# index-tts/index-tts

Hardware: AMD Instinct MI355X
Metric: audio-seconds/sec (RTF) IndexTTS-2.5, 64-utt batch @1/2/4/8 MI355X (higher is better)
Workload: dtype bf16 (GPT GEMM operands / KV cache; f32 accumulate, residual stream, norms: the reference's own GPU mode) + fp32x3 (flow matching: f32 activations / weights / accumulation, GEMM and attention products on the bf16 matrix pipe with every f32 operand carried exactly as three bf16 planes = 24 significan

## Files before the change

indextts_amd/csrc/capi_s2mel.hip:

```cpp
#include <math.h>
#include <stdlib.h>
#include <string.h>
#include <algorithm>
#include <map>
#include <string>
#include <vector>

#include "../../include/indextts_hip.h"
#include "gpt_kernels.h"
#include "s2mel_kernels.h"

static bool s2_fused(int precision, bool opt_fused) {
    if (precision == PREC_F32X3) return true;
    return (precision == PREC_BF16 || precision == PREC_F32) && opt_fused;
}

struct S2Layer {
    void *w_qkv = 0, *w_o = 0, *w_13 = 0, *w_2 = 0, *w_skip_a = 0, *w_skip_b = 0;
    float *g_attn = 0, *g_ffn = 0, *b_skip = 0;
};
struct S2Wn {
    void *w_in = 0, *w_rs = 0;
    float *b_in = 0, *b_rs = 0;
};

struct itts_s2mel {
    itts_s2mel_config cfg;
    int I = 0, Kx = 0;
    std::map<std::string, std::pair<std::vector<float>, std::vector<int64_t>>> host;
    std::vector<S2Layer> layers;
    std::vector<S2Wn> wn;
    float* g_norm = 0;
    void *w_x = 0, *w_sl_a = 0, *w_sl_b = 0, *w_c1 = 0, *w_rp = 0, *w_fl = 0, *w_c2 = 0;
    float *b_sl = 0, *b_c1 = 0, *b_rp = 0, *b_fl = 0, *b_c2 = 0;
    std::vector<void*> owned;
    bool finalized = false;
    bool opt_fused = true;
    bool opt_fused_qkv = true;
    int device = -1;
    bool profiling = false;
    std::vector<hipEvent_t> ev_pool;
    struct Rec { int cls; double flops; };
    std::vector<Rec> recs;
    hipStream_t prof_stream = nullptr;
    SeqTab tail{};
    const int* tail_src = nullptr;
    const int* tail_base = nullptr;
    bool tail_set = false;
    unsigned long long* trace = nullptr;
    int trace_cap = 0, trace_n = 0;
    int trace_wanted = 0;
    std::vector<const char*> trace_labels;
    char* capture = nullptr;
    size_t capture_bytes = 0, capture_used = 0;
    std::string capture_prefix;
    std::vector<long long> capture_off;
    std::vector<size_t> capture_len;
};

static int s2_trace(itts_s2mel* h, hipStream_t st, const char* label, const void* p, size_t bytes) {
    if (!h->trace) return ITTS_OK;
    ++h->trace_wanted;
    if (h->trace_n >= h->trace_cap) return ITTS_OK;
    if ((int)h->trace_labels.size() <= h->trace_n) { h->trace_labels.push_back(label); h->capture_off.push_back(-1); h->capture_len.push_back(0); }
    else { h->trace_labels[h->trace_n] = label; h->capture_off[h->trace_n] = -1; h->capture_len[h->trace_n] = 0; }
    if (h->capture && !h->capture_prefix.empty() && strncmp(label, h->capture_prefix.c_str(), h->capture_prefix.size()) == 0) {
        const size_t at = (h->capture_used + 255) & ~(size_t)255;
        if (at + bytes <= h->capture_bytes) {
            HIP_TRY(hipMemcpyAsync(h->capture + at, p, bytes, hipMemcpyDeviceToDevice, st));
            h->capture_off[h->trace_n] = (long long)at;
            h->capture_len[h->trace_n] = bytes;
            h->capture_used = at + bytes;
        }
    }
    return launch_trace_hash(p, bytes, h->trace + h->trace_n++, st);
}
static int s2_trace_begin(itts_s2mel* h, hipStream_t st) {
    h->trace_n = 0;
    h->trace_wanted = 0;
    h->capture_used = 0;
    if (h->trace && h->trace_cap > 0) HIP_TRY(hipMemsetAsync(h->trace, 0, (size_t)h->trace_cap * 8, st));
    return ITTS_OK;
}

enum { S2_GEMM = 0, S2_ATTN = 1, S2_OTHER = 2, S2_CLASSES = 3 };

struct S2Prof {
    itts_s2mel* h;
    hipStream_t st;
    bool on;
    size_t idx;
    S2Prof(itts_s2mel* h_, hipStream_t st_, int cls, double flops) : h(h_), st(st_), on(h_->profiling), idx(0) {
        if (!on) return;
        idx = h->recs.size();
        h->recs.push_back({cls, flops});
        while (h->ev_pool.size() < 2 * (idx + 1)) {
            hipEvent_t e;
            if (hipEventCreate(&e) != hipSuccess) { on = false; h->recs.pop_back(); return; }
            h->ev_pool.push_back(e);
        }
        (void)hipEventRecord(h->ev_pool[2 * idx], st);
    }
    ~S2Prof() { if (on) (void)hipEventRecord(h->ev_pool[2 * idx + 1], st); }
};

static int s2_upload(itts_s2mel* h, const void* host, size_t bytes, void** dst) {
    void* d = nullptr;
    HIP_TRY(hipMalloc(&d, bytes));
    h->owned.push_back(d);
    HIP_TRY(hipMemcpy(d, host, bytes, hipMemcpyHostToDevice));
    *dst = d;
    return ITTS_OK;
}

static int s2_intermediate(int H) {
    int n = (int)(2 * (4 * (long long)H) / 3);
    return n % 256 == 0 ? n : n + 256 - (n % 256);
}

extern "C" int itts_s2mel_create(const itts_s2mel_config* cfg, itts_s2mel** out) {
    if (!cfg || !out) { itts_set_error("s2mel_create: null"); return ITTS_ERR_ARG; }
    const itts_s2mel_config& c = *cfg;
    if (c.hidden_dim != c.num_heads * 64 || c.hidden_dim % 64 || c.depth < 1 || c.in_channels < 1 || c.in_channels % 4 || c.wavenet_hidden % 64 ||
        c.wavenet_layers < 1 || c.wavenet_kernel < 1 || (c.wavenet_kernel & 1) == 0 || c.wavenet_dilation_rate < 1 ||
        (c.precision != PREC_F32 && c.precision != PREC_BF16 && c.precision != PREC_F32X3)) {
        itts_set_error("s2mel_create: unsupported config (hidden=%d heads=%d: head_dim must be 64; wavenet=%d x %d k=%d; prec=%d)", c.hidden_dim,
                       c.num_heads, c.wavenet_hidden, c.wavenet_layers, c.wavenet_kernel, c.precision);
        return ITTS_ERR_ARG;
    }
    itts_s2mel* h = new itts_s2mel();
    h->cfg = c;
    h->opt_fused = itts_opt(OPT_S2MEL_FUSED) != 0;
    h->opt_fused_qkv = true;
    h->I = s2_intermediate(c.hidden_dim);
    h->Kx = (c.in_channels + 63) / 64 * 64;
    h->layers.resize(c.depth);
    h->wn.resize(c.wavenet_layers);
    h->device = itts_current_device();
    *out = h;
    return ITTS_OK;
}

extern "C" int itts_s2mel_device(const itts_s2mel* h) { return h ? h->device : -1; }

extern "C" void itts_s2mel_destroy(itts_s2mel* h) {
    if (!h) return;
    ItDevGuard dg(h->device);
    for (void* p : h->owned) (void)hipFree(p);
    for (hipEvent_t e : h->ev_pool) (void)hipEventDestroy(e);
    delete h;
}

extern "C" int itts_s2mel_set_profiling(itts_s2mel* h, int enable) {
    if (!h) { itts_set_error("s2mel_set_profiling: null"); return ITTS_ERR_ARG; }
    h->profiling = enable != 0;
    h->recs.clear();
    return ITTS_OK;
}

extern "C" int itts_s2mel_set_trace(itts_s2mel* h, void* dev_u64, int capacity) {
    if (!h || capacity < 0) { itts_set_error("s2mel_set_trace: bad args"); return ITTS_ERR_ARG; }
    h->trace = (unsigned long long*)dev_u64;
    h->trace_cap = dev_u64 ? capacity : 0;
    h->trace_n = 0;
    return ITTS_OK;
}
extern "C" int itts_s2mel_trace_count(const itts_s2mel* h) { return h ? h->trace_n : 0; }
extern "C" int itts_s2mel_trace_wanted(const itts_s2mel* h) { return h ? h->trace_wanted : 0; }
extern "C" int itts_s2mel_set_capture(itts_s2mel* h, void* dev_buf, size_t bytes, const char* label_prefix) {
    if (!h || (dev_buf && !label_prefix)) { itts_set_error("s2mel_set_capture: bad args"); return ITTS_ERR_ARG; }
    h->capture = (char*)dev_buf;
    h->capture_bytes = dev_buf ? bytes : 0;
    h->capture_used = 0;
    h->capture_prefix = dev_buf ? label_prefix : "";
    return ITTS_OK;
}
extern "C" long long itts_s2mel_capture_offset(const itts_s2mel* h, int index, size_t* bytes) {
    if (!h || index < 0 || index >= (int)h->capture_off.size() || index >= h->trace_n) return -1;
    if (bytes) *bytes = h->capture_len[index];
    return h->capture_off[index];
}
extern "C" const char* itts_s2mel_trace_label(const itts_s2mel* h, int i) {
    return (h && i >= 0 && i < (int)h->trace_labels.size()) ? h->trace_labels[i] : nullptr;
}

extern "C" int itts_s2mel_profile_read(itts_s2mel* h, double* ms, double* launches, double* flops) {
    if (!h || !ms || !launches || !flops) { itts_set_error("s2mel_profile_read: null"); return ITTS_ERR_ARG; }
    ItDevGuard dg(h->device);
    for (int i = 0; i < S2_CLASSES; ++i) ms[i] = launches[i] = flops[i] = 0;
    if (h->recs.empty()) return ITTS_OK;
    HIP_TRY(hipStreamSynchronize(h->prof_stream));
    for (size_t i = 0; i < h->recs.size(); ++i) {
        float t = 0.f;
        HIP_TRY(hipEventElapsedTime(&t, h->ev_pool[2 * i], h->ev_pool[2 * i + 1]));
        ms[h->recs[i].cls] += t; launches[h->recs[i].cls] += 1; flops[h->recs[i].cls] += h->recs[i].flops;
    }
    return ITTS_OK;
}

extern "C" int itts_s2mel_load_tensor(itts_s2mel* h, const char* name, const float* data, const int64_t* shape, int ndim) {
    if (!h || !name || !data || !shape || ndim < 1 || ndim > 3) { itts_set_error("s2mel_load_tensor: bad args"); return ITTS_ERR_ARG; }
    size_t n = 1;
    for (int i = 0; i < ndim; ++i) n *= (size_t)shape[i];
    auto& e = h->host[name];
    e.first.assign(data, data + n);
    e.second.assign(shape, shape + ndim);
    h->finalized = false;
    return ITTS_OK;
}

namespace {
struct Fin {
    itts_s2mel* h;
    std::string missing;
    const std::vector<float>* get(const std::string& name, std::initializer_list<int64_t> shape) {
        auto it = h->host.find(name);
        if (it == h->host.end()) { missing += name + " "; return nullptr; }
        const auto& sh = it->second.second;
        size_t want = 1, have = 1;
        for (auto v : shape) want *= (size_t)v;
        for (auto v : sh) have *= (size_t)v;
        if (want != have) { missing += name + "(shape) "; return nullptr; }
        return &it->second.first;
    }
    int pack_kn(const std::vector<float>& kn, int K, int Kp, int N, void** dst) {
        std::vector<float> m((size_t)Kp * N, 0.f);
        memcpy(m.data(), kn.data(), (size_t)K * N * sizeof(float));
        std::vector<char> pk(itts_packed_gemm_bytes(Kp, N, h->cfg.precision));
        int rc = itts_pack_gemm_weight(m.data(), Kp, N, 0, h->cfg.precision, pk.data());
        if (rc) return rc;
        return s2_upload(h, pk.data(), pk.size(), dst);
    }
    static std::vector<float> cols_kn(const std::vector<float>& w, int N, int ldw, int c0, int K) {
        std::vector<float> kn((size_t)K * N);
        for (int n = 0; n < N; ++n)
            for (int k = 0; k < K; ++k) kn[(size_t)k * N + n] = w[(size_t)n * ldw + c0 + k];
        return kn;
    }
    std::vector<float> pair_tiles(const std::vector<float>& kn, int K, int N) const {
        if (!s2_fused(h->cfg.precision, h->opt_fused)) return kn;
        const int half = N / 2;
        std::vector<float> o((size_t)K * N);
        for (int k = 0; k < K; ++k)
            for (int j = 0; j < half / 16; ++j)
                for (int c = 0; c < 16; ++c) {
                    o[(size_t)k * N + (2 * j) * 16 + c] = kn[(size_t)k * N + 16 * j + c];
                    o[(size_t)k * N + (2 * j + 1) * 16 + c] = kn[(size_t)k * N + half + 16 * j + c];
                }
        return o;
    }
    int vec(const std::vector<float>* v, float** dst) { return s2_upload(h, v->data(), v->size() * sizeof(float), (void**)dst); }
};
}

extern "C" int itts_s2mel_finalize(itts_s2mel* h) {
    if (!h) { itts_set_error("s2mel_finalize: null"); return ITTS_ERR_ARG; }
    ItDevGuard dg(h->device);
    const itts_s2mel_config& c = h->cfg;
    const int H = c.hidden_dim, I = h->I, W = c.wavenet_hidden, C = c.in_channels, Kx = h->Kx, k = c.wavenet_kernel, L = c.wavenet_layers;
    Fin f{h, ""};
    int rc = ITTS_OK;
    const std::string P = "estimator.";
#define NEED(var, name, ...) const std::vector<float>* var = f.get(name, {__VA_ARGS__})
    for (int i = 0; i < c.depth && rc == ITTS_OK; ++i) {
        const std::string Lp = P + "transformer.layers." + std::to_string(i) + ".";
        S2Layer& Ly = h->layers[i];
        NEED(wqkv, Lp + "attention.wqkv.weight", 3 * H, H);
        NEED(wo, Lp + "attention.wo.weight", H, H);
        NEED(w1, Lp + "feed_forward.w1.weight", I, H);
        NEED(w3, Lp + "feed_forward.w3.weight", I, H);
        NEED(w2, Lp + "feed_forward.w2.weight", H, I);
        NEED(ga, Lp + "attention_norm.norm.weight", H);
        NEED(gf, Lp + "ffn_norm.norm.weight", H);
        const bool skip = i > c.depth / 2;
        const std::vector<float>* ws = skip ? f.get(Lp + "skip_in_linear.weight", {H, 2 * H}) : nullptr;
        const std::vector<float>* bs = skip ? f.get(Lp + "skip_in_linear.bias", {H}) : nullptr;
        if (!wqkv || !wo || !w1 || !w3 || !w2 || !ga || !gf || (skip && (!ws || !bs))) continue;
        rc = f.pack_kn(Fin::cols_kn(*wqkv, 3 * H, H, 0, H), H, H, 3 * H, &Ly.w_qkv);
        if (!rc) rc = f.pack_kn(Fin::cols_kn(*wo, H, H, 0, H), H, H, H, &Ly.w_o);
        if (!rc) {
            std::vector<float> w13(*w1);
            w13.insert(w13.end(), w3->begin(), w3->end());
            rc = f.pack_kn(f.pair_tiles(Fin::cols_kn(w13, 2 * I, H, 0, H), H, 2 * I), H, H, 2 * I, &Ly.w_13);
        }
        if (!rc) rc = f.pack_kn(Fin::cols_kn(*w2, H, I, 0, I), I, I, H, &Ly.w_2);
        if (!rc) rc = f.vec(ga, &Ly.g_attn);
        if (!rc) rc = f.vec(gf, &Ly.g_ffn);
        if (!rc && skip) {
            rc = f.pack_kn(Fin::cols_kn(*ws, H, 2 * H, 0, H), H, H, H, &Ly.w_skip_a);
            if (!rc) rc = f.pack_kn(Fin::cols_kn(*ws, H, 2 * H, H, H), H, H, H, &Ly.w_skip_b);
            if (!rc) rc = f.vec(bs, &Ly.b_skip);
        }
    }
    NEED(gn, P + "transformer.norm.norm.weight", H);
    const std::vector<float>* wmerge = nullptr;
    {
        auto it = h->host.find(P + "cond_x_merge_linear.weight");
        if (it == h->host.end() || it->second.second.size() != 2 || it->second.second[0] != H) f.missing += P + "cond_x_merge_linear.weight ";
        else wmerge = &it->second.first;
    }
    NEED(wsl, P + "skip_linear.weight", H, H + C);
    NEED(bsl, P + "skip_linear.bias", H);
    NEED(wc1, P + "conv1.weight", W, H);
    NEED(bc1, P + "conv1.bias", W);
    NEED(wrp, P + "res_projection.weight", W, H);
    NEED(brp, P + "res_projection.bias", W);
    NEED(wfl, P + "final_layer.linear.weight", W, W);
    NEED(bfl, P + "final_layer.linear.bias", W);
    NEED(wc2, P + "conv2.weight", C, W);
    NEED(bc2, P + "conv2.bias", C);
    if (rc == ITTS_OK && gn && wmerge && wsl && bsl && wc1 && bc1 && wrp && brp && wfl && bfl && wc2 && bc2) {
        const int ldm = (int)h->host[P + "cond_x_merge_linear.weight"].second.back();
        if (ldm < C) { itts_set_error("s2mel_finalize: cond_x_merge_linear has %d input columns, fewer than the mel channels", ldm); return ITTS_ERR_ARG; }
        rc = f.vec(gn, &h->g_norm);
        if (!rc) rc = f.pack_kn(Fin::cols_kn(*wmerge, H, ldm, 0, C), C, Kx, H, &h->w_x);
        if (!rc) rc = f.pack_kn(Fin::cols_kn(*wsl, H, H + C, 0, H), H, H, H, &h->w_sl_a);
        if (!rc) rc = f.pack_kn(Fin::cols_kn(*wsl, H, H + C, H, C), C, Kx, H, &h->w_sl_b);
        if (!rc) rc = f.vec(bsl, &h->b_sl);
        if (!rc) rc = f.pack_kn(Fin::cols_kn(*wc1, W, H, 0, H), H, H, W, &h->w_c1);
        if (!rc) rc = f.vec(bc1, &h->b_c1);
        if (!rc) rc = f.pack_kn(Fin::cols_kn(*wrp, W, H, 0, H), H, H, W, &h->w_rp);
        if (!rc) rc = f.vec(brp, &h->b_rp);
        if (!rc) rc = f.pack_kn(Fin::cols_kn(*wfl, W, W, 0, W), W, W, W, &h->w_fl);
        if (!rc) rc = f.vec(bfl, &h->b_fl);
        if (!rc) rc = f.pack_kn(Fin::cols_kn(*wc2, C, W, 0, W), W, W, C, &h->w_c2);
        if (!rc) rc = f.vec(bc2, &h->b_c2);
    }
    for (int i = 0; i < L && rc == ITTS_OK; ++i) {
        const std::string a = P + "wavenet.in_layers." + std::to_string(i) + ".conv.conv.", b = P + "wavenet.res_skip_layers." + std::to_string(i) + ".conv.conv.";
        const int ro = i < L - 1 ? 2 * W : W;
        NEED(wi, a + "weight", 2 * W, W, k);
        NEED(bi, a + "bias", 2 * W);
        NEED(wr, b + "weight", ro, W, 1);
        NEED(br, b + "bias", ro);
        if (!wi || !bi || !wr || !br) continue;
        std::vector<float> kn((size_t)k * W * 2 * W);
        for (int n = 0; n < 2 * W; ++n)
            for (int cc = 0; cc < W; ++cc)
                for (int j = 0; j < k; ++j) kn[((size_t)j * W + cc) * 2 * W + n] = (*wi)[((size_t)n * W + cc) * k + j];
        rc = f.pack_kn(f.pair_tiles(kn, k * W, 2 * W), k * W, k * W, 2 * W, &h->wn[i].w_in);
        if (!rc) rc = f.vec(bi, &h->wn[i].b_in);
        if (!rc) rc = f.pack_kn(Fin::cols_kn(*wr, ro, W, 0, W), W, W, ro, &h->wn[i].w_rs);
        if (!rc) rc = f.vec(br, &h->wn[i].b_rs);
    }
#undef NEED
    if (rc) return rc;
    if (!f.missing.empty()) { itts_set_error("s2mel_finalize: missing or mis-shaped tensors: %s", f.missing.c_str()); return ITTS_ERR_STATE; }
    h->host.clear();
    h->finalized = true;
    return ITTS_OK;
}

extern "C" int itts_s2mel_mods_per_step(const itts_s2mel* h) {
    if (!h) return 0;
    const itts_s2mel_config& c = h->cfg;
    return c.depth * 4 * c.hidden_dim + 2 * c.hidden_dim + c.wavenet_layers * 2 * c.wavenet_hidden + 2 * c.wavenet_hidden;
}

static size_t s_a256(size_t x) { return (x + 255) & ~(size_t)255; }

struct S2Ws {
    float *X, *X2, *BIG, *WX, *OUT, *RP, *D;
    char *HB, *QA, *AO, *FC, *COL, *XA, *SK, *KC, *VC, *WXA, *ZR, *HBP;
    size_t hbp_stride;
    size_t sk_stride, total;
};

static S2Ws s2_carve(const itts_s2mel* h, char* base, int n_tok, int n_seq, int t_pad) {
    const itts_s2mel_config& c = h->cfg;
    const size_t N = (size_t)n_tok, H = c.hidden_dim, I = h->I, W = c.wavenet_hidden, C = c.in_channels, Kx = h->Kx;
    const size_t esz = c.precision == PREC_BF16 ? 2 : 4;
    const size_t big = std::max(std::max(3 * H, 2 * I), 2 * W);
    const size_t hw = std::max(H, W), fw = std::max(I, W);
    S2Ws w;
    size_t off = 0;
    auto take = [&](size_t bytes) { char* p = base ? base + off : nullptr; off += s_a256(bytes); return p; };
    w.X = (float*)take(N * H * 4);
    w.X2 = (float*)take(N * H * 4);
    w.BIG = (float*)take(N * big * 4);
    w.WX = (float*)take(N * W * 4);
    w.OUT = (float*)take(N * W * 4);
    w.RP = (float*)take(N * W * 4);
    w.D = (float*)take(N * C * 4);
    w.HB = take(N * hw * esz);
    w.QA = take(N * H * esz);
    w.AO = take(N * H * esz);
    w.FC = take(N * fw * esz);
    w.COL = take(N * (size_t)c.wavenet_kernel * W * esz);
    w.XA = take(N * Kx * esz);
    w.sk_stride = s_a256(N * H * esz);
    w.SK = take(w.sk_stride * (size_t)(c.depth / 2));
    w.WXA = take(N * W * esz);
    w.hbp_stride = (N * H + 127) / 128 * 128;
    w.HBP = take(c.precision == PREC_F32X3 ? w.hbp_stride * 6 : 0);
    const size_t kv = (size_t)n_seq * c.num_heads * t_pad * 64 * (c.precision == PREC_F32X3 ? 6 : esz);
    w.ZR = take(256);
    w.KC = take(kv);
    w.VC = take(kv);
    w.total = off + 256;
    return w;
}

extern "C" size_t itts_s2mel_workspace_bytes(const itts_s2mel* h, int n_tok, int n_seq, int t_max) {
    if (!h || n_tok <= 0 || n_seq <= 0 || t_max <= 0) return 0;
    return s2_carve(h, nullptr, n_tok, n_seq, (t_max + 63) / 64 * 64).total;
}

static int s2_launch_gemm(itts_s2mel* h, const GemmArgs& g, hipStream_t st) {
    S2Prof ps(h, st, S2_GEMM, 2.0 * g.M * (double)g.N * g.K);
    return launch_gemm(g, h->cfg.precision, true, st);
}

static int s2_gemm(itts_s2mel* h, const void* A, int lda, const void* Wp, const float* bias, float* out, int ldo, int M, int N, int K,
                   int epi, hipStream_t st, void* shadow = nullptr) {
    GemmArgs g{};
    g.A = A; g.lda = lda; g.Wp = Wp; g.bias = bias; g.M = M; g.N = N; g.K = K; g.nsplit = 1; g.epi = epi; g.out_f32 = out; g.ldo = ldo; g.D = N;
    g.out_act2 = shadow;
    return s2_launch_gemm(h, g, st);
}

static int s2_estimator(itts_s2mel* h, const S2Ws& w, const SeqTab& tab, int t_pad, const float* x_src, int src_rows, const float* const_in,
                        const float* mods, const float* rope, float* d_out, hipStream_t st, double attn_flops = 0.0,
                        const SeqTab* tail = nullptr, const int* tail_src = nullptr) {
    S2Prof whole(h, st, S2_OTHER, 0.0);
    const itts_s2mel_config& c = h->cfg;
    const int H = c.hidden_dim, I = h->I, W = c.wavenet_hidden, C = c.in_channels, Kx = h->Kx, N = tab.n_tok, prec = c.precision;
    const int nh = c.num_heads;
    const bool fused = s2_fused(prec, h->opt_fused);
    const bool x3_attn = prec == PREC_F32X3 && itts_opt(OPT_X3_ATTN) != 0;
    const size_t kv_plane = (size_t)tab.n_seq * nh * t_pad * 64;
    const bool a_planes = prec == PREC_F32X3 && fused && itts_opt(OPT_X3_APLANES) != 0 && itts_opt(OPT_X3_PRODUCTS) == 6 && itts_opt(OPT_X3_SCHED) != 0 && H % 32 == 0;
    int rc;
    float *X = w.X, *X2 = w.X2;
    const size_t esz = prec == PREC_BF16 ? 2 : 4;
    const size_t kvb = kv_plane * (prec == PREC_F32X3 ? (x3_attn ? 6 : 4) : esz);
#define S2_TRACE(label, ptr, bytes) do { if (h->trace && (rc = s2_trace(h, st, label, ptr, bytes))) return rc; } while (0)
    if ((rc = launch_cast_pad(x_src, w.XA, N, src_rows, C, Kx, prec, st))) return rc;
    HIP_TRY(hipMemcpyAsync(X, const_in, (size_t)N * H * 4, hipMemcpyDeviceToDevice, st));
    S2_TRACE("cast_pad(x) -> XA", w.XA, (size_t)N * Kx * esz);
    if ((rc = s2_gemm(h, w.XA, Kx, h->w_x, nullptr, X, H, N, H, Kx, EPI_RESIDUAL, st))) return rc;
    S2_TRACE("x_in GEMM -> X", X, (size_t)N * H * 4);
    int n_skip = 0;
    for (int i = 0; i < c.depth; ++i) {
        const S2Layer& L = h->layers[i];
        if (i > c.depth / 2) {
            if (!fused && (rc = launch_cast_pad(X, w.HB, N, N, H, H, prec, st))) return rc;
            --n_skip;
            if ((rc = s2_gemm(h, w.HB, H, L.w_skip_a, L.b_skip, X2, H, N, H, H, EPI_STORE_F32, st))) return rc;
            if ((rc = s2_gemm(h, w.SK + w.sk_stride * n_skip, H, L.w_skip_b, nullptr, X2, H, N, H, H, EPI_RESIDUAL, st))) return rc;
            S2_TRACE("skip_in GEMMs -> X", X2, (size_t)N * H * 4);
            float* tmp = X; X = X2; X2 = tmp;
        }
        if (a_planes) {
            if ((rc = launch_ada_rmsnorm_planes(X, L.g_attn, mods + (size_t)i * 4 * H, w.HBP, w.hbp_stride, N, H, c.norm_eps, st))) return rc;
            S2_TRACE("ada_rmsnorm(attn) -> HB planes", w.HBP, w.hbp_stride * 6);
        } else {
            if ((rc = launch_ada_rmsnorm(X, L.g_attn, mods + (size_t)i * 4 * H, w.HB, N, H, c.norm_eps, prec, st))) return rc;
            S2_TRACE("ada_rmsnorm(attn) -> HB", w.HB, (size_t)N * H * esz);
        }
        if (fused && h->opt_fused_qkv) {
            GemmArgs g{};
            g.A = w.HB; g.lda = H; g.Wp = L.w_qkv; g.M = N; g.N = 3 * H; g.K = H; g.nsplit = 1; g.epi = EPI_QKV_ROPE;
            if (a_planes) { g.A = w.HBP; g.a_planes = w.hbp_stride; }
            g.out_act = w.QA; g.kcache = w.KC; g.vcache = w.VC; g.D = H; g.H = nh; g.Tmax = t_pad;
            g.tok_seq = tab.tok_seq; g.tok_t = tab.tok_t; g.rope = rope;
            g.kv_planes = x3_attn ? kv_plane : 0;
            if ((rc = s2_launch_gemm(h, g, st))) return rc;
        } else {
            if ((rc = s2_gemm(h, w.HB, H, L.w_qkv, nullptr, w.BIG, 3 * H, N, 3 * H, H, EPI_STORE_F32, st))) return rc;
            if ((rc = launch_rope_split(w.BIG, rope, w.QA, w.KC, w.VC, tab, nh, t_pad, prec, st))) return rc;
        }
        S2_TRACE("wqkv -> Q", w.QA, (size_t)N * H * esz);
        S2_TRACE("wqkv -> K", w.KC, kvb);
        S2_TRACE("wqkv -> V^T", w.VC, kvb);
        { S2Prof ps(h, st, S2_ATTN, attn_flops);
          if (x3_attn) rc = launch_s2mel_attention_x3(w.QA, w.KC, w.VC, w.AO, tab, nh, t_pad, st);
          else rc = launch_s2mel_attention(w.QA, w.KC, w.VC, w.AO, tab, nh, t_pad, prec, st);
          if (rc) return rc; }
        S2_TRACE("attention -> AO", w.AO, (size_t)N * H * esz);
        if ((rc = s2_gemm(h, w.AO, H, L.w_o, nullptr, X, H, N, H, H, EPI_RESIDUAL, st))) return rc;
        S2_TRACE("wo GEMM -> X", X, (size_t)N * H * 4);
        if (a_planes) {
            if ((rc = launch_ada_rmsnorm_planes(X, L.g_ffn, mods + (size_t)i * 4 * H + 2 * H, w.HBP, w.hbp_stride, N, H, c.norm_eps, st))) return rc;
            S2_TRACE("ada_rmsnorm(ffn) -> HB planes", w.HBP, w.hbp_stride * 6);
        } else {
            if ((rc = launch_ada_rmsnorm(X, L.g_ffn, mods + (size_t)i * 4 * H + 2 * H, w.HB, N, H, c.norm_eps, prec, st))) return rc;
            S2_TRACE("ada_rmsnorm(ffn) -> HB", w.HB, (size_t)N * H * esz);
        }
        if (fused) {
            GemmArgs g{};
            g.A = w.HB; g.lda = H; g.Wp = L.w_13; g.M = N; g.N = 2 * I; g.K = H; g.nsplit = 1; g.epi = EPI_SWIGLU; g.out_act = w.FC; g.D = I;
            if (a_planes) { g.A = w.HBP; g.a_planes = w.hbp_stride; }
            if ((rc = s2_launch_gemm(h, g, st))) return rc;
        } else {
            if ((rc = s2_gemm(h, w.HB, H, L.w_13, nullptr, w.BIG, 2 * I, N, 2 * I, H, EPI_STORE_F32, st))) return rc;
            if ((rc = launch_swiglu(w.BIG, w.FC, N, I, prec, st))) return rc;
        }
        void* shadow = nullptr;
        if (fused && i < c.depth / 2) shadow = w.SK + w.sk_stride * n_skip;
        else if (fused && i + 1 < c.depth && i + 1 > c.depth / 2) shadow = w.HB;
        S2_TRACE("w13 + SwiGLU -> FC", w.FC, (size_t)N * I * esz);
        if ((rc = s2_gemm(h, w.FC, I, L.w_2, nullptr, X, H, N, H, I, EPI_RESIDUAL, st, shadow))) return rc;
        S2_TRACE("w2 GEMM -> X", X, (size_t)N * H * 4);
        if (i < c.depth / 2) {
            if (!fused && (rc = launch_cast_pad(X, w.SK + w.sk_stride * n_skip, N, N, H, H, prec, st))) return rc;
            ++n_skip;
        }
    }
    const float* m_norm = mods + (size_t)c.depth * 4 * H;
    const float* m_gc = m_norm + 2 * H;
    const float* m_fl = m_gc + (size_t)c.wavenet_layers * 2 * W;
    const SeqTab& tt = tail ? *tail : tab;
    const void* XAt = w.XA;
    if (tail) {
        if ((rc = launch_cast_pad(x_src, w.QA, tail->n_tok, src_rows, C, Kx, prec, st, tail_src))) return rc;
        XAt = w.QA;
    }
    const int NT = tt.n_tok;
    if ((rc = launch_ada_rmsnorm(X, h->g_norm, m_norm, w.HB, NT, H, c.norm_eps, prec, st, tail ? tail_src : nullptr))) return rc;
    S2_TRACE("final ada_rmsnorm -> HB", w.HB, (size_t)NT * H * esz);
    if ((rc = s2_gemm(h, w.HB, H, h->w_sl_a, h->b_sl, X2, H, NT, H, H, EPI_STORE_F32, st))) return rc;
    if ((rc = s2_gemm(h, XAt, Kx, h->w_sl_b, nullptr, X2, H, NT, H, Kx, EPI_RESIDUAL, st, fused ? w.HB : nullptr))) return rc;
    if (!fused && (rc = launch_cast_pad(X2, w.HB, NT, NT, H, H, prec, st))) return rc;
    S2_TRACE("skip_linear -> X2", X2, (size_t)NT * H * 4);
    if ((rc = s2_gemm(h, w.HB, H, h->w_c1, h->b_c1, w.WX, W, NT, W, H, EPI_STORE_F32, st, fused ? w.WXA : nullptr))) return rc;
    S2_TRACE("conv1 -> WX", w.WX, (size_t)NT * W * 4);
    if ((rc = s2_gemm(h, w.HB, H, h->w_rp, h->b_rp, w.RP, W, NT, W, H, EPI_STORE_F32, st))) return rc;
    int dil = 1;
    for (int i = 0; i < c.wavenet_layers; ++i) {
        const S2Wn& Wn = h->wn[i];
        const int last = i == c.wavenet_layers - 1;
        if (!fused && (rc = launch_im2col_reflect(w.WX, w.COL, tt, W, c.wavenet_kernel, dil, prec, st))) return rc;
        const int ro = last ? W : 2 * W;
        if (fused) {
            GemmArgs g{};
            g.A = w.WXA; g.lda = W; g.Wp = Wn.w_in; g.bias = Wn.b_in; g.M = NT; g.N = 2 * W; g.K = c.wavenet_kernel * W;
            g.nsplit = 1; g.epi = EPI_GATE; g.out_act = w.FC; g.gvec = m_gc + (size_t)i * 2 * W; g.D = W;
            g.conv_taps = c.wavenet_kernel; g.conv_dil = dil; g.conv_W = W; g.tok_seq = tt.tok_seq; g.tok_t = tt.tok_t;
            g.seq_start = tt.seq_start; g.seq_T = tt.seq_T; g.zero_row = w.ZR;
            if ((rc = s2_launch_gemm(h, g, st))) return rc;
            GemmArgs r{};
            r.A = w.FC; r.lda = W; r.Wp = Wn.w_rs; r.bias = Wn.b_rs; r.M = NT; r.N = ro; r.K = W; r.nsplit = 1; r.epi = EPI_WN_RS;
            r.out_f32 = w.WX; r.out2 = w.OUT; r.D = W; r.wn_first = i == 0; r.wn_last = last; r.out_act2 = last ? nullptr : w.WXA;
            r.tok_seq = tt.tok_seq; r.tok_t = tt.tok_t; r.seq_len = tt.seq_len;
            S2_TRACE("wavenet in_layer + gate -> FC", w.FC, (size_t)NT * W * esz);
            if ((rc = s2_launch_gemm(h, r, st))) return rc;
            S2_TRACE("wavenet res_skip -> WX", w.WX, (size_t)NT * W * 4);
            S2_TRACE("wavenet res_skip -> OUT", w.OUT, (size_t)NT * W * 4);
        } else {
            if ((rc = s2_gemm(h, w.COL, c.wavenet_kernel * W, Wn.w_in, Wn.b_in, w.BIG, 2 * W, NT, 2 * W, c.wavenet_kernel * W, EPI_STORE_F32, st))) return rc;
            if ((rc = launch_wn_gate(w.BIG, m_gc + (size_t)i * 2 * W, w.FC, NT, W, prec, st))) return rc;
            if ((rc = s2_gemm(h, w.FC, W, Wn.w_rs, Wn.b_rs, w.BIG, ro, NT, ro, W, EPI_STORE_F32, st))) return rc;
            if ((rc = launch_wn_update(w.BIG, w.WX, w.OUT, tt, W, i == 0, last, st))) return rc;
        }
        dil *= c.wavenet_dilation_rate;
    }
    if ((rc = launch_final_ln_mod(w.OUT, w.RP, m_fl, w.HB, tt, W, prec, st))) return rc;
    if ((rc = s2_gemm(h, w.HB, W, h->w_fl, h->b_fl, w.BIG, W, NT, W, W, EPI_STORE_F32, st, fused ? w.FC : nullptr))) return rc;
    if (!fused && (rc = launch_cast_pad(w.BIG, w.FC, NT, NT, W, W, prec, st))) return rc;
    S2_TRACE("final_layer -> FC", w.FC, (size_t)NT * W * esz);
    if ((rc = s2_gemm(h, w.FC, W, h->w_c2, h->b_c2, d_out, C, NT, C, W, EPI_STORE_F32, st))) return rc;
    S2_TRACE("conv2 -> output", d_out, (size_t)NT * C * 4);
    return ITTS_OK;
#undef S2_TRACE
}

static int s2_check(const itts_s2mel* h, const void* a, const void* b, const char* who) {
    const int da = itts_ptr_device(a), db = itts_ptr_device(b);
    if ((da >= 0 && da != h->device) || (db >= 0 && db != h->device)) {
        itts_set_error("%s: tensors are on device %d/%d but the model was created on device %d", who, da, db, h->device);
        return ITTS_ERR_ARG;
    }
    return ITTS_OK;
}

static SeqTab s2_tab(const int32_t* tok_seq, const int32_t* tok_t, const int32_t* seq_start, const int32_t* seq_T, const int32_t* seq_len,
                     int n_seq, int n_tok, int t_max) {
    SeqTab t;
    t.tok_seq = tok_seq; t.tok_t = tok_t; t.seq_start = seq_start; t.seq_T = seq_T; t.seq_len = seq_len;
    t.n_seq = n_seq; t.n_tok = n_tok; t.t_max = t_max;
    return t;
}

extern "C" int itts_s2mel_estimator(itts_s2mel* h, const float* x, const float* const_in, const float* mods, const float* rope,
                                    const int32_t* tok_seq, const int32_t* tok_t, const int32_t* seq_start, const int32_t* seq_T,
                                    const int32_t* seq_len, int n_seq, int n_tok, int t_max, float* d_out, void* workspace,
                                    size_t workspace_bytes, void* stream) {
    if (!h || !x || !const_in || !mods || !rope || !tok_seq || !tok_t || !seq_start || !seq_T || !seq_len || !d_out || !workspace) {
        itts_set_error("s2mel_estimator: null pointer");
        return ITTS_ERR_ARG;
    }
    if (!h->finalized) { itts_set_error("s2mel_estimator: call itts_s2mel_finalize first"); return ITTS_ERR_STATE; }
    if (n_seq <= 0 || n_tok <= 0 || t_max <= 0) { itts_set_error("s2mel_estimator: bad sizes"); return ITTS_ERR_ARG; }
    ItDevGuard dg(h->device);
    if (int rc = s2_check(h, x, workspace, "s2mel_estimator")) return rc;
    const int t_pad = (t_max + 63) / 64 * 64;
    const S2Ws w0 = s2_carve(h, nullptr, n_tok, n_seq, t_pad);
    if (workspace_bytes < w0.total) { itts_set_error("s2mel_estimator: workspace too small (%zu < %zu)", workspace_bytes, w0.total); return ITTS_ERR_ARG; }
    char* base = (char*)(((uintptr_t)workspace + 255) & ~(uintptr_t)255);
    const S2Ws w = s2_carve(h, base, n_tok, n_seq, t_pad);
    hipStream_t st = (hipStream_t)stream;
    const size_t kv = (size_t)((char*)w.VC - (char*)w.KC);
    HIP_TRY(hipMemsetAsync(w.ZR, 0, (size_t)((char*)w.KC - (char*)w.ZR) + 2 * kv, st));
    const SeqTab tab = s2_tab(tok_seq, tok_t, seq_start, seq_T, seq_len, n_seq, n_tok, t_max);
    h->recs.clear();
    h->prof_stream = st;
    if (int rc = s2_trace_begin(h, st)) return rc;
    return s2_estimator(h, w, tab, t_pad, x, n_tok, const_in, mods, rope, d_out, st);
}

extern "C" int itts_s2mel_solve(itts_s2mel* h, float* x_state, const float* const_in, const float* mods, const float* rope,
                                const int32_t* tok_seq, const int32_t* tok_t, const int32_t* seq_start, const int32_t* seq_T,
                                const int32_t* seq_len, const int32_t* prompt_len, int n_seq, int n_tok, int t_max, int n_branch,
                                int n_steps, const float* t_span, float cfg_rate, void* workspace, size_t workspace_bytes, void* stream) {
    if (!h || !x_state || !const_in || !mods || !rope || !tok_seq || !tok_t || !seq_start || !seq_T || !seq_len || !prompt_len || !t_span || !workspace) {
        itts_set_error("s2mel_solve: null pointer");
        return ITTS_ERR_ARG;
    }
    if (!h->finalized) { itts_set_error("s2mel_solve: call itts_s2mel_finalize first"); return ITTS_ERR_STATE; }
    if (n_seq <= 0 || n_tok <= 0 || t_max <= 0 || n_steps < 1 || (n_branch != 1 && n_branch != 2) || n_tok % n_branch || n_seq % n_branch) {
        itts_set_error("s2mel_solve: bad sizes (n_seq=%d n_tok=%d n_branch=%d n_steps=%d)", n_seq, n_tok, n_branch, n_steps);
        return ITTS_ERR_ARG;
    }
    ItDevGuard dg(h->device);
    if (int rc = s2_check(h, x_state, workspace, "s2mel_solve")) return rc;
    const int t_pad = (t_max + 63) / 64 * 64;
    const S2Ws w0 = s2_carve(h, nullptr, n_tok, n_seq, t_pad);
    if (workspace_bytes < w0.total) { itts_set_error("s2mel_solve: workspace too small (%zu < %zu)", workspace_bytes, w0.total); return ITTS_ERR_ARG; }
    char* base = (char*)(((uintptr_t)workspace + 255) & ~(uintptr_t)255);
    const S2Ws w = s2_carve(h, base, n_tok, n_seq, t_pad);
    hipStream_t st = (hipStream_t)stream;
    const size_t kv = (size_t)((char*)w.VC - (char*)w.KC);
    HIP_TRY(hipMemsetAsync(w.ZR, 0, (size_t)((char*)w.KC - (char*)w.ZR) + 2 * kv, st));
    const SeqTab tab = s2_tab(tok_seq, tok_t, seq_start, seq_T, seq_len, n_seq, n_tok, t_max);
    const int mps = itts_s2mel_mods_per_step(h);
    h->recs.clear();
    h->prof_stream = st;
    if (int rc = s2_trace_begin(h, st)) return rc;
    for (int step = 0; step < n_steps; ++step) {
        const bool use_tail = h->tail_set && h->tail.n_seq == n_seq && h->tail.n_tok > 0 && h->tail.n_tok <= n_tok && h->tail.n_tok % n_branch == 0;
        int rc = s2_estimator(h, w, tab, t_pad, x_state, n_tok / n_branch, const_in, mods + (size_t)step * mps, rope, w.D, st, 0.0,
                              use_tail ? &h->tail : nullptr, use_tail ? h->tail_src : nullptr);
        if (rc) return rc;
        const float dt = t_span[step + 1] - t_span[step];
        if ((rc = launch_euler_update(x_state, w.D, tab, prompt_len, h->cfg.in_channels, n_branch, dt, cfg_rate, st,
                                      use_tail ? h->tail_base : nullptr, use_tail ? h->tail.n_tok / n_branch : 0))) return rc;
    }
    return ITTS_OK;
}

extern "C" int itts_s2mel_set_tail(itts_s2mel* h, const int32_t* tok_seq, const int32_t* tok_t, const int32_t* seq_start, const int32_t* seq_T,
                                   const int32_t* seq_len, const int32_t* tail_src, const int32_t* tail_base, int n_seq, int n_tail, int t_max) {
    if (!h) { itts_set_error("s2mel_set_tail: null"); return ITTS_ERR_ARG; }
    if (!tok_seq) { h->tail_set = false; return ITTS_OK; }
    if (!tok_t || !seq_start || !seq_T || !seq_len || !tail_src || !tail_base || n_seq <= 0 || n_tail <= 0 || t_max <= 0) {
        itts_set_error("s2mel_set_tail: bad args");
        return ITTS_ERR_ARG;
    }
    h->tail = s2_tab(tok_seq, tok_t, seq_start, seq_T, seq_len, n_seq, n_tail, t_max);
    h->tail_src = tail_src; h->tail_base = tail_base; h->tail_set = true;
    return ITTS_OK;
}

extern "C" size_t itts_s2mel_attention_scratch_bytes(int n_tok, int n_seq, int heads, int t_max, int precision) {
    const size_t esz = precision == PREC_BF16 ? 2 : 4;
    const size_t t_pad = (size_t)(t_max + 63) / 64 * 64;
    const size_t planes = precision == PREC_F32X3 ? 2 * s_a256((size_t)n_seq * heads * t_pad * 64 * 6) : 0;
    return s_a256((size_t)n_tok * heads * 64 * esz) + 2 * s_a256((size_t)n_seq * heads * t_pad * 64 * esz) + planes + 256;
}

extern "C" int itts_s2mel_attention_forward(const float* qkv, const float* rope, const int32_t* tok_seq, const int32_t* tok_t,
                                            const int32_t* seq_start, const int32_t* seq_T, const int32_t* seq_len, int n_seq, int n_tok,
                                            int t_max, int heads, int precision, void* out, void* scratch, size_t scratch_bytes, void* stream) {
    if (!qkv || !rope || !tok_seq || !tok_t || !seq_start || !seq_T || !seq_len || !out || !scratch) { itts_set_error("s2mel_attention: null pointer"); return ITTS_ERR_ARG; }
    if (n_seq <= 0 || n_tok <= 0 || t_max <= 0 || heads <= 0 || (precision != PREC_F32 && precision != PREC_BF16 && precision != PREC_F32X3)) { itts_set_error("s2mel_attention: bad sizes"); return ITTS_ERR_ARG; }
    if (scratch_bytes < itts_s2mel_attention_scratch_bytes(n_tok, n_seq, heads, t_max, precision)) { itts_set_error("s2mel_attention: scratch too small"); return ITTS_ERR_ARG; }
    const size_t esz = precision == PREC_BF16 ? 2 : 4;
    const int t_pad = (t_max + 63) / 64 * 64;
    char* base = (char*)(((uintptr_t)scratch + 255) & ~(uintptr_t)255);
    char* q = base;
    char* k = q + s_a256((size_t)n_tok * heads * 64 * esz);
    const size_t kv = s_a256((size_t)n_seq * heads * t_pad * 64 * esz);
    char* v = k + kv;
    hipStream_t st = (hipStream_t)stream;
    HIP_TRY(hipMemsetAsync(k, 0, 2 * kv, st));
    const SeqTab tab = s2_tab(tok_seq, tok_t, seq_start, seq_T, seq_len, n_seq, n_tok, t_max);
    int rc = launch_rope_split(qkv, rope, q, k, v, tab, heads, t_pad, precision == PREC_F32X3 ? PREC_F32 : precision, st);
    if (rc) return rc;
    if (precision == PREC_F32X3) {
        const size_t n = (size_t)n_seq * heads * t_pad * 64;
        char* kp = v + kv;
        char* vp = kp + s_a256(n * 6);
        if ((rc = launch_split_planes((const float*)k, kp, n, st))) return rc;
        if ((rc = launch_split_planes((const float*)v, vp, n, st))) return rc;
        return launch_s2mel_attention_x3(q, kp, vp, out, tab, heads, t_pad, st);
    }
    return launch_s2mel_attention(q, k, v, out, tab, heads, t_pad, precision, st);
}
```

indextts_amd/csrc/common.h:

```cpp
#pragma once
#include <hip/hip_runtime.h>
#include <stdint.h>
#include <stdio.h>
#include <string.h>

#define ITTS_OK 0
#define ITTS_ERR_ARG 1
#define ITTS_ERR_HIP 2
#define ITTS_ERR_STATE 3
#define ITTS_ERR_NOMEM 4

#define HIP_TRY(expr)                                                                         \
    do {                                                                                      \
        hipError_t _e = (expr);                                                               \
        if (_e != hipSuccess) {                                                               \
            itts_set_error("%s:%d %s -> %s", __FILE__, __LINE__, #expr, hipGetErrorString(_e)); \
            return ITTS_ERR_HIP;                                                              \
        }                                                                                     \
    } while (0)

void itts_set_error(const char* fmt, ...);

enum { OPT_DECODE_FUSE_LN, OPT_DECODE_GEMM, OPT_DECODE_ROT, OPT_DECODE_WNT, OPT_DECODE_NT, OPT_PREFILL_GEMM, OPT_TILE256, OPT_F32_TILE,
       OPT_X3_PRODUCTS, OPT_X3_SCHED, OPT_X3_ATTN, OPT_SAMPLE_RADIX, OPT_GPT_COMPACT, OPT_ATTN_WAVES, OPT_S2MEL_FUSED, OPT_FA_QS,
       OPT_F32_ATTN_SCALAR, OPT_FA32_QS, OPT_AA_ACT, OPT_CONV_BM, OPT_H3_KERNEL, OPT_DECODE_LN_NT, OPT_X3_APLANES, OPT_X3_PIN, OPT_PREFILL_ATTN, OPT_VOC_ACT_PLANES, OPT_X3_WAVES, OPT_COUNT };
int itts_opt(int id);
unsigned itts_opt_epoch();

typedef float f32x4 __attribute__((ext_vector_type(4)));
typedef float f32x16 __attribute__((ext_vector_type(16)));
typedef short bf16x8 __attribute__((ext_vector_type(8)));
typedef unsigned short u16;

static inline int ceil_div(int a, int b) { return (a + b - 1) / b; }

struct ItDevGuard {
    int prev = -1;
    bool switched = false;
    explicit ItDevGuard(int dev) {
        if (dev < 0) return;
        if (hipGetDevice(&prev) != hipSuccess) { prev = -1; (void)hipGetLastError(); }
        if (prev != dev && hipSetDevice(dev) == hipSuccess) switched = true;
    }
    ~ItDevGuard() { if (switched && prev >= 0) (void)hipSetDevice(prev); }
    ItDevGuard(const ItDevGuard&) = delete;
    ItDevGuard& operator=(const ItDevGuard&) = delete;
};
static inline int itts_current_device() {
    int d = -1;
    if (hipGetDevice(&d) != hipSuccess) { d = -1; (void)hipGetLastError(); }
    return d;
}
static inline int itts_ptr_device(const void* p) {
    hipPointerAttribute_t at;
    if (!p || hipPointerGetAttributes(&at, p) != hipSuccess) { (void)hipGetLastError(); return -1; }
    return at.type == hipMemoryTypeDevice ? at.device : -1;
}

template <class T>
struct ItPerDevice {
    T v[32] = {};
    T& cur() {
        const int d = itts_current_device();
        return v[(d >= 0 && d < 32) ? d : 0];
    }
};

#ifdef __HIPCC__
__device__ __forceinline__ float wave_sum(float v) {
#pragma unroll
    for (int o = 32; o > 0; o >>= 1) v += __shfl_xor(v, o, 64);
    return v;
}
__device__ __forceinline__ float wave_max(float v) {
#pragma unroll
    for (int o = 32; o > 0; o >>= 1) v = fmaxf(v, __shfl_xor(v, o, 64));
    return v;
}
__device__ __forceinline__ float bf16_to_f32(u16 h) { return __uint_as_float(((uint32_t)h) << 16); }
__device__ __forceinline__ u16 f32_to_bf16(float f) {
    uint32_t u = __float_as_uint(f);
    if ((u & 0x7fffffffu) > 0x7f800000u) return (u16)((u >> 16) | 0x40);
    u += 0x7fffu + ((u >> 16) & 1u);
    return (u16)(u >> 16);
}
#endif

static inline u16 host_f32_to_bf16(float f) {
    uint32_t u;
    memcpy(&u, &f, 4);
    if ((u & 0x7fffffffu) > 0x7f800000u) return (u16)((u >> 16) | 0x40);
    u += 0x7fffu + ((u >> 16) & 1u);
    return (u16)(u >> 16);
}
```

indextts_amd/csrc/gemm_tile.h:

```cpp
#pragma once
#include "gpt_kernels.h"
#include <type_traits>

typedef __bf16 bf16x8_t __attribute__((ext_vector_type(8)));
typedef unsigned int v4u __attribute__((ext_vector_type(4)));

__device__ __forceinline__ float gelu_new_f(float x) {
    const float c = 0.7978845608028654f;
    return 0.5f * x * (1.0f + tanhf(c * (x + 0.044715f * x * x * x)));
}

#define PF_BM 128
#define PF_BN 128
#define PF_BK 64
#define PF_GM 8
#define PF_LDS 67584
#ifndef PF_SCHED
#define PF_SCHED 1
#endif

__device__ __forceinline__ uint32_t pf_pack2(float a, float b) { return (uint32_t)f32_to_bf16(a) | ((uint32_t)f32_to_bf16(b) << 16); }

template <int EPI>
__device__ __forceinline__ void pf_epilogue(const GemmArgs& a, int mbase, int nbase, int lane, f32x4 v) {
    const int n = nbase + (lane & 15);
    if (n >= a.N) return;
    const float bias = a.bias ? a.bias[n] : 0.f;
    int which = 0, c = n;
    if constexpr (EPI == EPI_QKV || EPI == EPI_QKV_ROPE) { which = n / a.D; c = n - which * a.D; }
    if constexpr (EPI == EPI_QKV_ROPE) {
        const int hd = c >> 6, d = c & 63, i = d >> 1;
        const bool odd = d & 1;
#pragma unroll
        for (int r = 0; r < 4; ++r) {
            const int m = mbase + (lane >> 4) * 4 + r;
            const int mc = m < a.M ? m : a.M - 1;
            const float val = v[r] + bias;
            const float partner = __shfl_xor(val, 1, 64);
            const int s = a.tok_seq[mc], t = a.tok_t[mc];
            float y = val;
            if (which < 2) {
                const float cs = a.rope[((size_t)t * 32 + i) * 2], sn = a.rope[((size_t)t * 32 + i) * 2 + 1];
                y = odd ? val * cs + partner * sn : val * cs - partner * sn;
            }
            if (m < a.M) {
                if (which == 0) ((u16*)a.out_act)[(size_t)m * a.D + c] = f32_to_bf16(y);
                else if (which == 1) ((u16*)a.kcache)[(((size_t)s * a.H + hd) * a.Tmax + t) * 64 + d] = f32_to_bf16(y);
                else ((u16*)a.vcache)[(((size_t)s * a.H + hd) * 64 + d) * a.Tmax + t] = f32_to_bf16(y);
            }
        }
        return;
    }
#pragma unroll
    for (int r = 0; r < 4; ++r) {
        const int m = mbase + (lane >> 4) * 4 + r;
        if (m >= a.M) continue;
        const float val = v[r] + bias;
        if constexpr (EPI == EPI_STORE_F32) {
            a.out_f32[(size_t)m * a.ldo + n] = val;
            if (a.out_act2) ((u16*)a.out_act2)[(size_t)m * a.ldo + n] = f32_to_bf16(val);
        } else if constexpr (EPI == EPI_RESIDUAL) {
            const float nv = a.out_f32[(size_t)m * a.ldo + n] + val;
            a.out_f32[(size_t)m * a.ldo + n] = nv;
            if (a.out_act2) ((u16*)a.out_act2)[(size_t)m * a.ldo + n] = f32_to_bf16(nv);
        } else if constexpr (EPI == EPI_GELU_ACT) ((u16*)a.out_act)[(size_t)m * a.ldo + n] = f32_to_bf16(gelu_new_f(val));
        else if constexpr (EPI == EPI_WN_RS) {
            if (a.wn_last || n >= a.D) {
                float* o = a.out2 + (size_t)m * a.D + (a.wn_last ? n : n - a.D);
                *o = a.wn_first ? val : *o + val;
            } else {
                const float mask = a.tok_t[m] < a.seq_len[a.tok_seq[m]] ? 1.f : 0.f;
                float* o = a.out_f32 + (size_t)m * a.D + n;
                *o = (*o + val) * mask;
            }
        } else {
            if (which == 0) {
                a.qbuf[(size_t)m * a.D + c] = val;
            } else {
                const int b = m / a.S, si = m - b * a.S;
                const size_t pb = (size_t)b * (a.seq_mul > 1 ? a.seq_mul : 1);
                const int pos = *a.pos_ptr + si - (a.pos_shift ? a.pos_shift[pb] : 0);
                const size_t o = ((pb * a.H + (c >> 6)) * a.Tmax + pos) * 64 + (c & 63);
                ((u16*)(which == 1 ? a.kcache : a.vcache))[o] = f32_to_bf16(val);
            }
        }
    }
}

typedef __bf16 pf_bf16x2_t __attribute__((ext_vector_type(2)));
typedef float pf_f32x2_t __attribute__((ext_vector_type(2)));
typedef unsigned int v2u_t __attribute__((ext_vector_type(2)));
__device__ __forceinline__ uint32_t pf_cvt2(float a, float b) { return __builtin_bit_cast(uint32_t, __builtin_convertvector(pf_f32x2_t{a, b}, pf_bf16x2_t)); }
__device__ __forceinline__ v2u_t pf_cvt4(f32x4 v) { return v2u_t{pf_cvt2(v[0], v[1]), pf_cvt2(v[2], v[3])}; }

__device__ __forceinline__ void pf_split4(const f32x4 v, v2u_t& H, v2u_t& M, v2u_t& L) {
#pragma unroll
    for (int i = 0; i < 2; ++i) {
        const float a = v[2 * i], b = v[2 * i + 1];
        const uint32_t h = pf_cvt2(a, b);
        const float ra = a - __uint_as_float(h << 16), rb = b - __uint_as_float(h & 0xffff0000u);
        const uint32_t m = pf_cvt2(ra, rb);
        const float sa = ra - __uint_as_float(m << 16), sb = rb - __uint_as_float(m & 0xffff0000u);
        H[i] = h; M[i] = m; L[i] = pf_cvt2(sa, sb);
    }
}
__device__ __forceinline__ void pf_store_planes4(void* base, size_t stride, size_t idx, const f32x4 v) {
    v2u_t h, m, l;
    pf_split4(v, h, m, l);
    u16* p = (u16*)base + idx;
    *(v2u_t*)p = h; *(v2u_t*)(p + stride) = m; *(v2u_t*)(p + 2 * stride) = l;
}
__device__ __forceinline__ void pf_store_planes1(void* base, size_t stride, size_t idx, float x) {
    const u16 h = f32_to_bf16(x);
    const float r = x - bf16_to_f32(h);
    const u16 m = f32_to_bf16(r);
    u16* p = (u16*)base + idx;
    p[0] = h; p[stride] = m; p[2 * stride] = f32_to_bf16(r - bf16_to_f32(m));
}

__device__ __forceinline__ float pf_sigmoid(float x) { return __builtin_amdgcn_rcpf(1.0f + __builtin_amdgcn_exp2f(-1.4426950408889634f * x)); }
__device__ __forceinline__ float pf_tanh(float x) { return 1.0f - 2.0f * __builtin_amdgcn_rcpf(1.0f + __builtin_amdgcn_exp2f(2.8853900817779268f * x)); }
template <bool F32> __device__ __forceinline__ float pf_sigmoid_t(float x) { if constexpr (F32) return 1.0f / (1.0f + expf(-x)); else return pf_sigmoid(x); }
template <bool F32> __device__ __forceinline__ float pf_tanh_t(float x) { if constexpr (F32) return tanhf(x); else return pf_tanh(x); }
template <bool F32> __device__ __forceinline__ void pf_store_act4(void* base, size_t idx, f32x4 v) {
    if constexpr (F32) *(f32x4*)((float*)base + idx) = v;
    else *(v2u_t*)((u16*)base + idx) = pf_cvt4(v);
}

template <int EPI, int ROWS>
__device__ __forceinline__ void pf_stage_meta(const GemmArgs& a, int* meta, int m0, int ltid) {
    if constexpr (EPI == EPI_QKV_ROPE || EPI == EPI_WN_RS) {
        if (ltid < ROWS) {
            int m = m0 + ltid;
            m = m < a.M ? m : a.M - 1;
            const int sq = a.tok_seq[m], t = a.tok_t[m];
            if constexpr (EPI == EPI_QKV_ROPE) { meta[ltid] = sq; meta[ROWS + ltid] = t; }
            else meta[ltid] = (a.wn_last || t < a.seq_len[sq]) ? 1 : 0;
        }
    }
}

__device__ __forceinline__ f32x4 pf_rope4(const f32x4 v, const f32x4 cs) {
    float t0 = v[1] * cs[1], t1 = v[1] * cs[0], t2 = v[3] * cs[3], t3 = v[3] * cs[2];
    asm volatile("" : "+v"(t0), "+v"(t1), "+v"(t2), "+v"(t3));
    float y0 = __builtin_fmaf(v[0], cs[0], -t0);
    asm volatile("" : "+v"(y0));
    float y1 = __builtin_fmaf(v[0], cs[1], t1);
    asm volatile("" : "+v"(y1));
    float y2 = __builtin_fmaf(v[2], cs[2], -t2);
    asm volatile("" : "+v"(y2));
    float y3 = __builtin_fmaf(v[2], cs[3], t3);
    asm volatile("" : "+v"(y3));
    return f32x4{y0, y1, y2, y3};
}

template <int EPI, int ROWS, int NT, bool F32 = false>
__device__ __forceinline__ void pf_store_tile(const GemmArgs& a, const float* ct, const int* meta, int m0, int n0, int tid) {
    constexpr bool PAIR = (EPI == EPI_SWIGLU || EPI == EPI_GATE);
    constexpr int CH = PAIR ? 16 : 32;
    constexpr int RSTEP = NT / CH;
    const int half = a.N >> 1;
    const int c4 = tid % CH, row0 = tid / CH;
    const int j = c4 >> 2, cc = (c4 & 3) * 4;
    const int n = PAIR ? (n0 >> 1) + j * 16 + cc : n0 + c4 * 4;
    if (PAIR ? n >= half : n >= a.N) return;
    const f32x4 zero4{0.f, 0.f, 0.f, 0.f};
    f32x4 b1 = zero4, b2 = zero4;
    if constexpr (EPI == EPI_GATE) {
        b1 = *(const f32x4*)(a.gvec + n);
        b2 = *(const f32x4*)(a.gvec + half + n);
        if (a.bias) {
            const f32x4 x1 = *(const f32x4*)(a.bias + n), x2 = *(const f32x4*)(a.bias + half + n);
#pragma unroll
            for (int q = 0; q < 4; ++q) { b1[q] += x1[q]; b2[q] += x2[q]; }
        }
    } else if constexpr (!PAIR) {
        if (a.bias) b1 = *(const f32x4*)(a.bias + n);
    }
    int which = 0, c = n;
    if constexpr (EPI == EPI_QKV || EPI == EPI_QKV_ROPE) { which = n / a.D; c = n - which * a.D; }
    const int hd = c >> 6, d = c & 63;
    const int ca = PAIR ? (2 * j) * 16 + cc : c4 * 4, cb = (2 * j + 1) * 16 + cc;
#pragma unroll 4
    for (int i = 0; i < ROWS / RSTEP; ++i) {
        const int row = row0 + i * RSTEP;
        const int m = m0 + row;
        if (m >= a.M) break;
        const int sw = ((row >> 2) & 3) << 4;
        if constexpr (PAIR) {
            const f32x4 va = *(const f32x4*)(ct + row * 128 + (ca ^ sw));
            const f32x4 vb = *(const f32x4*)(ct + row * 128 + (cb ^ sw));
            f32x4 o;
            if constexpr (EPI == EPI_SWIGLU) {
#pragma unroll
                for (int q = 0; q < 4; ++q) o[q] = va[q] * pf_sigmoid_t<F32>(va[q]) * vb[q];
            } else {
#pragma unroll
                for (int q = 0; q < 4; ++q) o[q] = pf_tanh_t<F32>(va[q] + b1[q]) * pf_sigmoid_t<F32>(vb[q] + b2[q]);
            }
            pf_store_act4<F32>(a.out_act, (size_t)m * half + n, o);
        } else {
            f32x4 v = *(const f32x4*)(ct + row * 128 + (ca ^ sw));
#pragma unroll
            for (int q = 0; q < 4; ++q) v[q] += b1[q];
            if constexpr (EPI == EPI_STORE_F32) {
                *(f32x4*)(a.out_f32 + (size_t)m * a.ldo + n) = v;
                if (a.out_act2) pf_store_act4<F32>(a.out_act2, (size_t)m * a.ldo + n, v);
            } else if constexpr (EPI == EPI_RESIDUAL) {
                f32x4* o = (f32x4*)(a.out_f32 + (size_t)m * a.ldo + n);
                const f32x4 old = *o;
#pragma unroll
                for (int q = 0; q < 4; ++q) v[q] += old[q];
                *o = v;
                if (a.out_act2) pf_store_act4<F32>(a.out_act2, (size_t)m * a.ldo + n, v);
            } else if constexpr (EPI == EPI_GELU_ACT) {
#pragma unroll
                for (int q = 0; q < 4; ++q) v[q] = gelu_new_f(v[q]);
                if constexpr (F32) *(f32x4*)((float*)a.out_act + (size_t)m * a.ldo + n) = v;
                else *(v2u_t*)((u16*)a.out_act + (size_t)m * a.ldo + n) = v2u_t{(uint32_t)f32_to_bf16(v[0]) | ((uint32_t)f32_to_bf16(v[1]) << 16),
                                                                               (uint32_t)f32_to_bf16(v[2]) | ((uint32_t)f32_to_bf16(v[3]) << 16)};
            } else if constexpr (EPI == EPI_WN_RS) {
                if (a.wn_last || n >= a.D) {
                    f32x4* o = (f32x4*)(a.out2 + (size_t)m * a.D + (a.wn_last ? n : n - a.D));
                    if (!a.wn_first) {
                        const f32x4 old = *o;
#pragma unroll
                        for (int q = 0; q < 4; ++q) v[q] += old[q];
                    }
                    *o = v;
                } else {
                    const float mask = (float)meta[row];
                    f32x4* o = (f32x4*)(a.out_f32 + (size_t)m * a.D + n);
                    const f32x4 old = *o;
#pragma unroll
                    for (int q = 0; q < 4; ++q) v[q] = (old[q] + v[q]) * mask;
                    *o = v;
                    if (a.out_act2) pf_store_act4<F32>(a.out_act2, (size_t)m * a.D + n, v);
                }
            } else if constexpr (EPI == EPI_QKV) {
                if (which == 0) {
                    *(f32x4*)(a.qbuf + (size_t)m * a.D + c) = v;
                } else {
                    const int b = m / a.S, si = m - b * a.S;
                    const size_t pb = (size_t)b * (a.seq_mul > 1 ? a.seq_mul : 1);
                    const int pos = *a.pos_ptr + si - (a.pos_shift ? a.pos_shift[pb] : 0);
                    const size_t o = ((pb * a.H + hd) * a.Tmax + pos) * 64 + d;
                    if constexpr (F32) *(f32x4*)((float*)(which == 1 ? a.kcache : a.vcache) + o) = v;
                    else *(v2u_t*)((u16*)(which == 1 ? a.kcache : a.vcache) + o) =
                        v2u_t{(uint32_t)f32_to_bf16(v[0]) | ((uint32_t)f32_to_bf16(v[1]) << 16), (uint32_t)f32_to_bf16(v[2]) | ((uint32_t)f32_to_bf16(v[3]) << 16)};
                }
            } else {
                const int sq = meta[row], t = meta[ROWS + row];
                if (which < 2) {
                    const f32x4 cs = *(const f32x4*)(a.rope + ((size_t)t * 32 + (d >> 1)) * 2);
                    const f32x4 y = pf_rope4(v, cs);
                    if (which == 0) pf_store_act4<F32>(a.out_act, (size_t)m * a.D + c, y);
                    else if (F32 && a.kv_planes) pf_store_planes4(a.kcache, a.kv_planes, (((size_t)sq * a.H + hd) * a.Tmax + t) * 64 + d, y);
                    else pf_store_act4<F32>(a.kcache, (((size_t)sq * a.H + hd) * a.Tmax + t) * 64 + d, y);
                } else if constexpr (F32) {
                    const size_t o = (((size_t)sq * a.H + hd) * 64 + d) * a.Tmax + t;
                    if (a.kv_planes) {
#pragma unroll
                        for (int q = 0; q < 4; ++q) pf_store_planes1(a.vcache, a.kv_planes, o + (size_t)q * a.Tmax, v[q]);
                    } else {
                        float* vt = (float*)a.vcache + o;
#pragma unroll
                        for (int q = 0; q < 4; ++q) vt[(size_t)q * a.Tmax] = v[q];
                    }
                } else {
                    u16* vt = (u16*)a.vcache + (((size_t)sq * a.H + hd) * 64 + d) * a.Tmax + t;
                    const v2u_t pk = pf_cvt4(v);
                    vt[0] = (u16)(pk.x & 0xffffu);
                    vt[(size_t)a.Tmax] = (u16)(pk.x >> 16);
                    vt[(size_t)2 * a.Tmax] = (u16)(pk.y & 0xffffu);
                    vt[(size_t)3 * a.Tmax] = (u16)(pk.y >> 16);
                }
            }
        }
    }
}

template <int ROWS, int NT, bool F32 = false>
__device__ __forceinline__ void pf_store_vt(const GemmArgs& a, const float* ctT, int m0, int n0, int tid) {
    constexpr int RQ = ROWS / 4, CSTEP = NT / RQ;
    const int rq = tid % RQ, col0 = tid / RQ;
    const int m = m0 + 4 * rq;
    if (m >= a.M) return;
    const int ml = m + 3 < a.M ? m + 3 : a.M - 1;
    const int s0 = a.tok_seq[m], t0 = a.tok_t[m];
    const bool run = m + 3 < a.M && a.tok_seq[ml] == s0;
    const bool wide = run && (((t0 | a.Tmax) & 3) == 0);
    int sq[4], tq[4];
    if (!run) {
#pragma unroll
        for (int q = 0; q < 4; ++q) { const int mq = m + q < a.M ? m + q : a.M - 1; sq[q] = a.tok_seq[mq]; tq[q] = a.tok_t[mq]; }
    }
#pragma unroll 4
    for (int i = 0; i < 128 / CSTEP; ++i) {
        const int col = col0 + i * CSTEP;
        const int n = n0 + col;
        if (n >= a.N) break;
        f32x4 v = *(const f32x4*)(ctT + col * (ROWS + 4) + 4 * rq);
        if (a.bias) {
            const float b = a.bias[n];
#pragma unroll
            for (int q = 0; q < 4; ++q) v[q] += b;
        }
        const int c = n - 2 * a.D, hd = c >> 6, d = c & 63;
        if constexpr (F32) {
            if (a.kv_planes) {
                if (run && wide) {
                    pf_store_planes4(a.vcache, a.kv_planes, (((size_t)s0 * a.H + hd) * 64 + d) * a.Tmax + t0, v);
                } else {
#pragma unroll
                    for (int q = 0; q < 4; ++q)
                        if (m + q < a.M) {
                            const size_t o = run ? (((size_t)s0 * a.H + hd) * 64 + d) * a.Tmax + t0 + q : (((size_t)sq[q] * a.H + hd) * 64 + d) * a.Tmax + tq[q];
                            pf_store_planes1(a.vcache, a.kv_planes, o, v[q]);
                        }
                }
                continue;
            }
            if (run) {
                float* vt = (float*)a.vcache + (((size_t)s0 * a.H + hd) * 64 + d) * a.Tmax + t0;
                if (wide) *(f32x4*)vt = v;
                else { vt[0] = v[0]; vt[1] = v[1]; vt[2] = v[2]; vt[3] = v[3]; }
            } else {
#pragma unroll
                for (int q = 0; q < 4; ++q)
                    if (m + q < a.M) ((float*)a.vcache)[(((size_t)sq[q] * a.H + hd) * 64 + d) * a.Tmax + tq[q]] = v[q];
            }
            continue;
        }
        const v2u_t pk = pf_cvt4(v);
        if (run) {
            u16* vt = (u16*)a.vcache + (((size_t)s0 * a.H + hd) * 64 + d) * a.Tmax + t0;
            if (wide) {
                *(v2u_t*)vt = pk;
            } else {
                vt[0] = (u16)(pk.x & 0xffffu); vt[1] = (u16)(pk.x >> 16); vt[2] = (u16)(pk.y & 0xffffu); vt[3] = (u16)(pk.y >> 16);
            }
        } else {
            const u16 e[4] = {(u16)(pk.x & 0xffffu), (u16)(pk.x >> 16), (u16)(pk.y & 0xffffu), (u16)(pk.y >> 16)};
#pragma unroll
            for (int q = 0; q < 4; ++q)
                if (m + q < a.M) ((u16*)a.vcache)[(((size_t)sq[q] * a.H + hd) * 64 + d) * a.Tmax + tq[q]] = e[q];
        }
    }
}

static inline bool pf_vec_ok(const GemmArgs& a) {
    return (a.N % 4 == 0) && (a.ldo % 4 == 0 || (a.epi != EPI_STORE_F32 && a.epi != EPI_RESIDUAL && a.epi != EPI_GELU_ACT)) && (a.D % 4 == 0);
}
static inline bool pf_f32_ok(const GemmArgs& a) {
    return a.K % 32 == 0 && a.lda % 4 == 0 && a.nsplit == 1 && a.epi != EPI_PARTIAL && pf_vec_ok(a) && (((uintptr_t)a.A) & 15) == 0;
}
```

indextts_amd/csrc/gemm_x3.hip:

```cpp
#include "gemm_tile.h"

#define X3_LDS PF_LDS
#define X3_LDS_ONE (96 * 1024)

typedef const __attribute__((address_space(1))) char* pf_gptr_t;
__device__ __forceinline__ pf_gptr_t pf_uni(const char* p) {
    const uint64_t u = (uint64_t)p;
    const uint32_t lo = __builtin_amdgcn_readfirstlane((uint32_t)u), hi = __builtin_amdgcn_readfirstlane((uint32_t)(u >> 32));
    return (pf_gptr_t)(((uint64_t)hi << 32) | lo);
}

__device__ __forceinline__ void x3_split8(const f32x4 p0, const f32x4 p1, v4u& H, v4u& M, v4u& L) {
    const float x[8] = {p0[0], p0[1], p0[2], p0[3], p1[0], p1[1], p1[2], p1[3]};
#pragma unroll
    for (int i = 0; i < 4; ++i) {
        const float a = x[2 * i], b = x[2 * i + 1];
        const uint32_t h = pf_cvt2(a, b);
        const float ra = a - __uint_as_float(h << 16), rb = b - __uint_as_float(h & 0xffff0000u);
        const uint32_t m = pf_cvt2(ra, rb);
        const float sa = ra - __uint_as_float(m << 16), sb = rb - __uint_as_float(m & 0xffff0000u);
        H[i] = h; M[i] = m; L[i] = pf_cvt2(sa, sb);
    }
}

template <int EPI, bool CONV = false, int NPROD = 8, bool SCHED = true, bool APL = false>
__global__ __launch_bounds__(256, 2) void gemm_x3_kernel(GemmArgs a) {
    extern __shared__ __attribute__((aligned(16))) char pf_sm[];
    const int lane = threadIdx.x & 63, w = __builtin_amdgcn_readfirstlane(threadIdx.x >> 6);
    const int wr = w >> 1, wc = w & 1;
    const int n_mt = (a.M + PF_BM - 1) / PF_BM, n_nt = (a.N + PF_BN - 1) / PF_BN;
    const int total = n_mt * n_nt, per = (total + 7) >> 3;
    const int t = (int)(blockIdx.x & 7) * per + (int)(blockIdx.x >> 3);
    if (t >= total) return;
    const int g0 = t / (PF_GM * n_nt), first_m = g0 * PF_GM;
    const int gm = (n_mt - first_m) < PF_GM ? (n_mt - first_m) : PF_GM;
    const int r = t - g0 * PF_GM * n_nt;
    const int bn = r / gm, bm = first_m + (r - bn * gm);
    const int m0 = bm * PF_BM, nt0 = bn * (PF_BN / 16);
    const int nk = a.K >> 5;
    const int ntiles = (a.N + 15) >> 4;

    constexpr int STAGE = APL ? 24576 : 16384;
    const char* asrc[APL ? 6 : 4];
    uint32_t aoff[APL ? 6 : 4];
    const char* abase = (const char*)a.A + (size_t)m0 * a.lda * (APL ? 2 : 4);
    int cv_t[4], cv_T[4];
    const char* cv_base[4];
    const char* cv_zero[4];
    const int cv_kpt = CONV ? a.conv_W / 32 : 1;
    const int cv_left = CONV ? (a.conv_taps - 1) * a.conv_dil - ((a.conv_taps - 1) * a.conv_dil) / 2 : 0;
    if constexpr (APL) {
#pragma unroll
        for (int i = 0; i < 6; ++i) {
            const int pl = i >> 1, c = w + 4 * (i & 1);
            int m = m0 + c * 16 + (lane >> 2);
            m = m < a.M ? m : a.M - 1;
            const int piece = (lane & 3) ^ ((lane >> 4) & 3);
            asrc[i] = (const char*)a.A + ((size_t)pl * a.a_planes + (size_t)m * a.lda) * 2 + piece * 16;
            aoff[i] = (uint32_t)(m - m0) * (uint32_t)a.lda * 2u + piece * 16;
        }
    } else {
#pragma unroll
    for (int i = 0; i < 4; ++i) {
        const int c = w * 4 + i;
        const int row_t = c * 8 + (lane >> 3), row16 = row_t & 15;
        const int piece = (lane & 7) ^ ((row16 >> 1) & 7);
        int m = m0 + row_t;
        m = m < a.M ? m : a.M - 1;
        asrc[i] = (const char*)a.A + (size_t)m * a.lda * 4 + piece * 16;
        aoff[i] = (uint32_t)(m - m0) * (uint32_t)a.lda * 4u + piece * 16;
        if constexpr (CONV) {
            const int sq = a.tok_seq[m];
            cv_t[i] = a.tok_t[m];
            cv_T[i] = a.seq_T[sq];
            cv_base[i] = (const char*)a.A + (size_t)a.seq_start[sq] * a.lda * 4 + piece * 16;
            cv_zero[i] = (const char*)a.zero_row + piece * 16;
        }
    }
    }
    const char* wbase[4];
    const uint32_t lane16 = lane * 16;
#pragma unroll
    for (int nt = 0; nt < 4; ++nt) {
        int ntile = nt0 + wc * 4 + nt;
        ntile = ntile < ntiles ? ntile : ntiles - 1;
        wbase[nt] = (const char*)a.Wp + (size_t)ntile * nk * 3072;
    }
    auto issue_a = [&](int kt, int buf) {
        char* base = pf_sm + buf * STAGE;
        if constexpr (APL) {
#pragma unroll
            for (int i = 0; i < 6; ++i)
                __builtin_amdgcn_global_load_lds((const __attribute__((address_space(1))) void*)(pf_uni(abase + (size_t)(i >> 1) * a.a_planes * 2 + (size_t)kt * 64) + aoff[i]),
                                                 (__attribute__((address_space(3))) void*)(base + (i >> 1) * 8192 + (w + 4 * (i & 1)) * 1024), 16, 0, 0);
            return;
        }
        int tap = 0, rem = kt;
        if constexpr (CONV) { tap = kt / cv_kpt; rem = kt - tap * cv_kpt; }
#pragma unroll
        for (int i = 0; i < 4; ++i) {
            const char* ap = asrc[i] + (size_t)kt * 128;
            if constexpr (CONV) {
                const int maxpad = cv_left;
                const int Tv = cv_T[i] <= maxpad ? maxpad + 1 : cv_T[i];
                int p = cv_t[i] + tap * a.conv_dil - cv_left;
                p = p < 0 ? -p : p;
                p = p >= Tv ? 2 * (Tv - 1) - p : p;
                const bool ok = p >= 0 && p < cv_T[i];
                ap = ok ? cv_base[i] + ((size_t)p * a.lda + (size_t)rem * 32) * 4 : cv_zero[i];
            }
            if constexpr (CONV)
                __builtin_amdgcn_global_load_lds((const __attribute__((address_space(1))) void*)ap,
                                                 (__attribute__((address_space(3))) void*)(base + (w * 4 + i) * 1024), 16, 0, 0);
            else
                __builtin_amdgcn_global_load_lds((const __attribute__((address_space(1))) void*)(pf_uni(abase + (size_t)kt * 128) + aoff[i]),
                                                 (__attribute__((address_space(3))) void*)(base + (w * 4 + i) * 1024), 16, 0, 0);
        }
    };
    auto load_w = [&](int kt, v4u (&bw)[4][3]) {
#pragma unroll
        for (int nt = 0; nt < 4; ++nt)
#pragma unroll
            for (int p = 0; p < 3; ++p) bw[nt][p] = *(const __attribute__((address_space(1))) v4u*)(pf_uni(wbase[nt] + (size_t)kt * 3072) + lane16 + p * 1024);
    };

    f32x4 acc[4][4];
#pragma unroll
    for (int i = 0; i < 4; ++i)
#pragma unroll
        for (int j = 0; j < 4; ++j) acc[i][j] = f32x4{0.f, 0.f, 0.f, 0.f};

    const int row16 = lane & 15, kg = lane >> 4;
    int a_off[2];
#pragma unroll
    for (int s2 = 0; s2 < 2; ++s2) {
        const int pos = (s2 * 4 + kg) ^ ((row16 >> 1) & 7);
        a_off[s2] = (row16 >> 3) * 1024 + ((row16 & 7) * 8 + pos) * 16;
    }
    const int a_wave = wr * 4 * 2048;
    const int a_off_pl = (row16 * 4 + (kg ^ ((row16 >> 2) & 3))) * 16;

    auto ktile = [&](int kt, v4u (&bw)[4][3], v4u (&bn_)[4][3]) {
        asm volatile("s_waitcnt vmcnt(0)" ::: "memory");
        __syncthreads();
        if (kt + 1 < nk) {
            issue_a(kt + 1, (kt + 1) & 1);
            load_w(kt + 1, bn_);
        }
        const char* base = pf_sm + (kt & 1) * STAGE;
        v4u ap[3], an[3];
        if constexpr (APL) {
#pragma unroll
            for (int pl = 0; pl < 3; ++pl) ap[pl] = *(const v4u*)(base + pl * 8192 + wr * 4096 + a_off_pl);
        } else {
            const f32x4 p0 = *(const f32x4*)(base + a_wave + a_off[0]);
            const f32x4 p1 = *(const f32x4*)(base + a_wave + a_off[1]);
            x3_split8(p0, p1, ap[0], ap[1], ap[2]);
        }
#pragma unroll
        for (int mt = 0; mt < 4; ++mt) {
            if (mt < 3) {
                if constexpr (APL) {
#pragma unroll
                    for (int pl = 0; pl < 3; ++pl) an[pl] = *(const v4u*)(base + pl * 8192 + wr * 4096 + (mt + 1) * 1024 + a_off_pl);
                } else {
                const f32x4 p0 = *(const f32x4*)(base + a_wave + (mt + 1) * 2048 + a_off[0]);
                const f32x4 p1 = *(const f32x4*)(base + a_wave + (mt + 1) * 2048 + a_off[1]);
                x3_split8(p0, p1, an[0], an[1], an[2]);
                }
            }
            constexpr int PA[8] = {2, 1, 2, 0, 1, 1, 0, 0};
            constexpr int PB[8] = {1, 2, 0, 2, 1, 0, 1, 0};
#pragma unroll
            for (int q = 8 - NPROD; q < 8; ++q)
#pragma unroll
                for (int nt = 0; nt < 4; ++nt)
                    acc[mt][nt] = __builtin_amdgcn_mfma_f32_16x16x32_bf16(__builtin_bit_cast(bf16x8_t, ap[PA[q]]),
                                                                          __builtin_bit_cast(bf16x8_t, bw[nt][PB[q]]), acc[mt][nt], 0, 0, 0);
            if (APL && mt < 3) {
                __builtin_amdgcn_sched_group_barrier(0x100, 3, 0);
                __builtin_amdgcn_sched_group_barrier(0x008, 4 * NPROD, 0);
            }
            if (!APL && SCHED && mt < 3) {
                __builtin_amdgcn_sched_group_barrier(0x100, 2, 0);
#pragma unroll
                for (int i = 0; i < 2 * NPROD; ++i) {
                    __builtin_amdgcn_sched_group_barrier(0x008, 2, 0);
                    __builtin_amdgcn_sched_group_barrier(0x002, 3, 0);
                }
            }
            if (mt < 3) { ap[0] = an[0]; ap[1] = an[1]; ap[2] = an[2]; }
        }
    };
    v4u bw0[4][3], bw1[4][3];
    issue_a(0, 0);
    load_w(0, bw0);
    for (int kt = 0; kt < nk; kt += 2) {
        ktile(kt, bw0, bw1);
        if (kt + 1 < nk) ktile(kt + 1, bw1, bw0);
    }
    __syncthreads();
    float* ct = (float*)pf_sm;
    const int g = lane >> 4, c16 = lane & 15;
    if (EPI == EPI_QKV_ROPE && a.D % 128 == 0 && nt0 * 16 >= 2 * a.D) {
#pragma unroll
        for (int mt = 0; mt < 4; ++mt)
#pragma unroll
            for (int nt = 0; nt < 4; ++nt) *(f32x4*)(ct + (wc * 64 + nt * 16 + c16) * 132 + wr * 64 + mt * 16 + g * 4) = acc[mt][nt];
        __syncthreads();
        pf_store_vt<128, 256, true>(a, ct, m0, nt0 * 16, threadIdx.x);
        return;
    }
#pragma unroll
    for (int mt = 0; mt < 4; ++mt)
#pragma unroll
        for (int nt = 0; nt < 4; ++nt)
#pragma unroll
            for (int rr = 0; rr < 4; ++rr)
                ct[(wr * 64 + mt * 16 + g * 4 + rr) * 128 + ((wc * 64 + nt * 16 + c16) ^ (g << 4))] = acc[mt][nt][rr];
    int* meta = (int*)(pf_sm + 65536);
    pf_stage_meta<EPI, 128>(a, meta, m0, threadIdx.x);
    __syncthreads();
    pf_store_tile<EPI, 128, 256, true>(a, ct, meta, m0, nt0 * 16, threadIdx.x);
}


#define X3W8_STAGE (16384 + 24576)
#define X3W8_LDS (2 * X3W8_STAGE)
template <int EPI, bool CONV = false>
__global__ __launch_bounds__(512, 2) void gemm_x3w8_kernel(GemmArgs a) {
    extern __shared__ __attribute__((aligned(16))) char pf_sm[];
    constexpr int NPROD = 6;
    const int lane = threadIdx.x & 63, w = __builtin_amdgcn_readfirstlane(threadIdx.x >> 6);
    const int wr = w >> 1, wc = w & 1;
    const int n_mt = (a.M + PF_BM - 1) / PF_BM, n_nt = (a.N + PF_BN - 1) / PF_BN;
    const int total = n_mt * n_nt, per = (total + 7) >> 3;
    const int t = (int)(blockIdx.x & 7) * per + (int)(blockIdx.x >> 3);
    if (t >= total) return;
    const int g0 = t / (PF_GM * n_nt), first_m = g0 * PF_GM;
    const int gm = (n_mt - first_m) < PF_GM ? (n_mt - first_m) : PF_GM;
    const int r = t - g0 * PF_GM * n_nt;
    const int bn = r / gm, bm = first_m + (r - bn * gm);
    const int m0 = bm * PF_BM, nt0 = bn * (PF_BN / 16);
    const int nk = a.K >> 5;
    const int ntiles = (a.N + 15) >> 4;

    const char* asrc[2];
    uint32_t aoff[2];
    const char* abase = (const char*)a.A + (size_t)m0 * a.lda * 4;
    int cv_t[2], cv_T[2];
    const char* cv_base[2];
    const char* cv_zero[2];
    const int cv_kpt = CONV ? a.conv_W / 32 : 1;
    const int cv_left = CONV ? (a.conv_taps - 1) * a.conv_dil - ((a.conv_taps - 1) * a.conv_dil) / 2 : 0;
#pragma unroll
    for (int i = 0; i < 2; ++i) {
        const int c = w * 2 + i;
        const int row_t = c * 8 + (lane >> 3), row16 = row_t & 15;
        const int piece = (lane & 7) ^ ((row16 >> 1) & 7);
        int m = m0 + row_t;
        m = m < a.M ? m : a.M - 1;
        asrc[i] = (const char*)a.A + (size_t)m * a.lda * 4 + piece * 16;
        aoff[i] = (uint32_t)(m - m0) * (uint32_t)a.lda * 4u + piece * 16;
        if constexpr (CONV) {
            const int sq = a.tok_seq[m];
            cv_t[i] = a.tok_t[m];
            cv_T[i] = a.seq_T[sq];
            cv_base[i] = (const char*)a.A + (size_t)a.seq_start[sq] * a.lda * 4 + piece * 16;
            cv_zero[i] = (const char*)a.zero_row + piece * 16;
        }
    }
    const char* wdma[3];
    const uint32_t lane16 = lane * 16;
#pragma unroll
    for (int i = 0; i < 3; ++i) {
        const int q = w + 8 * i;
        int ntile = nt0 + q / 3;
        ntile = ntile < ntiles ? ntile : ntiles - 1;
        wdma[i] = (const char*)a.Wp + (size_t)ntile * nk * 3072 + (q % 3) * 1024;
    }
    auto issue = [&](int kt, int buf) {
        char* base = pf_sm + buf * X3W8_STAGE;
        int tap = 0, rem = kt;
        if constexpr (CONV) { tap = kt / cv_kpt; rem = kt - tap * cv_kpt; }
#pragma unroll
        for (int i = 0; i < 2; ++i) {
            if constexpr (CONV) {
                const int maxpad = cv_left;
                const int Tv = cv_T[i] <= maxpad ? maxpad + 1 : cv_T[i];
                int p = cv_t[i] + tap * a.conv_dil - cv_left;
                p = p < 0 ? -p : p;
                p = p >= Tv ? 2 * (Tv - 1) - p : p;
                const bool ok = p >= 0 && p < cv_T[i];
                const char* ap = ok ? cv_base[i] + ((size_t)p * a.lda + (size_t)rem * 32) * 4 : cv_zero[i];
                __builtin_amdgcn_global_load_lds((const __attribute__((address_space(1))) void*)ap,
                                                 (__attribute__((address_space(3))) void*)(base + (w * 2 + i) * 1024), 16, 0, 0);
            } else {
                (void)asrc;
                __builtin_amdgcn_global_load_lds((const __attribute__((address_space(1))) void*)(pf_uni(abase + (size_t)kt * 128) + aoff[i]),
                                                 (__attribute__((address_space(3))) void*)(base + (w * 2 + i) * 1024), 16, 0, 0);
            }
        }
#pragma unroll
        for (int i = 0; i < 3; ++i)
            __builtin_amdgcn_global_load_lds((const __attribute__((address_space(1))) void*)(pf_uni(wdma[i] + (size_t)kt * 3072) + lane16),
                                             (__attribute__((address_space(3))) void*)(base + 16384 + (w + 8 * i) * 1024), 16, 0, 0);
    };

    f32x4 acc[2][4];
#pragma unroll
    for (int i = 0; i < 2; ++i)
#pragma unroll
        for (int j = 0; j < 4; ++j) acc[i][j] = f32x4{0.f, 0.f, 0.f, 0.f};

    const int row16 = lane & 15, kg = lane >> 4;
    int a_off[2];
#pragma unroll
    for (int s2 = 0; s2 < 2; ++s2) {
        const int pos = (s2 * 4 + kg) ^ ((row16 >> 1) & 7);
        a_off[s2] = (row16 >> 3) * 1024 + ((row16 & 7) * 8 + pos) * 16;
    }
    const int a_wave = wr * 2 * 2048;

    issue(0, 0);
    for (int kt = 0; kt < nk; ++kt) {
        asm volatile("s_waitcnt vmcnt(0)" ::: "memory");
        __syncthreads();
        if (kt + 1 < nk) issue(kt + 1, (kt + 1) & 1);
        const char* base = pf_sm + (kt & 1) * X3W8_STAGE;
        v4u bw[4][3];
#pragma unroll
        for (int nt = 0; nt < 4; ++nt)
#pragma unroll
            for (int p = 0; p < 3; ++p) bw[nt][p] = *(const v4u*)(base + 16384 + ((wc * 4 + nt) * 3 + p) * 1024 + lane16);
        v4u ap[3], an[3];
        {
            const f32x4 p0 = *(const f32x4*)(base + a_wave + a_off[0]);
            const f32x4 p1 = *(const f32x4*)(base + a_wave + a_off[1]);
            x3_split8(p0, p1, ap[0], ap[1], ap[2]);
        }
#pragma unroll
        for (int mt = 0; mt < 2; ++mt) {
            if (mt < 1) {
                const f32x4 p0 = *(const f32x4*)(base + a_wave + (mt + 1) * 2048 + a_off[0]);
                const f32x4 p1 = *(const f32x4*)(base + a_wave + (mt + 1) * 2048 + a_off[1]);
                x3_split8(p0, p1, an[0], an[1], an[2]);
            }
            constexpr int PA[8] = {2, 1, 2, 0, 1, 1, 0, 0};
            constexpr int PB[8] = {1, 2, 0, 2, 1, 0, 1, 0};
#pragma unroll
            for (int q = 8 - NPROD; q < 8; ++q)
#pragma unroll
                for (int nt = 0; nt < 4; ++nt)
                    acc[mt][nt] = __builtin_amdgcn_mfma_f32_16x16x32_bf16(__builtin_bit_cast(bf16x8_t, ap[PA[q]]),
                                                                          __builtin_bit_cast(bf16x8_t, bw[nt][PB[q]]), acc[mt][nt], 0, 0, 0);
            if (mt < 1) {
                __builtin_amdgcn_sched_group_barrier(0x100, 2, 0);
#pragma unroll
                for (int i = 0; i < 2 * NPROD; ++i) {
                    __builtin_amdgcn_sched_group_barrier(0x008, 2, 0);
                    __builtin_amdgcn_sched_group_barrier(0x002, 3, 0);
                }
                ap[0] = an[0]; ap[1] = an[1]; ap[2] = an[2];
            }
        }
    }
    __syncthreads();
    float* ct = (float*)pf_sm;
    const int g = lane >> 4, c16 = lane & 15;
    if (EPI == EPI_QKV_ROPE && a.D % 128 == 0 && nt0 * 16 >= 2 * a.D) {
#pragma unroll
        for (int mt = 0; mt < 2; ++mt)
#pragma unroll
            for (int nt = 0; nt < 4; ++nt) *(f32x4*)(ct + (wc * 64 + nt * 16 + c16) * 132 + wr * 32 + mt * 16 + g * 4) = acc[mt][nt];
        __syncthreads();
        pf_store_vt<128, 512, true>(a, ct, m0, nt0 * 16, threadIdx.x);
        return;
    }
#pragma unroll
    for (int mt = 0; mt < 2; ++mt)
#pragma unroll
        for (int nt = 0; nt < 4; ++nt)
#pragma unroll
            for (int rr = 0; rr < 4; ++rr)
                ct[(wr * 32 + mt * 16 + g * 4 + rr) * 128 + ((wc * 64 + nt * 16 + c16) ^ (g << 4))] = acc[mt][nt][rr];
    int* meta = (int*)(pf_sm + 65536);
    pf_stage_meta<EPI, 128>(a, meta, m0, threadIdx.x);
    __syncthreads();
    pf_store_tile<EPI, 128, 512, true>(a, ct, meta, m0, nt0 * 16, threadIdx.x);
}

template <int EPI, bool CONV = false>
static int launch_gemm_x3_e(const GemmArgs& a, hipStream_t st) {
    const int n_mt = ceil_div(a.M, PF_BM), n_nt = ceil_div(a.N, PF_BN);
    const int per = ceil_div(n_mt * n_nt, 8);
    const int nprod = itts_opt(OPT_X3_PRODUCTS) == 6 ? 6 : 8;
    const bool sched = itts_opt(OPT_X3_SCHED) != 0;
    static ItPerDevice<bool> attr_set_pd;
    bool& attr_set = attr_set_pd.cur();
    if (!attr_set) {
        HIP_TRY(hipFuncSetAttribute((const void*)gemm_x3_kernel<EPI, CONV, 8, true>, hipFuncAttributeMaxDynamicSharedMemorySize, X3_LDS_ONE));
        HIP_TRY(hipFuncSetAttribute((const void*)gemm_x3_kernel<EPI, CONV, 6, true>, hipFuncAttributeMaxDynamicSharedMemorySize, X3_LDS_ONE));
        HIP_TRY(hipFuncSetAttribute((const void*)gemm_x3_kernel<EPI, CONV, 8, false>, hipFuncAttributeMaxDynamicSharedMemorySize, X3_LDS_ONE));
        HIP_TRY(hipFuncSetAttribute((const void*)gemm_x3_kernel<EPI, CONV, 6, false>, hipFuncAttributeMaxDynamicSharedMemorySize, X3_LDS_ONE));
        attr_set = true;
    }
    const dim3 grid(per * 8), blk(256);
    const size_t lds = ((nprod == 6 && sched) || itts_opt(OPT_X3_PIN) == 0) ? X3_LDS : X3_LDS_ONE;
    if constexpr (!CONV && (EPI == EPI_QKV_ROPE || EPI == EPI_SWIGLU)) {
        if (a.a_planes) {
            if (nprod != 6 || !sched) { itts_set_error("gemm (f32x3): the plane-operand form exists for the shipped variant only (6 products, interleaved)"); return ITTS_ERR_ARG; }
            static ItPerDevice<bool> apl_set_pd;
            bool& apl_set = apl_set_pd.cur();
            if (!apl_set) {
                HIP_TRY(hipFuncSetAttribute((const void*)gemm_x3_kernel<EPI, CONV, 6, true, true>, hipFuncAttributeMaxDynamicSharedMemorySize, X3_LDS_ONE));
                apl_set = true;
            }
            hipLaunchKernelGGL((gemm_x3_kernel<EPI, CONV, 6, true, true>), grid, blk, lds, st, a);
            HIP_TRY(hipGetLastError());
            return ITTS_OK;
        }
    } else if (a.a_planes) { itts_set_error("gemm (f32x3): plane operands are supported for the wqkv / SwiGLU GEMMs only"); return ITTS_ERR_ARG; }
    if (nprod == 6 && sched && itts_opt(OPT_X3_WAVES) == 8 && itts_opt(OPT_X3_PIN) == 0) {
        static ItPerDevice<bool> w8_set_pd;
        bool& w8_set = w8_set_pd.cur();
        if (!w8_set) {
            HIP_TRY(hipFuncSetAttribute((const void*)gemm_x3w8_kernel<EPI, CONV>, hipFuncAttributeMaxDynamicSharedMemorySize, X3W8_LDS));
            w8_set = true;
        }
        hipLaunchKernelGGL((gemm_x3w8_kernel<EPI, CONV>), grid, dim3(512), X3W8_LDS, st, a);
        HIP_TRY(hipGetLastError());
        return ITTS_OK;
    }
    if (nprod == 6 && sched) hipLaunchKernelGGL((gemm_x3_kernel<EPI, CONV, 6, true>), grid, blk, lds, st, a);
    else if (nprod == 6) hipLaunchKernelGGL((gemm_x3_kernel<EPI, CONV, 6, false>), grid, blk, lds, st, a);
    else if (sched) hipLaunchKernelGGL((gemm_x3_kernel<EPI, CONV, 8, true>), grid, blk, lds, st, a);
    else hipLaunchKernelGGL((gemm_x3_kernel<EPI, CONV, 8, false>), grid, blk, lds, st, a);
    HIP_TRY(hipGetLastError());
    return ITTS_OK;
}

int launch_gemm_x3(const GemmArgs& a, hipStream_t st) {
    if (!pf_f32_ok(a)) {
        itts_set_error("gemm (f32x3): needs K %% 32 == 0, lda %% 4 == 0, N / ldo / D %% 4 == 0, 16-byte aligned rows, no split-K (M=%d N=%d K=%d lda=%d epi=%d)",
                       a.M, a.N, a.K, a.lda, a.epi);
        return ITTS_ERR_ARG;
    }
    if (a.epi == EPI_GATE && a.conv_taps > 0 &&
        (a.conv_W % 32 || a.K != a.conv_taps * a.conv_W || a.lda != a.conv_W || !a.tok_seq || !a.tok_t || !a.seq_start || !a.seq_T || !a.zero_row)) {
        itts_set_error("gemm tap mode (f32x3): need conv_W %% 32 == 0, K == taps * conv_W, lda == conv_W and the sequence tables");
        return ITTS_ERR_ARG;
    }
    switch (a.epi) {
        case EPI_STORE_F32: return launch_gemm_x3_e<EPI_STORE_F32>(a, st);
        case EPI_RESIDUAL: return launch_gemm_x3_e<EPI_RESIDUAL>(a, st);
        case EPI_SWIGLU: return launch_gemm_x3_e<EPI_SWIGLU>(a, st);
        case EPI_GATE: return a.conv_taps > 0 ? launch_gemm_x3_e<EPI_GATE, true>(a, st) : launch_gemm_x3_e<EPI_GATE>(a, st);
        case EPI_QKV_ROPE: return launch_gemm_x3_e<EPI_QKV_ROPE>(a, st);
        case EPI_WN_RS: return launch_gemm_x3_e<EPI_WN_RS>(a, st);
        default: itts_set_error("gemm (f32x3): unsupported epilogue %d", a.epi); return ITTS_ERR_ARG;
    }
}


int gemm_x3_occupancy(int* blocks) {
    int n = 0;
    (void)hipFuncSetAttribute((const void*)gemm_x3_kernel<EPI_RESIDUAL, false, 6, true>, hipFuncAttributeMaxDynamicSharedMemorySize, X3_LDS);
    const hipError_t e = hipOccupancyMaxActiveBlocksPerMultiprocessor(&n, (const void*)gemm_x3_kernel<EPI_RESIDUAL, false, 6, true>, 256, X3_LDS);
    if (e != hipSuccess) { itts_set_error("occupancy query: %s", hipGetErrorString(e)); return ITTS_ERR_HIP; }
    *blocks = n;
    return ITTS_OK;
}
```

indextts_amd/csrc/gpt_kernels.h:

```cpp
#pragma once
#include "common.h"

enum { PREC_F32 = 0, PREC_BF16 = 1,
       PREC_F32X3 = 2 };

struct LnArgs {
    float* x;
    const float* partial;
    int nsplit;
    const float* bias_prev;
    const float* g1; const float* b1;
    const float* g2; const float* b2;
    void* out;
    int out_f32;
    int rows, D;
    int in_row_mul, in_row_add;
    float eps;
};
int launch_ln(const LnArgs& a, int prec, hipStream_t st);

enum { EPI_STORE_F32 = 0, EPI_GELU_ACT = 1, EPI_PARTIAL = 2, EPI_RESIDUAL = 3, EPI_QKV = 4,
       EPI_SWIGLU = 5,
       EPI_GATE = 6,
       EPI_QKV_ROPE = 7,
       EPI_WN_RS = 8 };
struct GemmArgs {
    const void* A; int lda;
    const void* Wp;
    const float* bias;
    int M, N, K;
    int nsplit;
    int epi;
    float* out_f32; int ldo;
    void* out_act;
    float* partial;
    float* qbuf; void* kcache; void* vcache;
    const int* pos_ptr; int S, H, Tmax, D;
    const int* pos_shift;
    size_t a_planes;
    int kb_slice;
    int dma_rot;
    const float* ln_x; float* ln_x_out; const float* ln_partial; const float* ln_bias_prev; const float* ln_g; const float* ln_b; float ln_eps;
    const int* tok_seq; const int* tok_t; const int* seq_len; const float* rope; const float* gvec;
    float* out2; int wn_first, wn_last;
    int conv_taps, conv_dil, conv_W;
    const int* seq_start; const int* seq_T; const void* zero_row;
    void* out_act2;
    int seq_mul;
    const int* seq_map;
    size_t kv_planes;
};
int launch_gemm(const GemmArgs& a, int prec, bool prefill, hipStream_t st);
int launch_gemm_x3(const GemmArgs& a, hipStream_t st);
int gemm_x3_occupancy(int* blocks);
bool gemm_decode_ln_ok(int M, int K, int epi);
int launch_gemm_decode_ln(const GemmArgs& a, hipStream_t st);
int gemm_tile_occupancy(int prec, int* blocks);

struct AttnArgs {
    const float* qbuf;
    const void* kcache; const void* vcache;
    const int* pad;
    const int* row_map;
    const int* row_map_alt;
    const int* step_ptr;
    const int* pos_ptr;
    const int* pos_shift;
    void* out;
    int nseq, H, nq, Tmax, D;
    int seq_mul;
    const int* seq_map;
};
int launch_attention(const AttnArgs& a, int prec, hipStream_t st);

struct SampleArgs {
    const float* logits;
    unsigned char* seen;
    unsigned char* finished;
    long long* tokens;
    const int* step_ptr;
    const double* uniforms;
    unsigned long long seed;
    int B, V, max_new;
    int do_sample, top_k, min_keep;
    float top_p, temperature, rep_penalty;
    float typical_mass;
    int stop_token;
    const float* mel_emb; const float* mel_pos; float* x_next; int D; int pos_offset; int n_mel_pos;
    int* adv_state;
    const unsigned long long* seed_ptr;
    const int* row_slot; int uniforms_stride;
    int radix_select;
    unsigned long long* stamps;
    const int* row_limit;
    const int* row_step0;
};
int launch_sample(const SampleArgs& a, hipStream_t st);
int launch_advance(int* step_ptr, int* pos_ptr, hipStream_t st);

#define BEAM_MAX 4
struct BeamHyp { float score; int step; int row; int pad; };
struct BeamArgs {
    const float* logits;
    unsigned char* seen[2];
    int* row_map[2];
    float* beam_scores;
    float* next_scores; int* next_tokens; int* next_indices;
    int* surv_idx; float* surv_val; int* surv_n;
    BeamHyp* hyps;
    int* n_hyps;
    float* worst;
    unsigned char* done;
    int* hist_tok; int* hist_par;
    const int* step_ptr;
    int logits_shared;
    const double* uniforms;
    unsigned long long seed;
    int B, nb, V, max_new, Tmax, S;
    int do_sample, top_k, min_keep;
    float top_p, temperature, rep_penalty, length_penalty;
    float typical_mass;
    int stop_token;
    const float* mel_emb; const float* mel_pos; float* x_next; int D; int pos_offset; int n_mel_pos;
    int* adv_state;
    const unsigned long long* seed_ptr;
    int radix_select;
    const int* row_step0;
    const int* row_shift;
    const int* grp_cap;
    const int* grp_map;
    int n_grp;
};
int launch_beam_step(const BeamArgs& a, hipStream_t st);
int launch_beam_apply(const BeamArgs& a, hipStream_t st);
```

indextts_amd/csrc/options.hip:

```cpp
#include <atomic>
#include <stdlib.h>
#include <string.h>

#include "../../include/indextts_hip.h"
#include "common.h"

namespace {
struct OptDef {
    const char* name;
    int def, lo, hi;
    const char* doc;
    const char* allowed = nullptr;
};
const OptDef kDefs[OPT_COUNT] = {
    {"decode_fuse_ln", 1, 0, 2, "GPT decode: LayerNorm (+ split-K reduce, bias, residual) inside the consuming GEMM -- 1: steps of 1-8 rows (measured faster), 2: up to 16 rows (measured slower above 8, kept for the A/B record), 0: separate ln_kernel launches; bitwise equal"},
    {"decode_gemm", 1, 0, 1, "bf16 decode GEMMs on the LDS-DMA slab kernel (0: register-path gemm_kernel; bitwise equal)"},
    {"decode_rot", 1, 0, 1, "per-block rotation of the slab DMA issue order in the decode GEMM (same bytes, same LDS image)"},
    {"decode_wnt", 0, 0, 1, "non-temporal policy on the decode GEMM's weight stream"},
    {"decode_nt", 0, 0, 4, "force the n-tiles per block of the 64-row decode GEMM (0: smallest that fits one round of blocks)", "0,1,2,4"},
    {"prefill_gemm", 1, 0, 1, "bf16 prefill GEMMs on the LDS-DMA tile kernels (0: register-path gemm_kernel; bitwise equal)"},
    {"tile256", -1, -1, 2, "bf16 tile GEMM: -1 pick by shape, 0 always 128x128, 1 always 256x256, 2 always 256x128 (bitwise equal)"},
    {"f32_tile", 1, 0, 1, "f32 GEMMs with plain epilogues on the f32-MFMA tile kernel (0: register-path kernel; bitwise equal)"},
    {"x3_products", 6, 6, 8, "plane products per f32 product of the fp32x3 GEMMs and attention: 6 (hh, hm, mh, hl, lh, mm; drops m*l and l*m, 2^-24 |ab| each: measured error vs f64 <= the native f32-MFMA kernels' on every benchmarked shape) or 8 (every term down to 2^-24 |ab|; two blocks per CU like the default since the packed-RoPE fix -- option x3_pin = 1 restores round 4's one-block pin as a diagnostic)", "6,8"},
    {"x3_sched", 1, 0, 1, "fp32x3 GEMM: interleave the operand split with the MFMAs (0: split as a burst; bitwise equal)"},
    {"x3_attn", 1, 0, 1, "fp32x3 s2mel: attention products on bf16 planes too (K / V^T written as three planes by the wqkv epilogue, flash_attn_x3_kernel); 0: the f32-MFMA flash kernel"},
    {"sample_radix", -1, -1, 1, "top-k threshold: -1 per-kernel default (radix select in sample_kernel, ballot bisection in the beam kernels), 0 bisection, 1 radix select (identical ids)"},
    {"gpt_compact", 1, 0, 1, "row compaction of ragged decode batches (0 disables it for every handle; identical ids)"},
    {"attn_waves", 0, 0, 16, "waves per block of the KV-cache attention kernel: 0 pick by shape, else 4 / 8 / 16 (the 16 canonical key streams are mapped onto them; bitwise equal)", "0,4,8,16"},
    {"s2mel_fused", 1, 0, 2, "s2mel: fused GEMM epilogues, sampled when a handle is created -- 1: fused, 0: separate element-wise kernels (2: round 4's spelling of 'the bf16 wqkv epilogue fused too'; the same as 1 since the RoPE fix of round 5)"},
    {"fa_qs", 0, 0, 4, "bf16 flash attention: query sub-tiles per wave (0: pick by shape)", "0,1,2,4"},
    {"f32_attn_scalar", 0, 0, 1, "f32 s2mel attention on the one-wave-per-query reference kernel (the A/B path of the f32 flash kernel)"},
    {"fa32_qs", 2, 1, 2, "f32 flash attention: query sub-tiles per wave"},
    {"aa_act", 2, 0, 2, "anti-aliased activation kernel variant (2: swizzled LDS tiles)"},
    {"conv_bm", 0, 0, 128, "force the co-tile height of conv_mfma_kernel (0: pick by channel count)", "0,32,64,96,128"},
    {"h3_kernel", 1, 0, 1, "f16x3 vocoder conv: 1 window kernel, 0 two-stage kernel"},
    {"decode_ln_nt", 2, 2, 4, "LayerNorm-fused decode GEMM at 5-16 rows (weights on waves 0-3, LayerNorm on waves 4-7): n-tiles per block, 2 or 4 (bitwise equal)", "2,4"},
    {"x3_aplanes", 0, 0, 1, "fp32x3 s2mel: the adaptive-RMSNorm outputs as three bf16 planes in fragment order, wqkv / w1|w3 GEMMs without an operand split (bitwise equal)"},
    {"x3_pin", 0, 0, 1, "fp32x3 GEMM: 1 pins the variants that are not the default one (8 products, burst split) to one block per CU -- round 4's workaround for their run-to-run differences, kept as a diagnostic; not needed since the RoPE fix of round 5 (DESIGN.md section 9)"},
    {"prefill_attn", -1, -1, 1, "attention of S > 1 passes (prefill, latent pass): -1 causal MFMA kernel in the bf16 mode, canonical-stream kernel in the f32 parity mode; 0 canonical-stream kernel (one block per query) always; 1 MFMA kernel in both precisions"},
    {"voc_act_planes", 1, 0, 1, "vocoder, bf16x3 conv mode: the anti-aliased activation in front of an x3 conv writes the conv's three operand planes itself (aa_act_planes_kernel); 0: f32 activation + split pass (bit-identical planes)"},
    {"x3_waves", 8, 4, 8, "fp32x3 GEMM: waves per 128 x 128 block -- 8 (4 x 2, wave tile 32 x 64, weights through LDS: four waves per SIMD at two blocks per CU; 64-utterance solve 314.7 vs 323.0 ms per Euler step, profiles/r06k) or 4 (2 x 2, wave tile 64 x 64, weights in registers: round 5's kernel); bitwise equal", "4,8"},
};
std::atomic<int> g_val[OPT_COUNT];
std::atomic<unsigned> g_epoch{1};
std::atomic<bool> g_init{false};

void ensure_init() {
    if (g_init.load(std::memory_order_acquire)) return;
    static std::atomic_flag once = ATOMIC_FLAG_INIT;
    if (!once.test_and_set()) {
        for (int i = 0; i < OPT_COUNT; ++i) g_val[i].store(kDefs[i].def, std::memory_order_relaxed);
        g_init.store(true, std::memory_order_release);
    } else {
        while (!g_init.load(std::memory_order_acquire)) {}
    }
}
int find(const char* name) {
    if (!name) return -1;
    for (int i = 0; i < OPT_COUNT; ++i)
        if (strcmp(kDefs[i].name, name) == 0) return i;
    return -1;
}
}

int itts_opt(int id) {
    ensure_init();
    return g_val[id].load(std::memory_order_relaxed);
}
unsigned itts_opt_epoch() { return g_epoch.load(std::memory_order_relaxed); }

extern "C" int itts_set_option(const char* name, int value) {
    ensure_init();
    const int i = find(name);
    if (i < 0) { itts_set_error("set_option: unknown option '%s'", name ? name : "(null)"); return ITTS_ERR_ARG; }
    if (value < kDefs[i].lo || value > kDefs[i].hi) {
        itts_set_error("set_option: %s = %d outside [%d, %d]", name, value, kDefs[i].lo, kDefs[i].hi);
        return ITTS_ERR_ARG;
    }
    if (kDefs[i].allowed) {
        bool ok = false;
        for (const char* p = kDefs[i].allowed; *p;) {
            char* end;
            const long v = strtol(p, &end, 10);
            ok |= v == value;
            p = *end == ',' ? end + 1 : end;
        }
        if (!ok) { itts_set_error("set_option: %s = %d is not one of {%s}", name, value, kDefs[i].allowed); return ITTS_ERR_ARG; }
    }
    if (g_val[i].exchange(value) != value) g_epoch.fetch_add(1);
    return ITTS_OK;
}
extern "C" int itts_get_option(const char* name, int* value) {
    ensure_init();
    const int i = find(name);
    if (i < 0 || !value) { itts_set_error("get_option: unknown option '%s'", name ? name : "(null)"); return ITTS_ERR_ARG; }
    *value = g_val[i].load();
    return ITTS_OK;
}
extern "C" int itts_reset_options(void) {
    ensure_init();
    bool changed = false;
    for (int i = 0; i < OPT_COUNT; ++i) changed |= g_val[i].exchange(kDefs[i].def) != kDefs[i].def;
    if (changed) g_epoch.fetch_add(1);
    return ITTS_OK;
}
extern "C" int itts_option_count(void) { return OPT_COUNT; }
extern "C" const char* itts_option_name(int index) { return (index >= 0 && index < OPT_COUNT) ? kDefs[index].name : nullptr; }
extern "C" const char* itts_option_doc(int index) { return (index >= 0 && index < OPT_COUNT) ? kDefs[index].doc : nullptr; }
extern "C" int itts_option_default(int index) { return (index >= 0 && index < OPT_COUNT) ? kDefs[index].def : 0; }
```

indextts_amd/csrc/s2mel_kernels.h:

```cpp
#pragma once
#include "common.h"

struct SeqTab {
    const int* tok_seq;
    const int* tok_t;
    const int* seq_start;
    const int* seq_T;
    const int* seq_len;
    int n_seq, n_tok, t_max;
};

int launch_ada_rmsnorm(const float* x, const float* g, const float* wb, void* out, int n_tok, int H, float eps, int prec, hipStream_t st,
                       const int* row_map = nullptr);
int launch_final_ln_mod(const float* wn_out, const float* rp, const float* mod, void* out, const SeqTab& tab, int W, int prec, hipStream_t st);
int launch_cast_pad(const float* in, void* out, int rows, int src_rows, int C_in, int C_out, int prec, hipStream_t st, const int* row_map = nullptr);
int launch_rope_split(const float* qkv, const float* rope, void* q, void* k, void* v, const SeqTab& tab, int heads, int t_pad, int prec, hipStream_t st);
int launch_s2mel_attention(const void* q, const void* k, const void* v, void* out, const SeqTab& tab, int heads, int t_pad, int prec, hipStream_t st);
int launch_s2mel_attention_x3(const void* q, const void* kp, const void* vp, void* out, const SeqTab& tab, int heads, int t_pad, hipStream_t st);
int launch_split_planes(const float* in, void* out, size_t n, hipStream_t st);
int launch_ada_rmsnorm_planes(const float* x, const float* g, const float* wb, void* out, size_t plane_stride, int n_tok, int H, float eps, hipStream_t st);
int launch_trace_hash(const void* p, size_t bytes, unsigned long long* out, hipStream_t st);
int launch_swiglu(const float* in, void* out, int n_tok, int I, int prec, hipStream_t st);
int launch_im2col_reflect(const float* x, void* col, const SeqTab& tab, int W, int k, int dilation, int prec, hipStream_t st);
int launch_wn_gate(const float* in, const float* g, void* out, int n_tok, int W, int prec, hipStream_t st);
int launch_wn_update(const float* rs, float* x, float* out, const SeqTab& tab, int W, int first, int last, hipStream_t st);
int launch_euler_update(float* xs, const float* d, const SeqTab& tab, const int* prompt_len, int C, int n_branch, float dt, float cfg_rate, hipStream_t st,
                        const int* tail_base = nullptr, int tail_half = 0);
```

indextts_amd/csrc/s2mel_kernels.hip:

```cpp
#include <stdlib.h>
#include <type_traits>
#include "s2mel_kernels.h"
#include "gpt_kernels.h"

typedef __bf16 bf16x8_t __attribute__((ext_vector_type(8)));
typedef unsigned int v4u __attribute__((ext_vector_type(4)));
typedef unsigned int v2u __attribute__((ext_vector_type(2)));

typedef __bf16 bf16x2_t __attribute__((ext_vector_type(2)));
typedef float f32x2_t __attribute__((ext_vector_type(2)));
__device__ __forceinline__ uint32_t pack_bf16x2(float a, float b) {
    return __builtin_bit_cast(uint32_t, __builtin_convertvector(f32x2_t{a, b}, bf16x2_t));
}

template <bool BF16>
__device__ __forceinline__ void store_act4(void* base, size_t idx, f32x4 v) {
    if constexpr (BF16) {
        v2u pk{pack_bf16x2(v[0], v[1]), pack_bf16x2(v[2], v[3])};
        *(v2u*)((u16*)base + idx) = pk;
    } else {
        *(f32x4*)((float*)base + idx) = v;
    }
}

template <bool BF16>
__global__ __launch_bounds__(256) void ada_rmsnorm_kernel(const float* __restrict__ x, const float* __restrict__ g,
                                                          const float* __restrict__ wb, void* __restrict__ out, int n, int H, float eps,
                                                          const int* __restrict__ row_map) {
    const int lane = threadIdx.x & 63, w = threadIdx.x >> 6;
    const int m = blockIdx.x * 4 + w;
    if (m >= n) return;
    const float* xr = x + (size_t)(row_map ? row_map[m] : m) * H;
    float ss = 0.f;
    for (int c = lane * 4; c < H; c += 256) {
        const f32x4 v = *(const f32x4*)(xr + c);
        ss += (v[0] * v[0] + v[1] * v[1]) + (v[2] * v[2] + v[3] * v[3]);
    }
    ss = wave_sum(ss);
    const float rstd = 1.0f / sqrtf(ss / (float)H + eps);
    for (int c = lane * 4; c < H; c += 256) {
        const f32x4 v = *(const f32x4*)(xr + c), gg = *(const f32x4*)(g + c), ww = *(const f32x4*)(wb + c), bb = *(const f32x4*)(wb + H + c);
        f32x4 o;
#pragma unroll
        for (int j = 0; j < 4; ++j) o[j] = ww[j] * ((v[j] * rstd) * gg[j]) + bb[j];
        store_act4<BF16>(out, (size_t)m * H + c, o);
    }
}

__global__ __launch_bounds__(256) void ada_rmsnorm_planes_kernel(const float* __restrict__ x, const float* __restrict__ g, const float* __restrict__ wb,
                                                                 u16* __restrict__ out, size_t stride, int n, int H, float eps) {
    const int lane = threadIdx.x & 63, w = threadIdx.x >> 6;
    const int m = blockIdx.x * 4 + w;
    if (m >= n) return;
    const float* xr = x + (size_t)m * H;
    float ss = 0.f;
    for (int c = lane * 4; c < H; c += 256) {
        const f32x4 v = *(const f32x4*)(xr + c);
        ss += (v[0] * v[0] + v[1] * v[1]) + (v[2] * v[2] + v[3] * v[3]);
    }
    ss = wave_sum(ss);
    const float rstd = 1.0f / sqrtf(ss / (float)H + eps);
    for (int c = lane * 4; c < H; c += 256) {
        const f32x4 v = *(const f32x4*)(xr + c), gg = *(const f32x4*)(g + c), ww = *(const f32x4*)(wb + c), bb = *(const f32x4*)(wb + H + c);
        f32x4 o;
#pragma unroll
        for (int j = 0; j < 4; ++j) o[j] = ww[j] * ((v[j] * rstd) * gg[j]) + bb[j];
        v2u hh, mm, ll;
#pragma unroll
        for (int i = 0; i < 2; ++i) {
            const float a0 = o[2 * i], a1 = o[2 * i + 1];
            const uint32_t h = pack_bf16x2(a0, a1);
            const float r0 = a0 - __uint_as_float(h << 16), r1 = a1 - __uint_as_float(h & 0xffff0000u);
            const uint32_t mi = pack_bf16x2(r0, r1);
            const float s0 = r0 - __uint_as_float(mi << 16), s1 = r1 - __uint_as_float(mi & 0xffff0000u);
            hh[i] = h; mm[i] = mi; ll[i] = pack_bf16x2(s0, s1);
        }
        const int q = c & 31;
        u16* dst = out + (size_t)m * H + (c & ~31) + (((q & 15) >> 2) << 3) + ((q >> 4) << 2);
        *(v2u*)dst = hh;
        *(v2u*)(dst + stride) = mm;
        *(v2u*)(dst + 2 * stride) = ll;
    }
}

int launch_ada_rmsnorm_planes(const float* x, const float* g, const float* wb, void* out, size_t plane_stride, int n_tok, int H, float eps, hipStream_t st) {
    if (n_tok <= 0) return ITTS_OK;
    if (H % 32 || plane_stride % 8) { itts_set_error("ada_rmsnorm_planes: hidden size %d must be a multiple of 32 and the plane stride of 8", H); return ITTS_ERR_ARG; }
    hipLaunchKernelGGL(ada_rmsnorm_planes_kernel, dim3(ceil_div(n_tok, 4)), dim3(256), 0, st, x, g, wb, (u16*)out, plane_stride, n_tok, H, eps);
    HIP_TRY(hipGetLastError());
    return ITTS_OK;
}

int launch_ada_rmsnorm(const float* x, const float* g, const float* wb, void* out, int n_tok, int H, float eps, int prec, hipStream_t st,
                       const int* row_map) {
    if (n_tok <= 0) return ITTS_OK;
    if (H % 4) { itts_set_error("ada_rmsnorm: hidden size %d must be a multiple of 4", H); return ITTS_ERR_ARG; }
    const dim3 grid(ceil_div(n_tok, 4));
    if (prec == PREC_BF16) hipLaunchKernelGGL(ada_rmsnorm_kernel<true>, grid, dim3(256), 0, st, x, g, wb, out, n_tok, H, eps, row_map);
    else hipLaunchKernelGGL(ada_rmsnorm_kernel<false>, grid, dim3(256), 0, st, x, g, wb, out, n_tok, H, eps, row_map);
    HIP_TRY(hipGetLastError());
    return ITTS_OK;
}

template <bool BF16>
__global__ __launch_bounds__(256) void final_ln_mod_kernel(const float* __restrict__ wn, const float* __restrict__ rp,
                                                           const float* __restrict__ mod, void* __restrict__ out, SeqTab tab, int W) {
    const int lane = threadIdx.x & 63, w = threadIdx.x >> 6;
    const int m = blockIdx.x * 4 + w;
    if (m >= tab.n_tok) return;
    const float mask = tab.tok_t[m] < tab.seq_len[tab.tok_seq[m]] ? 1.f : 0.f;
    const float* a = wn + (size_t)m * W;
    const float* b = rp + (size_t)m * W;
    float s = 0.f;
    for (int c = lane * 4; c < W; c += 256) {
        const f32x4 va = *(const f32x4*)(a + c), vb = *(const f32x4*)(b + c);
#pragma unroll
        for (int j = 0; j < 4; ++j) s += va[j] * mask + vb[j];
    }
    const float mean = wave_sum(s) / (float)W;
    float q = 0.f;
    for (int c = lane * 4; c < W; c += 256) {
        const f32x4 va = *(const f32x4*)(a + c), vb = *(const f32x4*)(b + c);
#pragma unroll
        for (int j = 0; j < 4; ++j) { const float d = (va[j] * mask + vb[j]) - mean; q += d * d; }
    }
    const float rstd = 1.0f / sqrtf(wave_sum(q) / (float)W + 1e-6f);
    for (int c = lane * 4; c < W; c += 256) {
        const f32x4 va = *(const f32x4*)(a + c), vb = *(const f32x4*)(b + c), sh = *(const f32x4*)(mod + c), sc = *(const f32x4*)(mod + W + c);
        f32x4 o;
#pragma unroll
        for (int j = 0; j < 4; ++j) o[j] = (((va[j] * mask + vb[j]) - mean) * rstd) * (1.0f + sc[j]) + sh[j];
        store_act4<BF16>(out, (size_t)m * W + c, o);
    }
}

int launch_final_ln_mod(const float* wn_out, const float* rp, const float* mod, void* out, const SeqTab& tab, int W, int prec, hipStream_t st) {
    if (tab.n_tok <= 0) return ITTS_OK;
    if (W % 4) { itts_set_error("final_ln: width %d must be a multiple of 4", W); return ITTS_ERR_ARG; }
    const dim3 grid(ceil_div(tab.n_tok, 4));
    if (prec == PREC_BF16) hipLaunchKernelGGL(final_ln_mod_kernel<true>, grid, dim3(256), 0, st, wn_out, rp, mod, out, tab, W);
    else hipLaunchKernelGGL(final_ln_mod_kernel<false>, grid, dim3(256), 0, st, wn_out, rp, mod, out, tab, W);
    HIP_TRY(hipGetLastError());
    return ITTS_OK;
}

template <bool BF16>
__global__ __launch_bounds__(256) void cast_pad_kernel(const float* __restrict__ in, void* __restrict__ out, int rows, int src_rows,
                                                       int C_in, int C_out, const int* __restrict__ row_map) {
    const int c4n = C_out >> 2;
    const size_t total = (size_t)rows * c4n;
    for (size_t i = (size_t)blockIdx.x * 256 + threadIdx.x; i < total; i += (size_t)gridDim.x * 256) {
        const int m = (int)(i / c4n), c = (int)(i - (size_t)m * c4n) * 4;
        const float* r = in + (size_t)((row_map ? row_map[m] : m) % src_rows) * C_in;
        f32x4 v;
#pragma unroll
        for (int j = 0; j < 4; ++j) v[j] = (c + j) < C_in ? r[c + j] : 0.f;
        store_act4<BF16>(out, (size_t)m * C_out + c, v);
    }
}

int launch_cast_pad(const float* in, void* out, int rows, int src_rows, int C_in, int C_out, int prec, hipStream_t st, const int* row_map) {
    if (rows <= 0) return ITTS_OK;
    if (C_out % 4 || C_out < C_in) { itts_set_error("cast_pad: C_out=%d must be a multiple of 4 and >= C_in=%d", C_out, C_in); return ITTS_ERR_ARG; }
    const size_t total = (size_t)rows * (C_out >> 2);
    const unsigned grid = (unsigned)((total + 255) / 256 < 65536 * 8 ? (total + 255) / 256 : 65536 * 8);
    if (prec == PREC_BF16) hipLaunchKernelGGL(cast_pad_kernel<true>, dim3(grid), dim3(256), 0, st, in, out, rows, src_rows, C_in, C_out, row_map);
    else hipLaunchKernelGGL(cast_pad_kernel<false>, dim3(grid), dim3(256), 0, st, in, out, rows, src_rows, C_in, C_out, row_map);
    HIP_TRY(hipGetLastError());
    return ITTS_OK;
}

template <bool BF16>
__global__ __launch_bounds__(256) void rope_split_kernel(const float* __restrict__ qkv, const float* __restrict__ rope,
                                                         void* __restrict__ q, void* __restrict__ k, void* __restrict__ v, SeqTab tab,
                                                         int heads, int t_pad) {
    const int s = blockIdx.y, t0 = blockIdx.x * 4;
    const int T = tab.seq_T[s];
    if (t0 >= T) return;
    const int H = heads * 64, tid = threadIdx.x;
    const int m0 = tab.seq_start[s] + t0;
    const int nt = (T - t0) < 4 ? (T - t0) : 4;
    for (int tt = 0; tt < nt; ++tt) {
        const float* row = qkv + (size_t)(m0 + tt) * 3 * H;
        const int t = t0 + tt;
        for (int p = tid; p < H; p += 256) {
            const int which = p >= (H >> 1);
            const int pp = which ? p - (H >> 1) : p;
            const int h = pp >> 5, i = pp & 31, c = h * 64 + 2 * i;
            const float x0 = row[which * H + c], x1 = row[which * H + c + 1];
            const float cs = rope[((size_t)t * 32 + i) * 2], sn = rope[((size_t)t * 32 + i) * 2 + 1];
            const float y0 = x0 * cs - x1 * sn, y1 = x1 * cs + x0 * sn;
            const size_t o = which ? (((size_t)(s * heads + h) * t_pad + t) * 64 + 2 * i) : ((size_t)(m0 + tt) * H + c);
            void* dst = which ? k : q;
            if constexpr (BF16) *(uint32_t*)((u16*)dst + o) = pack_bf16x2(y0, y1);
            else { ((float*)dst)[o] = y0; ((float*)dst)[o + 1] = y1; }
        }
    }
    for (int c = tid; c < H; c += 256) {
        const int h = c >> 6, d = c & 63;
        float val[4];
#pragma unroll
        for (int tt = 0; tt < 4; ++tt) val[tt] = tt < nt ? qkv[(size_t)(m0 + tt) * 3 * H + 2 * H + c] : 0.f;
        if constexpr (BF16) {
            const v2u pk{pack_bf16x2(val[0], val[1]), pack_bf16x2(val[2], val[3])};
            *(v2u*)((u16*)v + ((size_t)(s * heads + h) * 64 + d) * t_pad + t0) = pk;
        } else {
            *(f32x4*)((float*)v + ((size_t)(s * heads + h) * 64 + d) * t_pad + t0) = f32x4{val[0], val[1], val[2], val[3]};
        }
    }
}

int launch_rope_split(const float* qkv, const float* rope, void* q, void* k, void* v, const SeqTab& tab, int heads, int t_pad, int prec,
                      hipStream_t st) {
    if (tab.n_tok <= 0) return ITTS_OK;
    if (t_pad % 64 || t_pad < tab.t_max) { itts_set_error("rope_split: t_pad=%d must be a multiple of 64 and >= %d", t_pad, tab.t_max); return ITTS_ERR_ARG; }
    const dim3 grid(ceil_div(tab.t_max, 4), tab.n_seq);
    if (prec == PREC_BF16) hipLaunchKernelGGL(rope_split_kernel<true>, grid, dim3(256), 0, st, qkv, rope, q, k, v, tab, heads, t_pad);
    else hipLaunchKernelGGL(rope_split_kernel<false>, grid, dim3(256), 0, st, qkv, rope, q, k, v, tab, heads, t_pad);
    HIP_TRY(hipGetLastError());
    return ITTS_OK;
}

__global__ __launch_bounds__(64) void attn_f32_kernel(const float* __restrict__ Q, const float* __restrict__ K, const float* __restrict__ V,
                                                      float* __restrict__ O, SeqTab tab, int heads, int t_pad) {
    const int m = blockIdx.x, h = blockIdx.y, lane = threadIdx.x;
    const int s = tab.tok_seq[m], len = tab.seq_len[s];
    const int H = heads * 64, sub = lane & 15, grp = lane >> 4;
    const f32x4 q = *(const f32x4*)(Q + (size_t)m * H + h * 64 + sub * 4);
    const float* Kb = K + ((size_t)(s * heads + h) * t_pad) * 64;
    const float* Vb = V + ((size_t)(s * heads + h) * 64) * t_pad;
    float m_run = -INFINITY, l_run = 0.f;
    f32x4 acc{0.f, 0.f, 0.f, 0.f};
    for (int t0 = 0; t0 < len; t0 += 4) {
        const int t = t0 + grp;
        const bool ok = t < len;
        const int tc = ok ? t : len - 1;
        const f32x4 kf = *(const f32x4*)(Kb + (size_t)tc * 64 + sub * 4);
        const f32x4 vf{Vb[(size_t)(sub * 4 + 0) * t_pad + tc], Vb[(size_t)(sub * 4 + 1) * t_pad + tc], Vb[(size_t)(sub * 4 + 2) * t_pad + tc],
                       Vb[(size_t)(sub * 4 + 3) * t_pad + tc]};
        float sc = (q[0] * kf[0] + q[1] * kf[1]) + (q[2] * kf[2] + q[3] * kf[3]);
#pragma unroll
        for (int o = 1; o < 16; o <<= 1) sc += __shfl_xor(sc, o, 64);
        sc *= 0.125f;
        if (ok) {
            const float nm = fmaxf(m_run, sc);
            const float al = expf(m_run - nm), p = expf(sc - nm);
            l_run = l_run * al + p;
#pragma unroll
            for (int j = 0; j < 4; ++j) acc[j] = acc[j] * al + p * vf[j];
            m_run = nm;
        }
    }
#pragma unroll
    for (int o = 16; o < 64; o <<= 1) {
        const float om = __shfl_xor(m_run, o, 64), ol = __shfl_xor(l_run, o, 64);
        const float nm = fmaxf(m_run, om);
        const float sa = (m_run == -INFINITY) ? 0.f : expf(m_run - nm), sb = (om == -INFINITY) ? 0.f : expf(om - nm);
        l_run = l_run * sa + ol * sb;
#pragma unroll
        for (int j = 0; j < 4; ++j) acc[j] = acc[j] * sa + __shfl_xor(acc[j], o, 64) * sb;
        m_run = nm;
    }
    if (lane < 16) {
        f32x4 r;
#pragma unroll
        for (int j = 0; j < 4; ++j) r[j] = l_run > 0.f ? acc[j] / l_run : 0.f;
        *(f32x4*)(O + (size_t)m * H + h * 64 + sub * 4) = r;
    }
}

#define FA_LD 64

__device__ __forceinline__ float fa_colmax(float x) {
    float a = x, b = x;
    asm volatile("s_nop 1\n\tv_permlane16_swap_b32 %0, %1\n\ts_nop 1\n\tv_max_f32 %0, %0, %1\n\tv_mov_b32 %1, %0\n\ts_nop 1\n\t"
                 "v_permlane32_swap_b32 %0, %1\n\ts_nop 1\n\tv_max_f32 %0, %0, %1"
                 : "+v"(a), "+v"(b));
    return a;
}
__device__ __forceinline__ float fa_max3(float a, float b, float c) { return __builtin_fmaxf(__builtin_fmaxf(a, b), c); }

template <int QS>
__global__ __launch_bounds__(256, (QS == 1 ? 4 : QS == 2 ? 2 : 1)) void flash_attn_bf16_kernel(const u16* __restrict__ Q, const u16* __restrict__ K, const u16* __restrict__ Vt,
                                                              u16* __restrict__ O, SeqTab tab, int heads, int t_pad, float scale_log2e) {
    __shared__ __attribute__((aligned(16))) u16 ks[2][64 * FA_LD];
    __shared__ __attribute__((aligned(16))) u16 vs[2][64 * FA_LD];
    const int s = blockIdx.z, h = blockIdx.y, q0 = blockIdx.x * (64 * QS);
    const int T = tab.seq_T[s], len = tab.seq_len[s];
    if (q0 >= T) return;
    const int H = heads * 64;
    const int tid = threadIdx.x, lane = tid & 63, w = tid >> 6;
    const int g = lane >> 4, c16 = lane & 15;
    const size_t row0 = (size_t)tab.seq_start[s];
    v4u qf[QS][2];
#pragma unroll
    for (int qs = 0; qs < QS; ++qs) {
        int qi = q0 + (w * QS + qs) * 16 + c16;
        qi = qi < T ? qi : T - 1;
        const u16* qrow = Q + (row0 + qi) * H + h * 64;
        qf[qs][0] = *(const v4u*)(qrow + g * 8);
        qf[qs][1] = *(const v4u*)(qrow + 32 + g * 8);
    }
    const u16* Kb = K + ((size_t)(s * heads + h) * t_pad) * 64;
    const u16* Vb = Vt + ((size_t)(s * heads + h) * 64) * t_pad;
    const int r0 = tid >> 3, p0 = tid & 7;
    v4u kreg[2], vreg[2];
    auto fetch = [&](int k0) {
#pragma unroll
        for (int i = 0; i < 2; ++i) {
            const int r = r0 + 32 * i;
            kreg[i] = *(const v4u*)(Kb + (size_t)(k0 + r) * 64 + p0 * 8);
            vreg[i] = *(const v4u*)(Vb + (size_t)r * t_pad + k0 + p0 * 8);
        }
    };
    auto stage = [&](int buf) {
#pragma unroll
        for (int i = 0; i < 2; ++i) {
            const int r = r0 + 32 * i;
            const int pk = (p0 ^ (((r >> 1) & 1) | (((r >> 3) & 3) << 1))) * 8;
            const int pv = (p0 ^ ((r >> 1) & 7)) * 8;
            *(v4u*)(ks[buf] + r * FA_LD + pk) = kreg[i];
            *(v4u*)(vs[buf] + r * FA_LD + pv) = vreg[i];
        }
    };
    const int krow = 8 * (c16 >> 2) + (c16 & 3);
    const int ksw = ((c16 >> 1) & 1) | ((c16 >> 2) << 1), vsw = (c16 >> 1) & 7;
    int k_off[2], v_off[2];
#pragma unroll
    for (int kx = 0; kx < 2; ++kx) {
        k_off[kx] = krow * FA_LD + (((kx * 4 + g) ^ ksw) << 3);
        v_off[kx] = c16 * FA_LD + (((kx * 4 + g) ^ vsw) << 3);
    }
    f32x4 o[QS][4], osum[QS];
    float m_run[QS];
#pragma unroll
    for (int qs = 0; qs < QS; ++qs) {
        m_run[qs] = -INFINITY;
        osum[qs] = f32x4{0.f, 0.f, 0.f, 0.f};
#pragma unroll
        for (int mt = 0; mt < 4; ++mt) o[qs][mt] = f32x4{0.f, 0.f, 0.f, 0.f};
    }
    const unsigned one2 = c16 == 0 ? 0x3f803f80u : 0u;
    const v4u ones_frag{one2, one2, one2, one2};
    fetch(0);
    stage(0);
    __syncthreads();
#pragma unroll
    for (int qs = 0; qs < QS; ++qs) {
        asm volatile("" : "+v"(qf[qs][0]));
        asm volatile("" : "+v"(qf[qs][1]));
    }
    auto tile = [&](auto bufc, int k0) {
        const int BUF = bufc;
        const bool more = k0 + 64 < len;
        if (more) fetch(k0 + 64);
        const u16* kt_s = ks[BUF];
        const u16* vt_s = vs[BUF];
        f32x4 st[QS][4];
#pragma unroll
        for (int kx = 0; kx < 2; ++kx)
#pragma unroll
            for (int kt = 0; kt < 4; ++kt) {
                const v4u a = *(const v4u*)(kt_s + (32 * (kt >> 1) + 4 * (kt & 1)) * FA_LD + k_off[kx]);
#pragma unroll
                for (int qs = 0; qs < QS; ++qs)
                    st[qs][kt] = __builtin_amdgcn_mfma_f32_16x16x32_bf16(__builtin_bit_cast(bf16x8_t, a), __builtin_bit_cast(bf16x8_t, qf[qs][kx]),
                                                                         kx == 0 ? f32x4{0.f, 0.f, 0.f, 0.f} : st[qs][kt], 0, 0, 0);
            }
        const bool tail = k0 + 64 > len;
        v4u pb[QS][2];
#pragma unroll
        for (int qs = 0; qs < QS; ++qs) {
            if (tail) {
#pragma unroll
                for (int kt = 0; kt < 4; ++kt)
#pragma unroll
                    for (int r = 0; r < 4; ++r)
                        if ((k0 + 32 * (kt >> 1) + 8 * g + 4 * (kt & 1) + r) >= len) st[qs][kt][r] = -INFINITY;
            }
            const float t0 = fa_max3(st[qs][0][0], st[qs][0][1], st[qs][0][2]), t1 = fa_max3(st[qs][1][0], st[qs][1][1], st[qs][1][2]);
            const float t2 = fa_max3(st[qs][2][0], st[qs][2][1], st[qs][2][2]), t3 = fa_max3(st[qs][3][0], st[qs][3][1], st[qs][3][2]);
            const float u0 = fa_max3(t0, t1, st[qs][0][3]), u1 = fa_max3(t2, t3, st[qs][1][3]);
            const float m_new = fa_colmax(fa_max3(u0, u1, fa_max3(st[qs][2][3], st[qs][3][3], m_run[qs])));
            if (__builtin_amdgcn_ballot_w64(m_new > m_run[qs]) != 0) {
                const float alpha = __builtin_amdgcn_exp2f((m_run[qs] - m_new) * scale_log2e);
#pragma unroll
                for (int mt = 0; mt < 4; ++mt)
#pragma unroll
                    for (int r = 0; r < 4; ++r) o[qs][mt][r] *= alpha;
                osum[qs][0] *= alpha;
                m_run[qs] = m_new;
            }
            const float off = -m_new * scale_log2e;
#pragma unroll
            for (int kt = 0; kt < 4; ++kt)
#pragma unroll
                for (int r = 0; r < 4; ++r) st[qs][kt][r] = __builtin_amdgcn_exp2f(__builtin_fmaf(st[qs][kt][r], scale_log2e, off));
#pragma unroll
            for (int kx = 0; kx < 2; ++kx)
                pb[qs][kx] = v4u{pack_bf16x2(st[qs][2 * kx][0], st[qs][2 * kx][1]), pack_bf16x2(st[qs][2 * kx][2], st[qs][2 * kx][3]),
                                 pack_bf16x2(st[qs][2 * kx + 1][0], st[qs][2 * kx + 1][1]), pack_bf16x2(st[qs][2 * kx + 1][2], st[qs][2 * kx + 1][3])};
        }
#pragma unroll
        for (int kx = 0; kx < 2; ++kx) {
#pragma unroll
            for (int mt = 0; mt < 4; ++mt) {
                const v4u a = *(const v4u*)(vt_s + mt * 16 * FA_LD + v_off[kx]);
#pragma unroll
                for (int qs = 0; qs < QS; ++qs)
                    o[qs][mt] = __builtin_amdgcn_mfma_f32_16x16x32_bf16(__builtin_bit_cast(bf16x8_t, a), __builtin_bit_cast(bf16x8_t, pb[qs][kx]),
                                                                        o[qs][mt], 0, 0, 0);
            }
#pragma unroll
            for (int qs = 0; qs < QS; ++qs)
                osum[qs] = __builtin_amdgcn_mfma_f32_16x16x32_bf16(__builtin_bit_cast(bf16x8_t, ones_frag), __builtin_bit_cast(bf16x8_t, pb[qs][kx]),
                                                                   osum[qs], 0, 0, 0);
        }
        if (more) stage(BUF ^ 1);
        __syncthreads();
    };
    for (int k0 = 0; k0 < len; k0 += 128) {
        tile(std::integral_constant<int, 0>{}, k0);
        if (k0 + 64 >= len) break;
        tile(std::integral_constant<int, 1>{}, k0 + 64);
    }
#pragma unroll
    for (int qs = 0; qs < QS; ++qs) {
        const float ls = __shfl(osum[qs][0], c16, 64);
        const int qi = q0 + (w * QS + qs) * 16 + c16;
        if (qi < T) {
            const float inv = ls > 0.f ? 1.0f / ls : 0.f;
            u16* orow = O + (row0 + qi) * H + h * 64;
#pragma unroll
            for (int mt = 0; mt < 4; ++mt) {
                const v2u pk{pack_bf16x2(o[qs][mt][0] * inv, o[qs][mt][1] * inv), pack_bf16x2(o[qs][mt][2] * inv, o[qs][mt][3] * inv)};
                *(v2u*)(orow + mt * 16 + g * 4) = pk;
            }
        }
    }
}

#define FA32_STAGE 32768
#define FA32_LDS (2 * FA32_STAGE)
template <int QS>
__global__ __launch_bounds__(256, 2) void flash_attn_f32_kernel(const float* __restrict__ Q, const float* __restrict__ K, const float* __restrict__ Vt,
                                                                float* __restrict__ O, SeqTab tab, int heads, int t_pad, float scale_log2e) {
    extern __shared__ __attribute__((aligned(16))) char fa32_sm[];
    const int s = blockIdx.z, h = blockIdx.y, q0 = blockIdx.x * (64 * QS);
    const int T = tab.seq_T[s], len = tab.seq_len[s];
    if (q0 >= T) return;
    const int H = heads * 64;
    const int tid = threadIdx.x, lane = tid & 63, w = tid >> 6;
    const int g = lane >> 4, c16 = lane & 15;
    const size_t row0 = (size_t)tab.seq_start[s];
    int qi[QS];
    bool q_ok[QS];
    f32x4 qf[QS][4];
#pragma unroll
    for (int qs = 0; qs < QS; ++qs) {
        qi[qs] = q0 + (w * QS + qs) * 16 + c16;
        q_ok[qs] = qi[qs] < T;
        qi[qs] = q_ok[qs] ? qi[qs] : T - 1;
        const float* qrow = Q + (row0 + qi[qs]) * H + h * 64 + g * 4;
#pragma unroll
        for (int ks = 0; ks < 4; ++ks) qf[qs][ks] = *(const f32x4*)(qrow + ks * 16);
    }
    const float* Kb = K + ((size_t)(s * heads + h) * t_pad) * 64;
    const float* Vb = Vt + ((size_t)(s * heads + h) * 64) * t_pad;
    const float* ksrc[4];
    const float* vsrc[4];
#pragma unroll
    for (int i = 0; i < 4; ++i) {
        const int r = 16 * w + 4 * i + g;
        const int piece = c16 ^ (r & 15);
        ksrc[i] = Kb + (size_t)r * 64 + piece * 4;
        vsrc[i] = Vb + (size_t)r * t_pad + piece * 4;
    }
    auto issue = [&](int k0, int buf) {
        char* base = fa32_sm + buf * FA32_STAGE;
#pragma unroll
        for (int i = 0; i < 4; ++i) {
            __builtin_amdgcn_global_load_lds((const __attribute__((address_space(1))) void*)(ksrc[i] + (size_t)k0 * 64),
                                             (__attribute__((address_space(3))) void*)(base + (w * 4 + i) * 1024), 16, 0, 0);
            __builtin_amdgcn_global_load_lds((const __attribute__((address_space(1))) void*)(vsrc[i] + k0),
                                             (__attribute__((address_space(3))) void*)(base + 16384 + (w * 4 + i) * 1024), 16, 0, 0);
        }
    };
    int f_off[4];
#pragma unroll
    for (int y = 0; y < 4; ++y) f_off[y] = c16 * 256 + (((4 * y + g) ^ c16) << 4);
    f32x4 o[QS][4];
    float m_run[QS], l_run[QS];
#pragma unroll
    for (int qs = 0; qs < QS; ++qs) {
        m_run[qs] = -INFINITY;
        l_run[qs] = 0.f;
#pragma unroll
        for (int dt = 0; dt < 4; ++dt) o[qs][dt] = f32x4{0.f, 0.f, 0.f, 0.f};
    }
    issue(0, 0);
    int it = 0;
    for (int k0 = 0; k0 < len; k0 += 64, ++it) {
        asm volatile("s_waitcnt vmcnt(0)" ::: "memory");
        __syncthreads();
        if (k0 + 64 < len) issue(k0 + 64, (it + 1) & 1);
        const char* kt_s = fa32_sm + (it & 1) * FA32_STAGE;
        const char* vt_s = kt_s + 16384;
        f32x4 st[QS][4];
#pragma unroll
        for (int qs = 0; qs < QS; ++qs)
#pragma unroll
            for (int kt = 0; kt < 4; ++kt) st[qs][kt] = f32x4{0.f, 0.f, 0.f, 0.f};
#pragma unroll
        for (int ks = 0; ks < 4; ++ks) {
            f32x4 a[4];
#pragma unroll
            for (int kt = 0; kt < 4; ++kt) a[kt] = *(const f32x4*)(kt_s + kt * 4096 + f_off[ks]);
#pragma unroll
            for (int j = 0; j < 4; ++j)
#pragma unroll
                for (int qs = 0; qs < QS; ++qs)
#pragma unroll
                    for (int kt = 0; kt < 4; ++kt)
                        st[qs][kt] = __builtin_amdgcn_mfma_f32_16x16x4f32(a[kt][j], qf[qs][ks][j], st[qs][kt], 0, 0, 0);
        }
        const bool tail = k0 + 64 > len;
#pragma unroll
        for (int qs = 0; qs < QS; ++qs) {
            if (tail) {
#pragma unroll
                for (int kt = 0; kt < 4; ++kt)
#pragma unroll
                    for (int r = 0; r < 4; ++r)
                        if (k0 + 16 * kt + 4 * g + r >= len) st[qs][kt][r] = -INFINITY;
            }
            const float t0 = fa_max3(st[qs][0][0], st[qs][0][1], st[qs][0][2]), t1 = fa_max3(st[qs][1][0], st[qs][1][1], st[qs][1][2]);
            const float t2 = fa_max3(st[qs][2][0], st[qs][2][1], st[qs][2][2]), t3 = fa_max3(st[qs][3][0], st[qs][3][1], st[qs][3][2]);
            const float u0 = fa_max3(t0, t1, st[qs][0][3]), u1 = fa_max3(t2, t3, st[qs][1][3]);
            const float m_new = fa_colmax(fa_max3(u0, u1, fa_max3(st[qs][2][3], st[qs][3][3], m_run[qs])));
            if (__builtin_amdgcn_ballot_w64(m_new > m_run[qs]) != 0) {
                const float alpha = __builtin_amdgcn_exp2f((m_run[qs] - m_new) * scale_log2e);
#pragma unroll
                for (int dt = 0; dt < 4; ++dt)
#pragma unroll
                    for (int r = 0; r < 4; ++r) o[qs][dt][r] *= alpha;
                l_run[qs] *= alpha;
                m_run[qs] = m_new;
            }
            const float off = -m_new * scale_log2e;
            float psum = 0.f;
#pragma unroll
            for (int kt = 0; kt < 4; ++kt)
#pragma unroll
                for (int r = 0; r < 4; ++r) {
                    const float p = __builtin_amdgcn_exp2f(__builtin_fmaf(st[qs][kt][r], scale_log2e, off));
                    st[qs][kt][r] = p;
                    psum += p;
                }
            l_run[qs] += psum;
        }
#pragma unroll
        for (int kt = 0; kt < 4; ++kt) {
            f32x4 a[4];
#pragma unroll
            for (int dt = 0; dt < 4; ++dt) a[dt] = *(const f32x4*)(vt_s + dt * 4096 + f_off[kt]);
#pragma unroll
            for (int j = 0; j < 4; ++j)
#pragma unroll
                for (int qs = 0; qs < QS; ++qs)
#pragma unroll
                    for (int dt = 0; dt < 4; ++dt)
                        o[qs][dt] = __builtin_amdgcn_mfma_f32_16x16x4f32(a[dt][j], st[qs][kt][j], o[qs][dt], 0, 0, 0);
        }
    }
#pragma unroll
    for (int qs = 0; qs < QS; ++qs) {
        float ls = l_run[qs];
        ls += __shfl_xor(ls, 16, 64);
        ls += __shfl_xor(ls, 32, 64);
        if (q_ok[qs]) {
            const float inv = ls > 0.f ? 1.0f / ls : 0.f;
            float* orow = O + (row0 + qi[qs]) * H + h * 64 + g * 4;
#pragma unroll
            for (int dt = 0; dt < 4; ++dt)
                *(f32x4*)(orow + dt * 16) = f32x4{o[qs][dt][0] * inv, o[qs][dt][1] * inv, o[qs][dt][2] * inv, o[qs][dt][3] * inv};
        }
    }
}

#define FX3_PLANE 8192
#define FX3_STAGE (6 * FX3_PLANE)
#define FX3_LDS (2 * FX3_STAGE)

__device__ __forceinline__ void fx3_split8(const f32x4 p0, const f32x4 p1, v4u& H, v4u& M, v4u& L) {
    const float x[8] = {p0[0], p0[1], p0[2], p0[3], p1[0], p1[1], p1[2], p1[3]};
#pragma unroll
    for (int i = 0; i < 4; ++i) {
        const float a = x[2 * i], b = x[2 * i + 1];
        const uint32_t h = pack_bf16x2(a, b);
        const float ra = a - __uint_as_float(h << 16), rb = b - __uint_as_float(h & 0xffff0000u);
        const uint32_t m = pack_bf16x2(ra, rb);
        const float sa = ra - __uint_as_float(m << 16), sb = rb - __uint_as_float(m & 0xffff0000u);
        H[i] = h; M[i] = m; L[i] = pack_bf16x2(sa, sb);
    }
}

template <int NPROD>
__global__ __launch_bounds__(512) void flash_attn_x3_kernel(const float* __restrict__ Q, const u16* __restrict__ Kp, const u16* __restrict__ Vp,
                                                            size_t pstride, float* __restrict__ O, SeqTab tab, int heads, int t_pad, float scale_log2e) {
    extern __shared__ __attribute__((aligned(16))) char fx3_sm[];
    const int s = blockIdx.z, h = blockIdx.y, q0 = blockIdx.x * 256;
    const int T = tab.seq_T[s], len = tab.seq_len[s];
    if (q0 >= T) return;
    const int H = heads * 64;
    const int tid = threadIdx.x, lane = tid & 63, w = __builtin_amdgcn_readfirstlane(tid >> 6);
    const int g = lane >> 4, c16 = lane & 15;
    const size_t row0 = (size_t)tab.seq_start[s];
    constexpr int PA[8] = {2, 1, 2, 0, 1, 1, 0, 0};
    constexpr int PB[8] = {1, 2, 0, 2, 1, 0, 1, 0};
    int qi[2];
    bool q_ok[2];
    v4u qp[2][3][2];
#pragma unroll
    for (int qs = 0; qs < 2; ++qs) {
        qi[qs] = q0 + (w * 2 + qs) * 16 + c16;
        q_ok[qs] = qi[qs] < T;
        qi[qs] = q_ok[qs] ? qi[qs] : T - 1;
        const float* qrow = Q + (row0 + qi[qs]) * H + h * 64 + g * 8;
#pragma unroll
        for (int kx = 0; kx < 2; ++kx) {
            const f32x4 p0 = *(const f32x4*)(qrow + 32 * kx), p1 = *(const f32x4*)(qrow + 32 * kx + 4);
            fx3_split8(p0, p1, qp[qs][0][kx], qp[qs][1][kx], qp[qs][2][kx]);
        }
    }
    const u16* Kb = Kp + ((size_t)(s * heads + h) * t_pad) * 64;
    const u16* Vb = Vp + ((size_t)(s * heads + h) * 64) * t_pad;
    const int rr = 8 * w + (lane >> 3), slot = lane & 7;
    const u16* ksrc = Kb + (size_t)rr * 64 + ((slot ^ (((rr >> 1) & 1) | (((rr >> 3) & 3) << 1))) << 3);
    const u16* vsrc = Vb + (size_t)rr * t_pad + ((slot ^ ((rr >> 1) & 7)) << 3);
    auto issue = [&](int k0, int buf) {
        char* base = fx3_sm + buf * FX3_STAGE + w * 1024;
#pragma unroll
        for (int p = 0; p < 3; ++p) {
            __builtin_amdgcn_global_load_lds((const __attribute__((address_space(1))) void*)(ksrc + p * pstride + (size_t)k0 * 64),
                                             (__attribute__((address_space(3))) void*)(base + p * FX3_PLANE), 16, 0, 0);
            __builtin_amdgcn_global_load_lds((const __attribute__((address_space(1))) void*)(vsrc + p * pstride + k0),
                                             (__attribute__((address_space(3))) void*)(base + (3 + p) * FX3_PLANE), 16, 0, 0);
        }
    };
    const int krow = 8 * (c16 >> 2) + (c16 & 3);
    const int ksw = ((c16 >> 1) & 1) | ((c16 >> 2) << 1), vsw = (c16 >> 1) & 7;
    int k_off[2], v_off[2];
#pragma unroll
    for (int kx = 0; kx < 2; ++kx) {
        k_off[kx] = (krow * 64 + (((kx * 4 + g) ^ ksw) << 3)) * 2;
        v_off[kx] = (c16 * 64 + (((kx * 4 + g) ^ vsw) << 3)) * 2;
    }
    f32x4 o[2][4];
    float m_run[2], l_run[2];
#pragma unroll
    for (int qs = 0; qs < 2; ++qs) {
        m_run[qs] = -INFINITY;
        l_run[qs] = 0.f;
#pragma unroll
        for (int mt = 0; mt < 4; ++mt) o[qs][mt] = f32x4{0.f, 0.f, 0.f, 0.f};
    }
    issue(0, 0);
    int it = 0;
    for (int k0 = 0; k0 < len; k0 += 64, ++it) {
        asm volatile("s_waitcnt vmcnt(0)" ::: "memory");
        __syncthreads();
        if (k0 + 64 < len) issue(k0 + 64, (it + 1) & 1);
        const char* kt_s = fx3_sm + (it & 1) * FX3_STAGE;
        const char* vt_s = kt_s + 3 * FX3_PLANE;
        f32x4 st[2][4];
#pragma unroll
        for (int qs = 0; qs < 2; ++qs)
#pragma unroll
            for (int kt = 0; kt < 4; ++kt) st[qs][kt] = f32x4{0.f, 0.f, 0.f, 0.f};
#pragma unroll
        for (int kx = 0; kx < 2; ++kx)
#pragma unroll
            for (int kp = 0; kp < 2; ++kp) {
                v4u ka[2][3];
#pragma unroll
                for (int j = 0; j < 2; ++j) {
                    const int kt = 2 * kp + j;
#pragma unroll
                    for (int p = 0; p < 3; ++p) ka[j][p] = *(const v4u*)(kt_s + p * FX3_PLANE + (32 * (kt >> 1) + 4 * (kt & 1)) * 128 + k_off[kx]);
                }
#pragma unroll
                for (int q = 8 - NPROD; q < 8; ++q)
#pragma unroll
                    for (int j = 0; j < 2; ++j)
#pragma unroll
                        for (int qs = 0; qs < 2; ++qs)
                            st[qs][2 * kp + j] = __builtin_amdgcn_mfma_f32_16x16x32_bf16(__builtin_bit_cast(bf16x8_t, ka[j][PA[q]]),
                                                                                         __builtin_bit_cast(bf16x8_t, qp[qs][PB[q]][kx]), st[qs][2 * kp + j], 0, 0, 0);
            }
        const bool tail = k0 + 64 > len;
        v4u pb[2][3][2];
#pragma unroll
        for (int qs = 0; qs < 2; ++qs) {
            if (tail) {
#pragma unroll
                for (int kt = 0; kt < 4; ++kt)
#pragma unroll
                    for (int r = 0; r < 4; ++r)
                        if ((k0 + 32 * (kt >> 1) + 8 * g + 4 * (kt & 1) + r) >= len) st[qs][kt][r] = -INFINITY;
            }
            const float t0 = fa_max3(st[qs][0][0], st[qs][0][1], st[qs][0][2]), t1 = fa_max3(st[qs][1][0], st[qs][1][1], st[qs][1][2]);
            const float t2 = fa_max3(st[qs][2][0], st[qs][2][1], st[qs][2][2]), t3 = fa_max3(st[qs][3][0], st[qs][3][1], st[qs][3][2]);
            const float u0 = fa_max3(t0, t1, st[qs][0][3]), u1 = fa_max3(t2, t3, st[qs][1][3]);
            const float m_new = fa_colmax(fa_max3(u0, u1, fa_max3(st[qs][2][3], st[qs][3][3], m_run[qs])));
            if (__builtin_amdgcn_ballot_w64(m_new > m_run[qs]) != 0) {
                const float alpha = __builtin_amdgcn_exp2f((m_run[qs] - m_new) * scale_log2e);
#pragma unroll
                for (int mt = 0; mt < 4; ++mt)
#pragma unroll
                    for (int r = 0; r < 4; ++r) o[qs][mt][r] *= alpha;
                l_run[qs] *= alpha;
                m_run[qs] = m_new;
            }
            const float off = -m_new * scale_log2e;
            float psum = 0.f;
#pragma unroll
            for (int kt = 0; kt < 4; ++kt)
#pragma unroll
                for (int r = 0; r < 4; ++r) {
                    const float p = __builtin_amdgcn_exp2f(__builtin_fmaf(st[qs][kt][r], scale_log2e, off));
                    st[qs][kt][r] = p;
                    psum += p;
                }
            l_run[qs] += psum;
#pragma unroll
            for (int kx = 0; kx < 2; ++kx) fx3_split8(st[qs][2 * kx], st[qs][2 * kx + 1], pb[qs][0][kx], pb[qs][1][kx], pb[qs][2][kx]);
        }
#pragma unroll
        for (int kx = 0; kx < 2; ++kx)
#pragma unroll
            for (int mp = 0; mp < 2; ++mp) {
                v4u va[2][3];
#pragma unroll
                for (int j = 0; j < 2; ++j)
#pragma unroll
                    for (int p = 0; p < 3; ++p) va[j][p] = *(const v4u*)(vt_s + p * FX3_PLANE + (2 * mp + j) * 2048 + v_off[kx]);
#pragma unroll
                for (int q = 8 - NPROD; q < 8; ++q)
#pragma unroll
                    for (int j = 0; j < 2; ++j)
#pragma unroll
                        for (int qs = 0; qs < 2; ++qs)
                            o[qs][2 * mp + j] = __builtin_amdgcn_mfma_f32_16x16x32_bf16(__builtin_bit_cast(bf16x8_t, va[j][PA[q]]),
                                                                                        __builtin_bit_cast(bf16x8_t, pb[qs][PB[q]][kx]), o[qs][2 * mp + j], 0, 0, 0);
            }
    }
#pragma unroll
    for (int qs = 0; qs < 2; ++qs) {
        float ls = l_run[qs];
        ls += __shfl_xor(ls, 16, 64);
        ls += __shfl_xor(ls, 32, 64);
        if (q_ok[qs]) {
            const float inv = ls > 0.f ? 1.0f / ls : 0.f;
            float* orow = O + (row0 + qi[qs]) * H + h * 64 + g * 4;
#pragma unroll
            for (int mt = 0; mt < 4; ++mt)
                *(f32x4*)(orow + mt * 16) = f32x4{o[qs][mt][0] * inv, o[qs][mt][1] * inv, o[qs][mt][2] * inv, o[qs][mt][3] * inv};
        }
    }
}

__global__ __launch_bounds__(256) void trace_hash_kernel(const uint32_t* __restrict__ p, size_t n_words, unsigned long long* __restrict__ out) {
    unsigned long long acc = 0;
    for (size_t i = (size_t)blockIdx.x * 256 + threadIdx.x; i < n_words; i += (size_t)gridDim.x * 256)
        acc += (unsigned long long)p[i] * (2 * (unsigned long long)i + 0x9E3779B97F4A7C15ull | 1ull);
#pragma unroll
    for (int o = 32; o > 0; o >>= 1) acc += __shfl_xor(acc, o, 64);
    if ((threadIdx.x & 63) == 0 && acc) atomicAdd(out, acc);
}
int launch_trace_hash(const void* p, size_t bytes, unsigned long long* out, hipStream_t st) {
    const size_t n = bytes / 4;
    if (!n) return ITTS_OK;
    const unsigned blocks = (unsigned)((n + 256 * 16 - 1) / (256 * 16) < 2048 ? (n + 256 * 16 - 1) / (256 * 16) : 2048);
    hipLaunchKernelGGL(trace_hash_kernel, dim3(blocks ? blocks : 1), dim3(256), 0, st, (const uint32_t*)p, n, out);
    HIP_TRY(hipGetLastError());
    return ITTS_OK;
}

__global__ __launch_bounds__(256) void split_planes_kernel(const float* __restrict__ in, u16* __restrict__ out, size_t n) {
    const size_t i = ((size_t)blockIdx.x * 256 + threadIdx.x) * 2;
    if (i >= n) return;
    const float a = in[i], b = in[i + 1];
    const uint32_t h = pack_bf16x2(a, b);
    const float ra = a - __uint_as_float(h << 16), rb = b - __uint_as_float(h & 0xffff0000u);
    const uint32_t m = pack_bf16x2(ra, rb);
    const float sa = ra - __uint_as_float(m << 16), sb = rb - __uint_as_float(m & 0xffff0000u);
    *(uint32_t*)(out + i) = h;
    *(uint32_t*)(out + n + i) = m;
    *(uint32_t*)(out + 2 * n + i) = pack_bf16x2(sa, sb);
}
int launch_split_planes(const float* in, void* out, size_t n, hipStream_t st) {
    if (n == 0) return ITTS_OK;
    if (n & 1) { itts_set_error("split_planes: n must be even"); return ITTS_ERR_ARG; }
    hipLaunchKernelGGL(split_planes_kernel, dim3((unsigned)((n / 2 + 255) / 256)), dim3(256), 0, st, in, (u16*)out, n);
    HIP_TRY(hipGetLastError());
    return ITTS_OK;
}

int launch_s2mel_attention_x3(const void* q, const void* kp, const void* vp, void* out, const SeqTab& tab, int heads, int t_pad, hipStream_t st) {
    if (tab.n_tok <= 0) return ITTS_OK;
    static ItPerDevice<bool> attr_set_pd;
    bool& attr_set = attr_set_pd.cur();
    if (!attr_set) {
        HIP_TRY(hipFuncSetAttribute((const void*)flash_attn_x3_kernel<8>, hipFuncAttributeMaxDynamicSharedMemorySize, FX3_LDS));
        HIP_TRY(hipFuncSetAttribute((const void*)flash_attn_x3_kernel<6>, hipFuncAttributeMaxDynamicSharedMemorySize, FX3_LDS));
        attr_set = true;
    }
    const float scale_log2e = 0.125f * 1.4426950408889634f;
    const size_t pstride = (size_t)tab.n_seq * heads * t_pad * 64;
    const dim3 grid(ceil_div(tab.t_max, 256), heads, tab.n_seq);
    if (itts_opt(OPT_X3_PRODUCTS) == 8)
        hipLaunchKernelGGL(flash_attn_x3_kernel<8>, grid, dim3(512), FX3_LDS, st, (const float*)q, (const u16*)kp, (const u16*)vp, pstride, (float*)out, tab, heads, t_pad, scale_log2e);
    else
        hipLaunchKernelGGL(flash_attn_x3_kernel<6>, grid, dim3(512), FX3_LDS, st, (const float*)q, (const u16*)kp, (const u16*)vp, pstride, (float*)out, tab, heads, t_pad, scale_log2e);
    HIP_TRY(hipGetLastError());
    return ITTS_OK;
}

int launch_s2mel_attention(const void* q, const void* k, const void* v, void* out, const SeqTab& tab, int heads, int t_pad, int prec,
                           hipStream_t st) {
    if (tab.n_tok <= 0) return ITTS_OK;
    if (prec == PREC_BF16) {
        const float scale_log2e = 0.125f * 1.4426950408889634f;
        const int force_qs = itts_opt(OPT_FA_QS);
        const int qs = force_qs ? force_qs : 2;
#define FA_LAUNCH(QS_) hipLaunchKernelGGL(flash_attn_bf16_kernel<QS_>, dim3(ceil_div(tab.t_max, 64 * QS_), heads, tab.n_seq), dim3(256), 0, st, \
                                          (const u16*)q, (const u16*)k, (const u16*)v, (u16*)out, tab, heads, t_pad, scale_log2e)
        if (qs >= 4) FA_LAUNCH(4); else if (qs == 2) FA_LAUNCH(2); else FA_LAUNCH(1);
#undef FA_LAUNCH
    } else {
        const bool scalar = itts_opt(OPT_F32_ATTN_SCALAR) != 0;
        if (scalar) {
            hipLaunchKernelGGL(attn_f32_kernel, dim3(tab.n_tok, heads), dim3(64), 0, st, (const float*)q, (const float*)k, (const float*)v, (float*)out, tab, heads, t_pad);
        } else {
            const int qs = itts_opt(OPT_FA32_QS) == 1 ? 1 : 2;
            static ItPerDevice<bool> attr_set_pd;
    bool& attr_set = attr_set_pd.cur();
            if (!attr_set) {
                HIP_TRY(hipFuncSetAttribute((const void*)flash_attn_f32_kernel<1>, hipFuncAttributeMaxDynamicSharedMemorySize, FA32_LDS));
                HIP_TRY(hipFuncSetAttribute((const void*)flash_attn_f32_kernel<2>, hipFuncAttributeMaxDynamicSharedMemorySize, FA32_LDS));
                attr_set = true;
            }
            const float scale_log2e = 0.125f * 1.4426950408889634f;
            if (qs == 2)
                hipLaunchKernelGGL(flash_attn_f32_kernel<2>, dim3(ceil_div(tab.t_max, 128), heads, tab.n_seq), dim3(256), FA32_LDS, st, (const float*)q,
                                   (const float*)k, (const float*)v, (float*)out, tab, heads, t_pad, scale_log2e);
            else
                hipLaunchKernelGGL(flash_attn_f32_kernel<1>, dim3(ceil_div(tab.t_max, 64), heads, tab.n_seq), dim3(256), FA32_LDS, st, (const float*)q,
                                   (const float*)k, (const float*)v, (float*)out, tab, heads, t_pad, scale_log2e);
        }
    }
    HIP_TRY(hipGetLastError());
    return ITTS_OK;
}

template <bool BF16>
__global__ __launch_bounds__(256) void swiglu_kernel(const float* __restrict__ in, void* __restrict__ out, int n, int I) {
    const int i4n = I >> 2;
    const size_t total = (size_t)n * i4n;
    for (size_t i = (size_t)blockIdx.x * 256 + threadIdx.x; i < total; i += (size_t)gridDim.x * 256) {
        const int m = (int)(i / i4n), c = (int)(i - (size_t)m * i4n) * 4;
        const f32x4 a = *(const f32x4*)(in + (size_t)m * 2 * I + c), b = *(const f32x4*)(in + (size_t)m * 2 * I + I + c);
        f32x4 o;
#pragma unroll
        for (int j = 0; j < 4; ++j) o[j] = (a[j] / (1.0f + expf(-a[j]))) * b[j];
        store_act4<BF16>(out, (size_t)m * I + c, o);
    }
}

int launch_swiglu(const float* in, void* out, int n_tok, int I, int prec, hipStream_t st) {
    if (n_tok <= 0) return ITTS_OK;
    if (I % 4) { itts_set_error("swiglu: width %d must be a multiple of 4", I); return ITTS_ERR_ARG; }
    const size_t total = (size_t)n_tok * (I >> 2);
    const unsigned grid = (unsigned)((total + 255) / 256 < 65536 * 8 ? (total + 255) / 256 : 65536 * 8);
    if (prec == PREC_BF16) hipLaunchKernelGGL(swiglu_kernel<true>, dim3(grid), dim3(256), 0, st, in, out, n_tok, I);
    else hipLaunchKernelGGL(swiglu_kernel<false>, dim3(grid), dim3(256), 0, st, in, out, n_tok, I);
    HIP_TRY(hipGetLastError());
    return ITTS_OK;
}

__device__ __forceinline__ int reflect_src(int p, int Tv) {
    if (p < 0) p = -p;
    if (p >= Tv) p = 2 * (Tv - 1) - p;
    return p;
}

template <bool BF16>
__global__ __launch_bounds__(256) void im2col_reflect_kernel(const float* __restrict__ x, void* __restrict__ col, SeqTab tab, int W, int k,
                                                             int dil) {
    const int w4n = W >> 2;
    const size_t total = (size_t)tab.n_tok * k * w4n;
    const int pad_total = (k - 1) * dil, right = pad_total / 2, left = pad_total - right;
    const int maxpad = left > right ? left : right;
    for (size_t i = (size_t)blockIdx.x * 256 + threadIdx.x; i < total; i += (size_t)gridDim.x * 256) {
        const int c = (int)(i % w4n) * 4;
        const size_t mj = i / w4n;
        const int j = (int)(mj % k), m = (int)(mj / k);
        const int s = tab.tok_seq[m], t = tab.tok_t[m], T = tab.seq_T[s];
        const int Tv = T <= maxpad ? maxpad + 1 : T;
        const int src = reflect_src(t + j * dil - left, Tv);
        f32x4 v{0.f, 0.f, 0.f, 0.f};
        if (src >= 0 && src < T) v = *(const f32x4*)(x + (size_t)(tab.seq_start[s] + src) * W + c);
        store_act4<BF16>(col, ((size_t)m * k + j) * W + c, v);
    }
}

int launch_im2col_reflect(const float* x, void* col, const SeqTab& tab, int W, int k, int dilation, int prec, hipStream_t st) {
    if (tab.n_tok <= 0) return ITTS_OK;
    if (W % 4 || k < 1 || dilation < 1) { itts_set_error("im2col: bad W=%d k=%d dilation=%d", W, k, dilation); return ITTS_ERR_ARG; }
    const size_t total = (size_t)tab.n_tok * k * (W >> 2);
    const unsigned grid = (unsigned)((total + 255) / 256 < 65536 * 8 ? (total + 255) / 256 : 65536 * 8);
    if (prec == PREC_BF16) hipLaunchKernelGGL(im2col_reflect_kernel<true>, dim3(grid), dim3(256), 0, st, x, col, tab, W, k, dilation);
    else hipLaunchKernelGGL(im2col_reflect_kernel<false>, dim3(grid), dim3(256), 0, st, x, col, tab, W, k, dilation);
    HIP_TRY(hipGetLastError());
    return ITTS_OK;
}

template <bool BF16>
__global__ __launch_bounds__(256) void wn_gate_kernel(const float* __restrict__ in, const float* __restrict__ gvec, void* __restrict__ out, int n, int W) {
    const int w4n = W >> 2;
    const size_t total = (size_t)n * w4n;
    for (size_t i = (size_t)blockIdx.x * 256 + threadIdx.x; i < total; i += (size_t)gridDim.x * 256) {
        const int m = (int)(i / w4n), c = (int)(i - (size_t)m * w4n) * 4;
        const f32x4 a = *(const f32x4*)(in + (size_t)m * 2 * W + c), b = *(const f32x4*)(in + (size_t)m * 2 * W + W + c);
        const f32x4 ga = *(const f32x4*)(gvec + c), gb = *(const f32x4*)(gvec + W + c);
        f32x4 o;
#pragma unroll
        for (int j = 0; j < 4; ++j) o[j] = tanhf(a[j] + ga[j]) * (1.0f / (1.0f + expf(-(b[j] + gb[j]))));
        store_act4<BF16>(out, (size_t)m * W + c, o);
    }
}

int launch_wn_gate(const float* in, const float* g, void* out, int n_tok, int W, int prec, hipStream_t st) {
    if (n_tok <= 0) return ITTS_OK;
    const size_t total = (size_t)n_tok * (W >> 2);
    const unsigned grid = (unsigned)((total + 255) / 256 < 65536 * 8 ? (total + 255) / 256 : 65536 * 8);
    if (prec == PREC_BF16) hipLaunchKernelGGL(wn_gate_kernel<true>, dim3(grid), dim3(256), 0, st, in, g, out, n_tok, W);
    else hipLaunchKernelGGL(wn_gate_kernel<false>, dim3(grid), dim3(256), 0, st, in, g, out, n_tok, W);
    HIP_TRY(hipGetLastError());
    return ITTS_OK;
}

__global__ __launch_bounds__(256) void wn_update_kernel(const float* __restrict__ rs, float* __restrict__ x, float* __restrict__ out, SeqTab tab,
                                                        int W, int first, int last) {
    const int w4n = W >> 2;
    const size_t total = (size_t)tab.n_tok * w4n;
    const int ld = last ? W : 2 * W;
    for (size_t i = (size_t)blockIdx.x * 256 + threadIdx.x; i < total; i += (size_t)gridDim.x * 256) {
        const int m = (int)(i / w4n), c = (int)(i - (size_t)m * w4n) * 4;
        const float* r = rs + (size_t)m * ld;
        f32x4 sk;
        if (!last) {
            const float mask = tab.tok_t[m] < tab.seq_len[tab.tok_seq[m]] ? 1.f : 0.f;
            const f32x4 res = *(const f32x4*)(r + c);
            f32x4 xv = *(const f32x4*)(x + (size_t)m * W + c);
#pragma unroll
            for (int j = 0; j < 4; ++j) xv[j] = (xv[j] + res[j]) * mask;
            *(f32x4*)(x + (size_t)m * W + c) = xv;
            sk = *(const f32x4*)(r + W + c);
        } else {
            sk = *(const f32x4*)(r + c);
        }
        if (!first) {
            const f32x4 ov = *(const f32x4*)(out + (size_t)m * W + c);
#pragma unroll
            for (int j = 0; j < 4; ++j) sk[j] += ov[j];
        }
        *(f32x4*)(out + (size_t)m * W + c) = sk;
    }
}

int launch_wn_update(const float* rs, float* x, float* out, const SeqTab& tab, int W, int first, int last, hipStream_t st) {
    if (tab.n_tok <= 0) return ITTS_OK;
    const size_t total = (size_t)tab.n_tok * (W >> 2);
    const unsigned grid = (unsigned)((total + 255) / 256 < 65536 * 8 ? (total + 255) / 256 : 65536 * 8);
    hipLaunchKernelGGL(wn_update_kernel, dim3(grid), dim3(256), 0, st, rs, x, out, tab, W, first, last);
    HIP_TRY(hipGetLastError());
    return ITTS_OK;
}

__global__ __launch_bounds__(256) void euler_update_kernel(float* __restrict__ xs, const float* __restrict__ d, SeqTab tab,
                                                           const int* __restrict__ prompt_len, int C, int n_branch, float dt, float cfg_rate,
                                                           const int* __restrict__ tail_base, int tail_half) {
    const int n_half = tab.n_tok / n_branch;
    const size_t total = (size_t)n_half * C;
    for (size_t i = (size_t)blockIdx.x * 256 + threadIdx.x; i < total; i += (size_t)gridDim.x * 256) {
        const int m = (int)(i / C);
        const int sq = tab.tok_seq[m], t = tab.tok_t[m];
        float v = 0.f;
        if (t >= prompt_len[sq]) {
            const size_t j = tail_base ? (size_t)(tail_base[sq] + t) * C + (i - (size_t)m * C) : i;
            float dphi = d[j];
            if (n_branch == 2) dphi = (1.0f + cfg_rate) * dphi - cfg_rate * d[j + (tail_base ? (size_t)tail_half * C : total)];
            v = xs[i] + dt * dphi;
        }
        xs[i] = v;
    }
}

int launch_euler_update(float* xs, const float* d, const SeqTab& tab, const int* prompt_len, int C, int n_branch, float dt, float cfg_rate,
                        hipStream_t st, const int* tail_base, int tail_half) {
    if (tab.n_tok <= 0) return ITTS_OK;
    const size_t total = (size_t)(tab.n_tok / n_branch) * C;
    const unsigned grid = (unsigned)((total + 255) / 256 < 65536 * 8 ? (total + 255) / 256 : 65536 * 8);
    hipLaunchKernelGGL(euler_update_kernel, dim3(grid), dim3(256), 0, st, xs, d, tab, prompt_len, C, n_branch, dt, cfg_rate, tail_base, tail_half);
    HIP_TRY(hipGetLastError());
    return ITTS_OK;
}
```

Measured before the change: 140.2.

## Prune last DiT layer to tail rows and skip masked attention tiles

In the fp32x3 s2mel estimator, the last DiT layer now computes attention queries, wo, the FFN norm and the FFN GEMMs only for the tail rows that the final projection consumes. The residual is gathered through a row map in a new EPI_RESIDUAL_SRC GEMM epilogue. The x_in GEMM reads its residual directly from const_in, which removes a device-to-device copy. Separately, the x3 flash attention kernel skips the MFMAs for the fully masked half of a short last key tile, and waves with no valid queries only stage K/V. This adds code complexity and depends on the tail-layout bookkeeping being correct.

```diff
diff --git a/indextts_amd/csrc/capi_s2mel.hip b/indextts_amd/csrc/capi_s2mel.hip
--- a/indextts_amd/csrc/capi_s2mel.hip
+++ b/indextts_amd/csrc/capi_s2mel.hip
@@ -430,15 +430,22 @@
     const bool x3_attn = prec == PREC_F32X3 && itts_opt(OPT_X3_ATTN) != 0;
     const size_t kv_plane = (size_t)tab.n_seq * nh * t_pad * 64;
     const bool a_planes = prec == PREC_F32X3 && fused && itts_opt(OPT_X3_APLANES) != 0 && itts_opt(OPT_X3_PRODUCTS) == 6 && itts_opt(OPT_X3_SCHED) != 0 && H % 32 == 0;
+    const bool prune_opt = prec == PREC_F32X3 && fused && itts_opt(OPT_S2MEL_PRUNE_LAST) != 0;
+    const bool prune_last = prune_opt && x3_attn && tail != nullptr && c.depth > 0;
     int rc;
     float *X = w.X, *X2 = w.X2;
     const size_t esz = prec == PREC_BF16 ? 2 : 4;
     const size_t kvb = kv_plane * (prec == PREC_F32X3 ? (x3_attn ? 6 : 4) : esz);
 #define S2_TRACE(label, ptr, bytes) do { if (h->trace && (rc = s2_trace(h, st, label, ptr, bytes))) return rc; } while (0)
     if ((rc = launch_cast_pad(x_src, w.XA, N, src_rows, C, Kx, prec, st))) return rc;
-    HIP_TRY(hipMemcpyAsync(X, const_in, (size_t)N * H * 4, hipMemcpyDeviceToDevice, st));
+    if (!prune_opt) HIP_TRY(hipMemcpyAsync(X, const_in, (size_t)N * H * 4, hipMemcpyDeviceToDevice, st));
     S2_TRACE("cast_pad(x) -> XA", w.XA, (size_t)N * Kx * esz);
-    if ((rc = s2_gemm(h, w.XA, Kx, h->w_x, nullptr, X, H, N, H, Kx, EPI_RESIDUAL, st))) return rc;
+    if (prune_opt) {
+        GemmArgs g{};
+        g.A = w.XA; g.lda = Kx; g.Wp = h->w_x; g.M = N; g.N = H; g.K = Kx; g.nsplit = 1; g.epi = EPI_RESIDUAL_SRC; g.out_f32 = X; g.ldo = H; g.D = H;
+        g.res_src = const_in;
+        if ((rc = s2_launch_gemm(h, g, st))) return rc;
+    } else if ((rc = s2_gemm(h, w.XA, Kx, h->w_x, nullptr, X, H, N, H, Kx, EPI_RESIDUAL, st))) return rc;
     S2_TRACE("x_in GEMM -> X", X, (size_t)N * H * 4);
     int n_skip = 0;
     for (int i = 0; i < c.depth; ++i) {
@@ -473,35 +480,43 @@
         S2_TRACE("wqkv -> Q", w.QA, (size_t)N * H * esz);
         S2_TRACE("wqkv -> K", w.KC, kvb);
         S2_TRACE("wqkv -> V^T", w.VC, kvb);
-        { S2Prof ps(h, st, S2_ATTN, attn_flops);
-          if (x3_attn) rc = launch_s2mel_attention_x3(w.QA, w.KC, w.VC, w.AO, tab, nh, t_pad, st);
+        const bool pruned = prune_last && i == c.depth - 1;
+        const int NL = pruned ? tail->n_tok : N;
+        { S2Prof ps(h, st, S2_ATTN, attn_flops * ((double)NL / (double)N));
+          if (x3_attn) rc = launch_s2mel_attention_x3(w.QA, w.KC, w.VC, w.AO, tab, nh, t_pad, st, pruned ? tail : nullptr);
           else rc = launch_s2mel_attention(w.QA, w.KC, w.VC, w.AO, tab, nh, t_pad, prec, st);
           if (rc) return rc; }
-        S2_TRACE("attention -> AO", w.AO, (size_t)N * H * esz);
-        if ((rc = s2_gemm(h, w.AO, H, L.w_o, nullptr, X, H, N, H, H, EPI_RESIDUAL, st))) return rc;
-        S2_TRACE("wo GEMM -> X", X, (size_t)N * H * 4);
+        S2_TRACE("attention -> AO", w.AO, (size_t)NL * H * esz);
+        if (pruned) {
+            GemmArgs g{};
+            g.A = w.AO; g.lda = H; g.Wp = L.w_o; g.M = NL; g.N = H; g.K = H; g.nsplit = 1; g.epi = EPI_RESIDUAL_SRC; g.out_f32 = X2; g.ldo = H; g.D = H;
+            g.res_src = X; g.res_map = tail_src;
+            if ((rc = s2_launch_gemm(h, g, st))) return rc;
+            float* tmp = X; X = X2; X2 = tmp;
+        } else if ((rc = s2_gemm(h, w.AO, H, L.w_o, nullptr, X, H, N, H, H, EPI_RESIDUAL, st))) return rc;
+        S2_TRACE("wo GEMM -> X", X, (size_t)NL * H * 4);
         if (a_planes) {
-            if ((rc = launch_ada_rmsnorm_planes(X, L.g_ffn, mods + (size_t)i * 4 * H + 2 * H, w.HBP, w.hbp_stride, N, H, c.norm_eps, st))) return rc;
+            if ((rc = launch_ada_rmsnorm_planes(X, L.g_ffn, mods + (size_t)i * 4 * H + 2 * H, w.HBP, w.hbp_stride, NL, H, c.norm_eps, st))) return rc;
             S2_TRACE("ada_rmsnorm(ffn) -> HB planes", w.HBP, w.hbp_stride * 6);
         } else {
-            if ((rc = launch_ada_rmsnorm(X, L.g_ffn, mods + (size_t)i * 4 * H + 2 * H, w.HB, N, H, c.norm_eps, prec, st))) return rc;
-            S2_TRACE("ada_rmsnorm(ffn) -> HB", w.HB, (size_t)N * H * esz);
+            if ((rc = launch_ada_rmsnorm(X, L.g_ffn, mods + (size_t)i * 4 * H + 2 * H, w.HB, NL, H, c.norm_eps, prec, st))) return rc;
+            S2_TRACE("ada_rmsnorm(ffn) -> HB", w.HB, (size_t)NL * H * esz);
         }
         if (fused) {
             GemmArgs g{};
-            g.A = w.HB; g.lda = H; g.Wp = L.w_13; g.M = N; g.N = 2 * I; g.K = H; g.nsplit = 1; g.epi = EPI_SWIGLU; g.out_act = w.FC; g.D = I;
+            g.A = w.HB; g.lda = H; g.Wp = L.w_13; g.M = NL; g.N = 2 * I; g.K = H; g.nsplit = 1; g.epi = EPI_SWIGLU; g.out_act = w.FC; g.D = I;
             if (a_planes) { g.A = w.HBP; g.a_planes = w.hbp_stride; }
             if ((rc = s2_launch_gemm(h, g, st))) return rc;
         } else {
-            if ((rc = s2_gemm(h, w.HB, H, L.w_13, nullptr, w.BIG, 2 * I, N, 2 * I, H, EPI_STORE_F32, st))) return rc;
-            if ((rc = launch_swiglu(w.BIG, w.FC, N, I, prec, st))) return rc;
+            if ((rc = s2_gemm(h, w.HB, H, L.w_13, nullptr, w.BIG, 2 * I, NL, 2 * I, H, EPI_STORE_F32, st))) return rc;
+            if ((rc = launch_swiglu(w.BIG, w.FC, NL, I, prec, st))) return rc;
         }
         void* shadow = nullptr;
         if (fused && i < c.depth / 2) shadow = w.SK + w.sk_stride * n_skip;
         else if (fused && i + 1 < c.depth && i + 1 > c.depth / 2) shadow = w.HB;
-        S2_TRACE("w13 + SwiGLU -> FC", w.FC, (size_t)N * I * esz);
-        if ((rc = s2_gemm(h, w.FC, I, L.w_2, nullptr, X, H, N, H, I, EPI_RESIDUAL, st, shadow))) return rc;
-        S2_TRACE("w2 GEMM -> X", X, (size_t)N * H * 4);
+        S2_TRACE("w13 + SwiGLU -> FC", w.FC, (size_t)NL * I * esz);
+        if ((rc = s2_gemm(h, w.FC, I, L.w_2, nullptr, X, H, NL, H, I, EPI_RESIDUAL, st, shadow))) return rc;
+        S2_TRACE("w2 GEMM -> X", X, (size_t)NL * H * 4);
         if (i < c.depth / 2) {
             if (!fused && (rc = launch_cast_pad(X, w.SK + w.sk_stride * n_skip, N, N, H, H, prec, st))) return rc;
             ++n_skip;
@@ -517,7 +532,7 @@
         XAt = w.QA;
     }
     const int NT = tt.n_tok;
-    if ((rc = launch_ada_rmsnorm(X, h->g_norm, m_norm, w.HB, NT, H, c.norm_eps, prec, st, tail ? tail_src : nullptr))) return rc;
+    if ((rc = launch_ada_rmsnorm(X, h->g_norm, m_norm, w.HB, NT, H, c.norm_eps, prec, st, tail && !prune_last ? tail_src : nullptr))) return rc;
     S2_TRACE("final ada_rmsnorm -> HB", w.HB, (size_t)NT * H * esz);
     if ((rc = s2_gemm(h, w.HB, H, h->w_sl_a, h->b_sl, X2, H, NT, H, H, EPI_STORE_F32, st))) return rc;
     if ((rc = s2_gemm(h, XAt, Kx, h->w_sl_b, nullptr, X2, H, NT, H, Kx, EPI_RESIDUAL, st, fused ? w.HB : nullptr))) return rc;
diff --git a/indextts_amd/csrc/common.h b/indextts_amd/csrc/common.h
--- a/indextts_amd/csrc/common.h
+++ b/indextts_amd/csrc/common.h
@@ -23,7 +23,7 @@
 
 enum { OPT_DECODE_FUSE_LN, OPT_DECODE_GEMM, OPT_DECODE_ROT, OPT_DECODE_WNT, OPT_DECODE_NT, OPT_PREFILL_GEMM, OPT_TILE256, OPT_F32_TILE,
        OPT_X3_PRODUCTS, OPT_X3_SCHED, OPT_X3_ATTN, OPT_SAMPLE_RADIX, OPT_GPT_COMPACT, OPT_ATTN_WAVES, OPT_S2MEL_FUSED, OPT_FA_QS,
-       OPT_F32_ATTN_SCALAR, OPT_FA32_QS, OPT_AA_ACT, OPT_CONV_BM, OPT_H3_KERNEL, OPT_DECODE_LN_NT, OPT_X3_APLANES, OPT_X3_PIN, OPT_PREFILL_ATTN, OPT_VOC_ACT_PLANES, OPT_X3_WAVES, OPT_COUNT };
+       OPT_F32_ATTN_SCALAR, OPT_FA32_QS, OPT_AA_ACT, OPT_CONV_BM, OPT_H3_KERNEL, OPT_DECODE_LN_NT, OPT_X3_APLANES, OPT_X3_PIN, OPT_PREFILL_ATTN, OPT_VOC_ACT_PLANES, OPT_X3_WAVES, OPT_S2MEL_PRUNE_LAST, OPT_X3_ATTN_SKIP, OPT_COUNT };
 int itts_opt(int id);
 unsigned itts_opt_epoch();
 
diff --git a/indextts_amd/csrc/gemm_tile.h b/indextts_amd/csrc/gemm_tile.h
--- a/indextts_amd/csrc/gemm_tile.h
+++ b/indextts_amd/csrc/gemm_tile.h
@@ -136,6 +136,12 @@
             const int sq = a.tok_seq[m], t = a.tok_t[m];
             if constexpr (EPI == EPI_QKV_ROPE) { meta[ltid] = sq; meta[ROWS + ltid] = t; }
             else meta[ltid] = (a.wn_last || t < a.seq_len[sq]) ? 1 : 0;
+        }
+    } else if constexpr (EPI == EPI_RESIDUAL_SRC) {
+        if (ltid < ROWS) {
+            int m = m0 + ltid;
+            m = m < a.M ? m : a.M - 1;
+            meta[ltid] = a.res_map ? a.res_map[m] : m;
         }
     }
 }
@@ -213,6 +219,12 @@
                 for (int q = 0; q < 4; ++q) v[q] += old[q];
                 *o = v;
                 if (a.out_act2) pf_store_act4<F32>(a.out_act2, (size_t)m * a.ldo + n, v);
+            } else if constexpr (EPI == EPI_RESIDUAL_SRC) {
+                const f32x4 old = *(const f32x4*)(a.res_src + (size_t)meta[row] * a.ldo + n);
+#pragma unroll
+                for (int q = 0; q < 4; ++q) v[q] += old[q];
+                *(f32x4*)(a.out_f32 + (size_t)m * a.ldo + n) = v;
+                if (a.out_act2) pf_store_act4<F32>(a.out_act2, (size_t)m * a.ldo + n, v);
             } else if constexpr (EPI == EPI_GELU_ACT) {
 #pragma unroll
                 for (int q = 0; q < 4; ++q) v[q] = gelu_new_f(v[q]);
@@ -350,7 +362,7 @@
 }
 
 static inline bool pf_vec_ok(const GemmArgs& a) {
-    return (a.N % 4 == 0) && (a.ldo % 4 == 0 || (a.epi != EPI_STORE_F32 && a.epi != EPI_RESIDUAL && a.epi != EPI_GELU_ACT)) && (a.D % 4 == 0);
+    return (a.N % 4 == 0) && (a.ldo % 4 == 0 || (a.epi != EPI_STORE_F32 && a.epi != EPI_RESIDUAL && a.epi != EPI_RESIDUAL_SRC && a.epi != EPI_GELU_ACT)) && (a.D % 4 == 0);
 }
 static inline bool pf_f32_ok(const GemmArgs& a) {
     return a.K % 32 == 0 && a.lda % 4 == 0 && a.nsplit == 1 && a.epi != EPI_PARTIAL && pf_vec_ok(a) && (((uintptr_t)a.A) & 15) == 0;
diff --git a/indextts_amd/csrc/gemm_x3.hip b/indextts_amd/csrc/gemm_x3.hip
--- a/indextts_amd/csrc/gemm_x3.hip
+++ b/indextts_amd/csrc/gemm_x3.hip
@@ -454,6 +454,9 @@
     switch (a.epi) {
         case EPI_STORE_F32: return launch_gemm_x3_e<EPI_STORE_F32>(a, st);
         case EPI_RESIDUAL: return launch_gemm_x3_e<EPI_RESIDUAL>(a, st);
+        case EPI_RESIDUAL_SRC:
+            if (!a.res_src || a.res_src == a.out_f32) { itts_set_error("gemm (f32x3): EPI_RESIDUAL_SRC needs a residual source other than the output"); return ITTS_ERR_ARG; }
+            return launch_gemm_x3_e<EPI_RESIDUAL_SRC>(a, st);
         case EPI_SWIGLU: return launch_gemm_x3_e<EPI_SWIGLU>(a, st);
         case EPI_GATE: return a.conv_taps > 0 ? launch_gemm_x3_e<EPI_GATE, true>(a, st) : launch_gemm_x3_e<EPI_GATE>(a, st);
         case EPI_QKV_ROPE: return launch_gemm_x3_e<EPI_QKV_ROPE>(a, st);
diff --git a/indextts_amd/csrc/gpt_kernels.h b/indextts_amd/csrc/gpt_kernels.h
--- a/indextts_amd/csrc/gpt_kernels.h
+++ b/indextts_amd/csrc/gpt_kernels.h
@@ -23,7 +23,8 @@
        EPI_SWIGLU = 5,
        EPI_GATE = 6,
        EPI_QKV_ROPE = 7,
-       EPI_WN_RS = 8 };
+       EPI_WN_RS = 8,
+       EPI_RESIDUAL_SRC = 9 };
 struct GemmArgs {
     const void* A; int lda;
     const void* Wp;
@@ -49,6 +50,8 @@
     int seq_mul;
     const int* seq_map;
     size_t kv_planes;
+    const float* res_src;
+    const int* res_map;
 };
 int launch_gemm(const GemmArgs& a, int prec, bool prefill, hipStream_t st);
 int launch_gemm_x3(const GemmArgs& a, hipStream_t st);
diff --git a/indextts_amd/csrc/options.hip b/indextts_amd/csrc/options.hip
--- a/indextts_amd/csrc/options.hip
+++ b/indextts_amd/csrc/options.hip
@@ -40,6 +40,8 @@
     {"prefill_attn", -1, -1, 1, "attention of S > 1 passes (prefill, latent pass): -1 causal MFMA kernel in the bf16 mode, canonical-stream kernel in the f32 parity mode; 0 canonical-stream kernel (one block per query) always; 1 MFMA kernel in both precisions"},
     {"voc_act_planes", 1, 0, 1, "vocoder, bf16x3 conv mode: the anti-aliased activation in front of an x3 conv writes the conv's three operand planes itself (aa_act_planes_kernel); 0: f32 activation + split pass (bit-identical planes)"},
     {"x3_waves", 8, 4, 8, "fp32x3 GEMM: waves per 128 x 128 block -- 8 (4 x 2, wave tile 32 x 64, weights through LDS: four waves per SIMD at two blocks per CU; 64-utterance solve 314.7 vs 323.0 ms per Euler step, profiles/r06k) or 4 (2 x 2, wave tile 64 x 64, weights in registers: round 5's kernel); bitwise equal", "4,8"},
+    {"s2mel_prune_last", 1, 0, 1, "fp32x3 s2mel solve with a tail layout: the LAST DiT layer's attention runs the queries of the tail rows only (keys / values: every frame) and writes the tail layout, its wo / FFN norm / w1|w3 / w2 stages run on the tail rows (residual gathered by a row map in the wo epilogue); the x_in GEMM reads its residual from const_in instead of a copy of it; 0: every row, copy first (bitwise equal)"},
+    {"x3_attn_skip", 1, 0, 1, "fp32x3 flash attention: a last key tile with <= 32 valid keys skips the MFMAs of its fully masked half, and a wave whose 32 queries are all out of range only stages its share of K / V^T (0: full tiles, every wave computes; bitwise equal)"},
 };
 std::atomic<int> g_val[OPT_COUNT];
 std::atomic<unsigned> g_epoch{1};
diff --git a/indextts_amd/csrc/s2mel_kernels.h b/indextts_amd/csrc/s2mel_kernels.h
--- a/indextts_amd/csrc/s2mel_kernels.h
+++ b/indextts_amd/csrc/s2mel_kernels.h
@@ -16,7 +16,8 @@
 int launch_cast_pad(const float* in, void* out, int rows, int src_rows, int C_in, int C_out, int prec, hipStream_t st, const int* row_map = nullptr);
 int launch_rope_split(const float* qkv, const float* rope, void* q, void* k, void* v, const SeqTab& tab, int heads, int t_pad, int prec, hipStream_t st);
 int launch_s2mel_attention(const void* q, const void* k, const void* v, void* out, const SeqTab& tab, int heads, int t_pad, int prec, hipStream_t st);
-int launch_s2mel_attention_x3(const void* q, const void* kp, const void* vp, void* out, const SeqTab& tab, int heads, int t_pad, hipStream_t st);
+int launch_s2mel_attention_x3(const void* q, const void* kp, const void* vp, void* out, const SeqTab& tab, int heads, int t_pad, hipStream_t st,
+                              const SeqTab* out_tab = nullptr);
 int launch_split_planes(const float* in, void* out, size_t n, hipStream_t st);
 int launch_ada_rmsnorm_planes(const float* x, const float* g, const float* wb, void* out, size_t plane_stride, int n_tok, int H, float eps, hipStream_t st);
 int launch_trace_hash(const void* p, size_t bytes, unsigned long long* out, hipStream_t st);
diff --git a/indextts_amd/csrc/s2mel_kernels.hip b/indextts_amd/csrc/s2mel_kernels.hip
--- a/indextts_amd/csrc/s2mel_kernels.hip
+++ b/indextts_amd/csrc/s2mel_kernels.hip
@@ -605,19 +605,112 @@
     }
 }
 
+template <int NPROD, int MODE>
+__device__ __forceinline__ void fx3_tile(const char* kt_s, const char* vt_s, const v4u (&qp)[2][3][2], f32x4 (&o)[2][4], float (&m_run)[2], float (&l_run)[2],
+                                         const int (&k_off)[2], const int (&v_off)[2], int k0, int len, int g, float scale_log2e) {
+    constexpr int PA[8] = {2, 1, 2, 0, 1, 1, 0, 0};
+    constexpr int PB[8] = {1, 2, 0, 2, 1, 0, 1, 0};
+    constexpr int NKP = MODE == 2 ? 1 : 2;
+    f32x4 st[2][4];
+#pragma unroll
+    for (int qs = 0; qs < 2; ++qs)
+#pragma unroll
+        for (int kt = 0; kt < 4; ++kt) {
+            const float z = kt < 2 * NKP ? 0.f : -INFINITY;
+            st[qs][kt] = f32x4{z, z, z, z};
+        }
+#pragma unroll
+    for (int kx = 0; kx < 2; ++kx)
+#pragma unroll
+        for (int kp = 0; kp < NKP; ++kp) {
+            v4u ka[2][3];
+#pragma unroll
+            for (int j = 0; j < 2; ++j) {
+                const int kt = 2 * kp + j;
+#pragma unroll
+                for (int p = 0; p < 3; ++p) ka[j][p] = *(const v4u*)(kt_s + p * FX3_PLANE + (32 * (kt >> 1) + 4 * (kt & 1)) * 128 + k_off[kx]);
+            }
+#pragma unroll
+            for (int q = 8 - NPROD; q < 8; ++q)
+#pragma unroll
+                for (int j = 0; j < 2; ++j)
+#pragma unroll
+                    for (int qs = 0; qs < 2; ++qs)
+                        st[qs][2 * kp + j] = __builtin_amdgcn_mfma_f32_16x16x32_bf16(__builtin_bit_cast(bf16x8_t, ka[j][PA[q]]),
+                                                                                     __builtin_bit_cast(bf16x8_t, qp[qs][PB[q]][kx]), st[qs][2 * kp + j], 0, 0, 0);
+        }
+    v4u pb[2][3][2];
+#pragma unroll
+    for (int qs = 0; qs < 2; ++qs) {
+        if constexpr (MODE != 0) {
+#pragma unroll
+            for (int kt = 0; kt < 2 * NKP; ++kt)
+#pragma unroll
+                for (int r = 0; r < 4; ++r)
+                    if ((k0 + 32 * (kt >> 1) + 8 * g + 4 * (kt & 1) + r) >= len) st[qs][kt][r] = -INFINITY;
+        }
+        const float t0 = fa_max3(st[qs][0][0], st[qs][0][1], st[qs][0][2]), t1 = fa_max3(st[qs][1][0], st[qs][1][1], st[qs][1][2]);
+        const float t2 = fa_max3(st[qs][2][0], st[qs][2][1], st[qs][2][2]), t3 = fa_max3(st[qs][3][0], st[qs][3][1], st[qs][3][2]);
+        const float u0 = fa_max3(t0, t1, st[qs][0][3]), u1 = fa_max3(t2, t3, st[qs][1][3]);
+        const float m_new = fa_colmax(fa_max3(u0, u1, fa_max3(st[qs][2][3], st[qs][3][3], m_run[qs])));
+        if (__builtin_amdgcn_ballot_w64(m_new > m_run[qs]) != 0) {
+            const float alpha = __builtin_amdgcn_exp2f((m_run[qs] - m_new) * scale_log2e);
+#pragma unroll
+            for (int mt = 0; mt < 4; ++mt)
+#pragma unroll
+                for (int r = 0; r < 4; ++r) o[qs][mt][r] *= alpha;
+            l_run[qs] *= alpha;
+            m_run[qs] = m_new;
+        }
+        const float off = -m_new * scale_log2e;
+        float psum = 0.f;
+#pragma unroll
+        for (int kt = 0; kt < 2 * NKP; ++kt)
+#pragma unroll
+            for (int r = 0; r < 4; ++r) {
+                const float p = __builtin_amdgcn_exp2f(__builtin_fmaf(st[qs][kt][r], scale_log2e, off));
+                st[qs][kt][r] = p;
+                psum += p;
+            }
+        l_run[qs] += psum;
+#pragma unroll
+        for (int kx = 0; kx < NKP; ++kx) fx3_split8(st[qs][2 * kx], st[qs][2 * kx + 1], pb[qs][0][kx], pb[qs][1][kx], pb[qs][2][kx]);
+    }
+#pragma unroll
+    for (int kx = 0; kx < NKP; ++kx)
+#pragma unroll
+        for (int mp = 0; mp < 2; ++mp) {
+            v4u va[2][3];
+#pragma unroll
+            for (int j = 0; j < 2; ++j)
+#pragma unroll
+                for (int p = 0; p < 3; ++p) va[j][p] = *(const v4u*)(vt_s + p * FX3_PLANE + (2 * mp + j) * 2048 + v_off[kx]);
+#pragma unroll
+            for (int q = 8 - NPROD; q < 8; ++q)
+#pragma unroll
+                for (int j = 0; j < 2; ++j)
+#pragma unroll
+                    for (int qs = 0; qs < 2; ++qs)
+                        o[qs][2 * mp + j] = __builtin_amdgcn_mfma_f32_16x16x32_bf16(__builtin_bit_cast(bf16x8_t, va[j][PA[q]]),
+                                                                                    __builtin_bit_cast(bf16x8_t, pb[qs][PB[q]][kx]), o[qs][2 * mp + j], 0, 0, 0);
+        }
+}
+
 template <int NPROD>
 __global__ __launch_bounds__(512) void flash_attn_x3_kernel(const float* __restrict__ Q, const u16* __restrict__ Kp, const u16* __restrict__ Vp,
-                                                            size_t pstride, float* __restrict__ O, SeqTab tab, int heads, int t_pad, float scale_log2e) {
+                                                            size_t pstride, float* __restrict__ O, SeqTab tab, int heads, int t_pad, float scale_log2e,
+                                                            const int* __restrict__ out_start, const int* __restrict__ out_T, int skip) {
     extern __shared__ __attribute__((aligned(16))) char fx3_sm[];
-    const int s = blockIdx.z, h = blockIdx.y, q0 = blockIdx.x * 256;
+    const int s = blockIdx.z, h = blockIdx.y;
     const int T = tab.seq_T[s], len = tab.seq_len[s];
+    const int cut = T - out_T[s];
+    const int q0 = cut + blockIdx.x * 256;
     if (q0 >= T) return;
     const int H = heads * 64;
     const int tid = threadIdx.x, lane = tid & 63, w = __builtin_amdgcn_readfirstlane(tid >> 6);
     const int g = lane >> 4, c16 = lane & 15;
     const size_t row0 = (size_t)tab.seq_start[s];
-    constexpr int PA[8] = {2, 1, 2, 0, 1, 1, 0, 0};
-    constexpr int PB[8] = {1, 2, 0, 2, 1, 0, 1, 0};
+    const size_t orow0 = (size_t)out_start[s];
     int qi[2];
     bool q_ok[2];
     v4u qp[2][3][2];
@@ -648,6 +741,16 @@
                                              (__attribute__((address_space(3))) void*)(base + (3 + p) * FX3_PLANE), 16, 0, 0);
         }
     };
+    issue(0, 0);
+    if (skip && q0 + w * 32 >= T) {
+        int it = 0;
+        for (int k0 = 0; k0 < len; k0 += 64, ++it) {
+            asm volatile("s_waitcnt vmcnt(0)" ::: "memory");
+            __syncthreads();
+            if (k0 + 64 < len) issue(k0 + 64, (it + 1) & 1);
+        }
+        return;
+    }
     const int krow = 8 * (c16 >> 2) + (c16 & 3);
     const int ksw = ((c16 >> 1) & 1) | ((c16 >> 2) << 1), vsw = (c16 >> 1) & 7;
     int k_off[2], v_off[2];
@@ -665,95 +768,20 @@
 #pragma unroll
         for (int mt = 0; mt < 4; ++mt) o[qs][mt] = f32x4{0.f, 0.f, 0.f, 0.f};
     }
-    issue(0, 0);
-    int it = 0;
-    for (int k0 = 0; k0 < len; k0 += 64, ++it) {
+    int it = 0, k0 = 0;
+    for (; k0 + 64 <= len; k0 += 64, ++it) {
         asm volatile("s_waitcnt vmcnt(0)" ::: "memory");
         __syncthreads();
         if (k0 + 64 < len) issue(k0 + 64, (it + 1) & 1);
         const char* kt_s = fx3_sm + (it & 1) * FX3_STAGE;
-        const char* vt_s = kt_s + 3 * FX3_PLANE;
-        f32x4 st[2][4];
-#pragma unroll
-        for (int qs = 0; qs < 2; ++qs)
-#pragma unroll
-            for (int kt = 0; kt < 4; ++kt) st[qs][kt] = f32x4{0.f, 0.f, 0.f, 0.f};
-#pragma unroll
-        for (int kx = 0; kx < 2; ++kx)
-#pragma unroll
-            for (int kp = 0; kp < 2; ++kp) {
-                v4u ka[2][3];
-#pragma unroll
-                for (int j = 0; j < 2; ++j) {
-                    const int kt = 2 * kp + j;
-#pragma unroll
-                    for (int p = 0; p < 3; ++p) ka[j][p] = *(const v4u*)(kt_s + p * FX3_PLANE + (32 * (kt >> 1) + 4 * (kt & 1)) * 128 + k_off[kx]);
-                }
-#pragma unroll
-                for (int q = 8 - NPROD; q < 8; ++q)
-#pragma unroll
-                    for (int j = 0; j < 2; ++j)
-#pragma unroll
-                        for (int qs = 0; qs < 2; ++qs)
-                            st[qs][2 * kp + j] = __builtin_amdgcn_mfma_f32_16x16x32_bf16(__builtin_bit_cast(bf16x8_t, ka[j][PA[q]]),
-                                                                                         __builtin_bit_cast(bf16x8_t, qp[qs][PB[q]][kx]), st[qs][2 * kp + j], 0, 0, 0);
-            }
-        const bool tail = k0 + 64 > len;
-        v4u pb[2][3][2];
-#pragma unroll
-        for (int qs = 0; qs < 2; ++qs) {
-            if (tail) {
-#pragma unroll
-                for (int kt = 0; kt < 4; ++kt)
-#pragma unroll
-                    for (int r = 0; r < 4; ++r)
-                        if ((k0 + 32 * (kt >> 1) + 8 * g + 4 * (kt & 1) + r) >= len) st[qs][kt][r] = -INFINITY;
-            }
-            const float t0 = fa_max3(st[qs][0][0], st[qs][0][1], st[qs][0][2]), t1 = fa_max3(st[qs][1][0], st[qs][1][1], st[qs][1][2]);
-            const float t2 = fa_max3(st[qs][2][0], st[qs][2][1], st[qs][2][2]), t3 = fa_max3(st[qs][3][0], st[qs][3][1], st[qs][3][2]);
-            const float u0 = fa_max3(t0, t1, st[qs][0][3]), u1 = fa_max3(t2, t3, st[qs][1][3]);
-            const float m_new = fa_colmax(fa_max3(u0, u1, fa_max3(st[qs][2][3], st[qs][3][3], m_run[qs])));
-            if (__builtin_amdgcn_ballot_w64(m_new > m_run[qs]) != 0) {
-                const float alpha = __builtin_amdgcn_exp2f((m_run[qs] - m_new) * scale_log2e);
-#pragma unroll
-                for (int mt = 0; mt < 4; ++mt)
-#pragma unroll
-                    for (int r = 0; r < 4; ++r) o[qs][mt][r] *= alpha;
-                l_run[qs] *= alpha;
-                m_run[qs] = m_new;
-            }
-            const float off = -m_new * scale_log2e;
-            float psum = 0.f;
-#pragma unroll
-            for (int kt = 0; kt < 4; ++kt)
-#pragma unroll
-                for (int r = 0; r < 4; ++r) {
-                    const float p = __builtin_amdgcn_exp2f(__builtin_fmaf(st[qs][kt][r], scale_log2e, off));
-                    st[qs][kt][r] = p;
-                    psum += p;
-                }
-            l_run[qs] += psum;
-#pragma unroll
-            for (int kx = 0; kx < 2; ++kx) fx3_split8(st[qs][2 * kx], st[qs][2 * kx + 1], pb[qs][0][kx], pb[qs][1][kx], pb[qs][2][kx]);
-        }
-#pragma unroll
-        for (int kx = 0; kx < 2; ++kx)
-#pragma unroll
-            for (int mp = 0; mp < 2; ++mp) {
-                v4u va[2][3];
-#pragma unroll
-                for (int j = 0; j < 2; ++j)
-#pragma unroll
-                    for (int p = 0; p < 3; ++p) va[j][p] = *(const v4u*)(vt_s + p * FX3_PLANE + (2 * mp + j) * 2048 + v_off[kx]);
-#pragma unroll
-                for (int q = 8 - NPROD; q < 8; ++q)
-#pragma unroll
-                    for (int j = 0; j < 2; ++j)
-#pragma unroll
-                        for (int qs = 0; qs < 2; ++qs)
-                            o[qs][2 * mp + j] = __builtin_amdgcn_mfma_f32_16x16x32_bf16(__builtin_bit_cast(bf16x8_t, va[j][PA[q]]),
-                                                                                        __builtin_bit_cast(bf16x8_t, pb[qs][PB[q]][kx]), o[qs][2 * mp + j], 0, 0, 0);
-            }
+        fx3_tile<NPROD, 0>(kt_s, kt_s + 3 * FX3_PLANE, qp, o, m_run, l_run, k_off, v_off, k0, len, g, scale_log2e);
+    }
+    if (k0 < len) {
+        asm volatile("s_waitcnt vmcnt(0)" ::: "memory");
+        __syncthreads();
+        const char* kt_s = fx3_sm + (it & 1) * FX3_STAGE;
+        if (len - k0 > (skip ? 32 : 0)) fx3_tile<NPROD, 1>(kt_s, kt_s + 3 * FX3_PLANE, qp, o, m_run, l_run, k_off, v_off, k0, len, g, scale_log2e);
+        else fx3_tile<NPROD, 2>(kt_s, kt_s + 3 * FX3_PLANE, qp, o, m_run, l_run, k_off, v_off, k0, len, g, scale_log2e);
     }
 #pragma unroll
     for (int qs = 0; qs < 2; ++qs) {
@@ -762,7 +790,7 @@
         ls += __shfl_xor(ls, 32, 64);
         if (q_ok[qs]) {
             const float inv = ls > 0.f ? 1.0f / ls : 0.f;
-            float* orow = O + (row0 + qi[qs]) * H + h * 64 + g * 4;
+            float* orow = O + (orow0 + (qi[qs] - cut)) * H + h * 64 + g * 4;
 #pragma unroll
             for (int mt = 0; mt < 4; ++mt)
                 *(f32x4*)(orow + mt * 16) = f32x4{o[qs][mt][0] * inv, o[qs][mt][1] * inv, o[qs][mt][2] * inv, o[qs][mt][3] * inv};
@@ -807,8 +835,13 @@
     return ITTS_OK;
 }
 
-int launch_s2mel_attention_x3(const void* q, const void* kp, const void* vp, void* out, const SeqTab& tab, int heads, int t_pad, hipStream_t st) {
+int launch_s2mel_attention_x3(const void* q, const void* kp, const void* vp, void* out, const SeqTab& tab, int heads, int t_pad, hipStream_t st,
+                              const SeqTab* out_tab) {
     if (tab.n_tok <= 0) return ITTS_OK;
+    if (out_tab && (out_tab->n_seq != tab.n_seq || out_tab->t_max > tab.t_max || out_tab->t_max <= 0)) {
+        itts_set_error("s2mel attention (f32x3): the output layout does not belong to these sequences");
+        return ITTS_ERR_ARG;
+    }
     static ItPerDevice<bool> attr_set_pd;
     bool& attr_set = attr_set_pd.cur();
     if (!attr_set) {
@@ -818,11 +851,16 @@
     }
     const float scale_log2e = 0.125f * 1.4426950408889634f;
     const size_t pstride = (size_t)tab.n_seq * heads * t_pad * 64;
-    const dim3 grid(ceil_div(tab.t_max, 256), heads, tab.n_seq);
+    const int* out_start = out_tab ? out_tab->seq_start : tab.seq_start;
+    const int* out_T = out_tab ? out_tab->seq_T : tab.seq_T;
+    const int skip = itts_opt(OPT_X3_ATTN_SKIP) != 0;
+    const dim3 grid(ceil_div(out_tab ? out_tab->t_max : tab.t_max, 256), heads, tab.n_seq);
     if (itts_opt(OPT_X3_PRODUCTS) == 8)
-        hipLaunchKernelGGL(flash_attn_x3_kernel<8>, grid, dim3(512), FX3_LDS, st, (const float*)q, (const u16*)kp, (const u16*)vp, pstride, (float*)out, tab, heads, t_pad, scale_log2e);
+        hipLaunchKernelGGL(flash_attn_x3_kernel<8>, grid, dim3(512), FX3_LDS, st, (const float*)q, (const u16*)kp, (const u16*)vp, pstride, (float*)out, tab, heads, t_pad, scale_log2e,
+                           out_start, out_T, skip);
     else
-        hipLaunchKernelGGL(flash_attn_x3_kernel<6>, grid, dim3(512), FX3_LDS, st, (const float*)q, (const u16*)kp, (const u16*)vp, pstride, (float*)out, tab, heads, t_pad, scale_log2e);
+        hipLaunchKernelGGL(flash_attn_x3_kernel<6>, grid, dim3(512), FX3_LDS, st, (const float*)q, (const u16*)kp, (const u16*)vp, pstride, (float*)out, tab, heads, t_pad, scale_log2e,
+                           out_start, out_T, skip);
     HIP_TRY(hipGetLastError());
     return ITTS_OK;
 }
```

New measurement: 142.0, median of 6. 1.01x the previous value.
